# Matthew-Mosior/text-compression

Measured on AMD Instinct MI355X. Metric: BWT+MTF+RLE encode MB/s on 1 GiB ACGTN, higher is better.
Workload: dtype u8; 1 GPU; 1 x 1073741824-byte iid ACGTN record(s) (splitmix64 counter generator), fused BWT->MTF->RLE encode, in/out resident in HBM; record_bytes=1073741824, records=1, parallelism=record-per-gpu x1

## Files before the change

include/textcomp_debug.h:

```cpp
#ifndef TEXTCOMP_DEBUG_H
#define TEXTCOMP_DEBUG_H
#include "textcomp.h"
#ifdef __cplusplus
extern "C" {
#endif
int tc_dbg_checksum64_dev(tc_ctx *ctx, const void *d_p, uint64_t bytes, uint64_t *out);
int tc_dbg_stream_bench(tc_ctx *ctx, uint64_t bytes, int width, int mode, int iters, double *gbps);
int tc_dbg_sort_bench(tc_ctx *ctx, uint64_t n, int key_bits, int iters, int check, double *ms_per_pass);
int tc_dbg_scatter_bench(tc_ctx *ctx, uint64_t n, uint32_t bins, uint32_t xrun, int iters, double *ms_per_pass);
int tc_dbg_dispatch_probe(tc_ctx *ctx, uint32_t grid, uint32_t lds_bytes, uint32_t spin_cycles, uint32_t *out6);
int tc_dbg_lcp_set_short_cap(tc_ctx *ctx, uint32_t cap);
int tc_dbg_fm_set_lcp_fanout(tc_ctx *ctx, uint32_t fanout);
int tc_dbg_lz_set_tile(tc_ctx *ctx, uint32_t tile);
int tc_dbg_msd_split_used(tc_ctx *ctx, uint32_t *used);
int tc_dbg_msd_dir(tc_ctx *ctx, uint32_t out[2]);
int tc_dbg_tied_probe(tc_ctx *ctx, uint32_t out[2]);
int tc_dbg_ibwt_walk(tc_ctx *ctx, uint32_t out[3]);
int tc_dbg_seg_sort(tc_ctx *ctx, uint64_t *keys, uint32_t *vals, uint32_t m, int rbits, uint32_t levels[16]);
int tc_dbg_tied_small(tc_ctx *ctx, int mode, uint32_t *slot, uint32_t *idx, uint32_t *grp, uint32_t m,
                      uint32_t *t_idx, uint32_t *t_rank, uint32_t *tpos);
#ifdef __cplusplus
}
#endif
#endif
```

text-compression_amd/csrc/tc_common.hpp:

```cpp
#pragma once
#include <hip/hip_runtime.h>
#include <stdint.h>
#include <stdio.h>
#include <string.h>

#include <string>
#include <vector>

#include "textcomp.h"

typedef uint8_t u8;
typedef uint16_t u16;
typedef uint32_t u32;
typedef uint64_t u64;
typedef int16_t i16;
typedef int32_t i32;
typedef int64_t i64;

#define TC_WAVE 64

struct tc_ctx {
    int device = 0;
    hipStream_t stream = nullptr;
    char *ws = nullptr;
    size_t ws_cap = 0;
    size_t ws_off = 0;
    std::vector<hipMemGenericAllocationHandle_t> ws_chunks;
    size_t ws_chunk_bytes = 0, ws_mapped = 0;
    size_t ws_reserved = 0;
    u32 *d_err = nullptr;
    u64 *d_scalars = nullptr;
    u64 *h_scalars = nullptr;
    u8 *h_hdr = nullptr;
    hipEvent_t ev[8] = {};
    hipEvent_t pev[2 * 16] = {};
    int profile = 0;
    int coding = 0;
    int num_cus = 0;
    int reserved_cus = 0;
    void *hostpipe = nullptr;
    u32 stats_ws_grown = 0;
    u32 lcp_cap = 0;
    u32 fm_lcp_fanout = 0;
    u32 lz_tile = 0;
    int msd_dir_used = 0;
    int msd_split_used = 0;
    int tied_probe_used = 0;
    u32 tied_probe_found = 0;
    u32 ibwt_attempts = 0, ibwt_overflowed = 0, ibwt_extra_taken = 0;
    int mtf_fastin_failed = 0;
    int live_comms = 0;
    int safe_tickets = 0;
    u32 ticket_fallbacks = 0;
    int pev_used = 0;
    std::string err;
    tc_stats stats = {};
};

struct TcFail {
    int code;
};

#define TC_HIP(ctx, expr)                                                                  \
    do {                                                                                   \
        hipError_t e__ = (expr);                                                           \
        if (e__ != hipSuccess) {                                                           \
            char b__[512];                                                                 \
            snprintf(b__, sizeof b__, "%s:%d: %s -> %s", __FILE__, __LINE__, #expr,        \
                     hipGetErrorString(e__));                                              \
            (ctx)->err = b__;                                                              \
            throw TcFail{e__ == hipErrorOutOfMemory ? TC_ERR_OOM : TC_ERR_HIP};            \
        }                                                                                  \
    } while (0)

#define TC_FAIL(ctx, code_, ...)                         \
    do {                                                 \
        char b__[512];                                   \
        snprintf(b__, sizeof b__, __VA_ARGS__);          \
        (ctx)->err = b__;                                \
        throw TcFail{code_};                             \
    } while (0)

#define TC_LAUNCH_CHECK(ctx) TC_HIP(ctx, hipGetLastError())

struct Arena {
    char *base;
    size_t off = 0, peak = 0;
    explicit Arena(char *b) : base(b) {}
    template <class T>
    T *get(size_t count) {
        size_t bytes = (count * sizeof(T) + 255) & ~size_t(255);
        T *p = base ? reinterpret_cast<T *>(base + off) : nullptr;
        off += bytes;
        if (off > peak) peak = off;
        return p;
    }
    void rewind(size_t mark) { off = mark; }
};

void tc_ws_reserve(tc_ctx *ctx, size_t bytes);
template <class F>
static inline void tc_ws_plan(tc_ctx *ctx, size_t base, F &&fn) {
    Arena dry(nullptr);
    fn(dry, true);
    tc_ws_reserve(ctx, base + dry.peak);
    Arena A(ctx->ws + base);
    fn(A, false);
}
u32 tc_persistent_grid(tc_ctx *ctx, int blocks_per_cu);
template <class K>
static inline u32 tc_persistent_grid_for(tc_ctx *ctx, K kernel, int threads, int want_per_cu) {
    int occ = 0;
    if (hipOccupancyMaxActiveBlocksPerMultiprocessor(&occ, kernel, threads, 0) != hipSuccess || occ < 1) {
        (void)hipGetLastError();
        occ = 1;
    }
    return tc_persistent_grid(ctx, occ < want_per_cu ? occ : want_per_cu);
}
void *tc_chunked_alloc(tc_ctx *ctx, size_t bytes, int chunk_log2, void **handle);
void tc_chunked_free(void *handle);
void tc_sync_check(tc_ctx *ctx);

static inline u32 tc_cdiv(u64 a, u64 b) { return (u32)((a + b - 1) / b); }

#ifdef __HIPCC__

__device__ __forceinline__ u32 lane_id() { return __lane_id(); }

__device__ __forceinline__ u64 lanemask_lt() {
    return (1ull << lane_id()) - 1ull;
}

__device__ __forceinline__ u32 wave_incl_sum(u32 v) {
#pragma unroll
    for (int d = 1; d < 64; d <<= 1) {
        u32 t = __shfl_up(v, d, 64);
        if ((int)lane_id() >= d) v += t;
    }
    return v;
}
__device__ __forceinline__ u32 wave_incl_max(u32 v) {
#pragma unroll
    for (int d = 1; d < 64; d <<= 1) {
        u32 t = __shfl_up(v, d, 64);
        if ((int)lane_id() >= d) v = v > t ? v : t;
    }
    return v;
}
__device__ __forceinline__ u64 wave_incl_max64(u64 v) {
#pragma unroll
    for (int d = 1; d < 64; d <<= 1) {
        u64 t = __shfl_up(v, d, 64);
        if ((int)lane_id() >= d) v = v > t ? v : t;
    }
    return v;
}
__device__ __forceinline__ u32 wave_sum(u32 v) {
#pragma unroll
    for (int d = 32; d >= 1; d >>= 1) v += __shfl_xor(v, d, 64);
    return v;
}
__device__ __forceinline__ u64 wave_max64(u64 v) {
#pragma unroll
    for (int d = 32; d >= 1; d >>= 1) {
        u64 t = __shfl_xor(v, d, 64);
        v = v > t ? v : t;
    }
    return v;
}

template <int NT>
__device__ __forceinline__ u32 block_excl_sum(u32 v, u32 *smem, u32 *total) {
    const int w = threadIdx.x >> 6;
    u32 inc = wave_incl_sum(v);
    __syncthreads();
    if (lane_id() == 63) smem[w] = inc;
    __syncthreads();
    u32 base = 0, tot = 0;
#pragma unroll
    for (int i = 0; i < NT / 64; i++) {
        u32 s = smem[i];
        if (i < w) base += s;
        tot += s;
    }
    *total = tot;
    return base + inc - v;
}

template <int NT>
__device__ __forceinline__ u64 block_incl_max64(u64 v, u64 *smem, u64 *total) {
    const int w = threadIdx.x >> 6;
    u64 inc = wave_incl_max64(v);
    __syncthreads();
    if (lane_id() == 63) smem[w] = inc;
    __syncthreads();
    u64 base = 0, tot = 0;
#pragma unroll
    for (int i = 0; i < NT / 64; i++) {
        u64 s = smem[i];
        if (i < w) base = base > s ? base : s;
        tot = tot > s ? tot : s;
// ... 99 lines not shown
```

text-compression_amd/csrc/tc_msd.hpp:

```cpp
#pragma once
#include "tc_sa.hpp"
#include "tc_msd_dir.hpp"

#ifndef MSD_NT
#define MSD_NT 1024
#endif
#ifndef MSD_ITEMS
#define MSD_ITEMS 8
#endif
#define MSD_TILE (MSD_NT * MSD_ITEMS)
#ifndef MSD_GROUP
#define MSD_GROUP 16
#endif
#define MSD_GLOG (MSD_GROUP == 32 ? 5 : MSD_GROUP == 16 ? 4 : 3)
#ifndef MSD_SUB
#define MSD_SUB 1
#endif
#ifndef MSD_BPC
#define MSD_BPC 1
#endif
#define MSD_LEVELS 3
#define MSDF_CAP_SMALL 2048
#ifndef MSDF_KO_NT
#define MSDF_KO_NT 256
// ... 19 lines not shown
    u32 ntot;
    const u32 *cnt_in;
    u32 *flags;
    u64 *dbg;
    u32 *dirfills;
};

#ifdef __HIPCC__

__device__ __forceinline__ u32 msd_tile_lo(u32 T, u32 b, u32 G) { return (u32)(((u64)T * b) / G); }
__device__ __forceinline__ u32 msd_block_of_tile(u32 T, u32 t, u32 G) {
    return (u32)((((u64)t + 1) * G - 1) / T);
}

__global__ void msd_root_kernel(u32 *pstart, u32 *pcnt, u32 N, u32 *maxchild, u32 *dirfills) {
    pstart[0] = 0;
    pcnt[0] = N;
    *maxchild = 0;
    *dirfills = 0;
}

__device__ __forceinline__ u32 msd_block_of_parent(const MsdLevel &L, u32 q, u32 G) {
    return (u32)(((u64)L.pstart[q] * G) / L.ntot);
}
__device__ __forceinline__ u32 msd_first_parent(const MsdLevel &L, u32 b, u32 G) {
    if (b == 0) return 0;
    if (b >= G) return L.nparents;
    u32 lo = 0, hi = L.nparents;
    while (lo < hi) {
        const u32 mid = (lo + hi) >> 1;
        if (msd_block_of_parent(L, mid, G) >= b) hi = mid; else lo = mid + 1;
    }
    return lo;
}
__device__ __forceinline__ void msd_block_range(const MsdLevel &L, u32 b, u32 G, u32 *t0, u32 *t1) {
    if (L.aligned) {
        *t0 = L.tpre[msd_first_parent(L, b, G)];
        *t1 = L.tpre[msd_first_parent(L, b + 1, G)];
    } else {
        const u32 T = L.tpre[L.nparents];
        *t0 = (u32)(((u64)T * b) / G);
        *t1 = (u32)(((u64)T * (b + 1)) / G);
    }
}

__global__ __launch_bounds__(1024) void msd_prep_kernel(const u32 *__restrict__ pcnt, u32 nparents,
                                                        u32 *__restrict__ tpre) {
    __shared__ u32 s_scan[1024 / 64 + 1];
    const u32 per = (nparents + 1023) / 1024;
    const u32 lo = threadIdx.x * per;
    u32 sum = 0;
    if (per == 64 && nparents == 65536u) {
        uint4 v[16];
        const uint4 *pv = reinterpret_cast<const uint4 *>(pcnt + lo);
#pragma unroll
        for (int i = 0; i < 16; i++) v[i] = pv[i];
        u32 t[64];
#pragma unroll
        for (int i = 0; i < 16; i++) {
            t[4 * i] = (v[i].x + MSD_TILE - 1) / MSD_TILE; t[4 * i + 1] = (v[i].y + MSD_TILE - 1) / MSD_TILE;
            t[4 * i + 2] = (v[i].z + MSD_TILE - 1) / MSD_TILE; t[4 * i + 3] = (v[i].w + MSD_TILE - 1) / MSD_TILE;
        }
#pragma unroll
        for (int i = 0; i < 64; i++) sum += t[i];
        u32 tot;
        u32 run = block_excl_sum<1024>(sum, s_scan, &tot);
        uint4 *ov = reinterpret_cast<uint4 *>(tpre + lo);
#pragma unroll
        for (int i = 0; i < 16; i++) {
            uint4 o;
            o.x = run; run += t[4 * i];
            o.y = run; run += t[4 * i + 1];
            o.z = run; run += t[4 * i + 2];
            o.w = run; run += t[4 * i + 3];
            ov[i] = o;
        }
        if (threadIdx.x == 0) tpre[nparents] = tot;
        return;
    }
    for (u32 i = 0; i < per; i++) {
        const u32 q = lo + i;
        if (q < nparents) sum += (pcnt[q] + MSD_TILE - 1) / MSD_TILE;
    }
    u32 tot;
    u32 run = block_excl_sum<1024>(sum, s_scan, &tot);
    for (u32 i = 0; i < per; i++) {
        const u32 q = lo + i;
        if (q < nparents) {
            tpre[q] = run;
            run += (pcnt[q] + MSD_TILE - 1) / MSD_TILE;
        }
    }
    if (threadIdx.x == 0) tpre[nparents] = tot;
}

__device__ __forceinline__ u32 msd_find_parent(const u32 *tpre, u32 nparents, u32 t) {
    u32 lo = 0, hi = nparents;
    while (hi - lo > 1) {
        const u32 mid = (lo + hi) >> 1;
        if (tpre[mid] <= t) lo = mid; else hi = mid;
    }
    return lo;
}

struct MsdTileInfo {
    u32 base;
    u32 valid;
    u32 q;
    u32 last;
};
struct MsdCur {
    u32 q, tq0, tq1, ps, pc;
};
__device__ __forceinline__ void msd_cur_init(const MsdLevel &L, MsdCur &c, u32 t) {
    c.q = msd_find_parent(L.tpre, L.nparents, t);
    c.tq0 = L.tpre[c.q]; c.tq1 = L.tpre[c.q + 1]; c.ps = L.pstart[c.q]; c.pc = L.pcnt[c.q];
}
__device__ __forceinline__ void msd_cur_info(const MsdLevel &L, MsdCur &c, u32 t, u32 t_end, MsdTileInfo *out) {
    if (t >= t_end) {
        out->base = 0; out->valid = 0; out->q = 0; out->last = 0;
        return;
    }
    if (t >= c.tq1) {
        u32 q = c.q + 1;
        while (L.tpre[q + 1] <= t) q++;
        c.q = q; c.tq0 = L.tpre[q]; c.tq1 = L.tpre[q + 1]; c.ps = L.pstart[q]; c.pc = L.pcnt[q];
    }
    const u32 off = (t - c.tq0) * MSD_TILE;
    out->base = c.ps + off;
    out->valid = c.pc - off < MSD_TILE ? c.pc - off : MSD_TILE;
    out->q = c.q;
    out->last = (t + 1 >= t_end || t + 1 >= c.tq1) ? 1u : 0u;
}

struct MsdTextDigit {
    const u8 *text;
    u32 n;
    u32 B, s;
    u16 lut[256];
    u32 hash_ok, hsh, tlo, thi;
};

#ifndef MSD_XCD_MAP
#define MSD_XCD_MAP 0
#endif
__device__ __forceinline__ u32 msd_logical_wg(u32 b, u32 G) {
    return (MSD_XCD_MAP && (G & 7u) == 0) ? (b & 7u) * (G >> 3) + (b >> 3) : b;
}

struct MsdJointRows {
    u8 row[256];
    u8 dig[128];
};
template <bool TEXT, bool JOINT, bool HI>
__device__ __forceinline__ void msd_count_body(const MsdLevel &L, const u64 *__restrict__ keys,
                                               const MsdTextDigit &td, u32 *__restrict__ joint_out,
                                               const MsdJointRows &jr) {
    static_assert(!HI || (!TEXT && JOINT), "the high halves serve the joint count of keys only");
    __shared__ u32 s_cnt[256];
    __shared__ u16 s_lut[TEXT ? 256 : 1];
    __shared__ u32 s_seg[4];
    __shared__ u32 s_joint[JOINT ? 32768 : 1];
    const u32 tid = threadIdx.x, G = gridDim.x, b = msd_logical_wg(blockIdx.x, G);
    if (tid < 256) s_cnt[tid] = 0;
    if (TEXT && tid < 256) s_lut[tid] = td.lut[tid];
    __shared__ u8 s_row[JOINT ? 256 : 1];
    if (JOINT) {
        for (u32 i = tid; i < 32768; i += MSD_NT) s_joint[i] = 0;
        if (tid < 256) s_row[tid] = jr.row[tid];
    }
    const u32 T = L.tpre[L.nparents];
    const u32 t0 = msd_tile_lo(T, b, G), t1 = msd_tile_lo(T, b + 1, G);
    if (t0 >= t1) return;
    u32 t = t0;
    u32 q = 0;
    if (tid == 0) q = msd_find_parent(L.tpre, L.nparents, t0);
    while (t < t1) {
        if (tid == 0) {
            while (L.tpre[q + 1] <= t) q++;
            const u32 tq0 = L.tpre[q], tq1 = L.tpre[q + 1];
            const u32 te = tq1 < t1 ? tq1 : t1;
            const u32 ps = L.pstart[q], pc = L.pcnt[q];
            const u32 lo = ps + (t - tq0) * MSD_TILE;
            const u64 hi = (u64)ps + (u64)(te - tq0) * MSD_TILE;
            s_seg[0] = q; s_seg[1] = lo; s_seg[2] = hi < (u64)ps + pc ? (u32)hi : ps + pc; s_seg[3] = te;
        }
        __syncthreads();
        const u32 sq = s_seg[0], lo = s_seg[1], hi = s_seg[2];
        t = s_seg[3];
        if (TEXT) {
            const bool words = td.s <= 5 && (u64)lo + 8 < td.n && ((((uintptr_t)td.text) + lo) & 15) == 0;
            u32 p = lo;
            if (words) {
                const u32 span = (u64)hi + 8 <= td.n ? hi - lo : td.n - 8 - lo;
                const u32 nfull = span / (16 * MSD_NT);
                const u32 *tw = reinterpret_cast<const u32 *>(td.text + lo);
                auto fetch = [&](u32 r, u32 *x) {
                    const u32 wi = (r * MSD_NT + tid) * 4;
#pragma unroll
                    for (int q = 0; q < 5; q++) x[q] = tw[wi + q];
                };
                auto tally = [&](const u32 *x) {
                    u32 cd[20];
                    if (td.hash_ok) {
#pragma unroll
                        for (int q = 0; q < 5; q++) {
                            const u32 y = __builtin_amdgcn_perm(td.thi, td.tlo, (x[q] >> td.hsh) & 0x07070707u);
#pragma unroll
                            for (int j = 0; j < 4; j++) cd[4 * q + j] = (y >> (8 * j)) & 255u;
                        }
                    } else {
#pragma unroll
                        for (int j = 0; j < 20; j++) cd[j] = s_lut[(x[j >> 2] >> (8 * (j & 3))) & 255u];
                    }
#pragma unroll
                    for (int k = 0; k < 16; k++) {
                        u32 g = 0;
#pragma unroll
                        for (int j = 0; j < 5; j++)
                            if (j < (int)td.s) g = g * td.B + cd[k + j];
                        atomicAdd(&s_cnt[g], 1u);
                    }
                };
                u32 r = 0;
                for (; r + 4 <= nfull; r += 4) {
                    u32 xa[5], xb[5], xc[5], xd[5];
                    fetch(r, xa); fetch(r + 1, xb); fetch(r + 2, xc); fetch(r + 3, xd);
                    tally(xa); tally(xb); tally(xc); tally(xd);
                }
                for (; r < nfull; r++) {
                    u32 x[5];
                    fetch(r, x);
                    tally(x);
                }
                p = lo + nfull * 16 * MSD_NT;
            }
            for (u64 i0 = (u64)p + tid; i0 < hi; i0 += MSD_NT) {
                u64 i = i0;
                u32 g = 0;
                for (u32 j = 0; j < td.s; j++, i++) g = g * td.B + (i < td.n ? (u32)s_lut[td.text[i]] : 0u);
                atomicAdd(&s_cnt[g], 1u);
            }
        } else {
            auto add_dd = [&](u32 dd) {
                if (JOINT) {
                    const u32 r = s_row[dd >> 8];
                    if (r != 0xffu) atomicAdd(&s_joint[(r << 8) | (dd & 255u)], 1u);
                    else {
                        atomicAdd(&s_cnt[dd >> 8], 1u);
                        atomicAdd(&joint_out[((size_t)sq * 256 + (dd >> 8)) * 256 + (dd & 255u)], 1u);
                    }
                } else {
                    atomicAdd(&s_cnt[dd >> 8], 1u);
                }
            };
            auto add = [&](u64 k) { add_dd((u32)(k >> (L.shift - 8)) & 0xffffu); };
            if (HI) {
                const u32 *khi = reinterpret_cast<const u32 *>(keys);
                const u32 hs = (u32)L.shift - 40u;
                auto add4 = [&](const uint4 v) {
                    add_dd((v.x >> hs) & 0xffffu); add_dd((v.y >> hs) & 0xffffu);
                    add_dd((v.z >> hs) & 0xffffu); add_dd((v.w >> hs) & 0xffffu);
                };
                const u32 a0 = (lo + 3u) & ~3u, a = a0 < hi ? a0 : hi;
                if (lo + tid < a) add_dd((khi[lo + tid] >> hs) & 0xffffu);
                const u32 nq = (hi - a) >> 2;
                const uint4 *q4 = reinterpret_cast<const uint4 *>(khi + a);
                u32 i = tid;
                for (; i + 3 * MSD_NT < nq; i += 4 * MSD_NT) {
                    const uint4 v0 = q4[i], v1 = q4[i + MSD_NT], v2 = q4[i + 2 * MSD_NT], v3 = q4[i + 3 * MSD_NT];
                    add4(v0); add4(v1); add4(v2); add4(v3);
                }
                for (; i < nq; i += MSD_NT) add4(q4[i]);
                const u32 p = a + 4 * nq + tid;
                if (p < hi) add_dd((khi[p] >> hs) & 0xffffu);
            } else {
                u32 p = lo + tid;
                for (; p + 3 * MSD_NT < hi; p += 4 * MSD_NT) {
                    const u64 k0 = keys[p], k1 = keys[p + MSD_NT], k2 = keys[p + 2 * MSD_NT], k3 = keys[p + 3 * MSD_NT];
                    add(k0); add(k1); add(k2); add(k3);
                }
                for (; p < hi; p += MSD_NT) add(keys[p]);
            }
        }
        __syncthreads();
        if (JOINT) {
            for (u32 w = tid; w < 32768; w += MSD_NT) {
                const u32 v = s_joint[w];
                if (v) {
                    atomicAdd(&joint_out[((size_t)sq * 256 + jr.dig[w >> 8]) * 256 + (w & 255u)], v);
                    atomicAdd(&s_cnt[jr.dig[w >> 8]], v);
                    s_joint[w] = 0;
                }
            }
            __syncthreads();
        }
        if (tid < 256) {
            L.seg[((size_t)sq + b) * 256 + tid] = s_cnt[tid];
            s_cnt[tid] = 0;
        }
    }
}
template <bool TEXT, bool JOINT>
__global__ __launch_bounds__(MSD_NT) void msd_count_kernel(MsdLevel L, const u64 *__restrict__ keys,
                                                           MsdTextDigit td, u32 *__restrict__ joint_out,
                                                           MsdJointRows jr) {
    msd_count_body<TEXT, JOINT, false>(L, keys, td, joint_out, jr);
}
__global__ __launch_bounds__(MSD_NT) void msd_count_hi_kernel(MsdLevel L, const u32 *__restrict__ khi,
                                                              MsdTextDigit td, u32 *__restrict__ joint_out,
                                                              MsdJointRows jr) {
    msd_count_body<false, true, true>(L, reinterpret_cast<const u64 *>(khi), td, joint_out, jr);
}

__global__ __launch_bounds__(256) void msd_scan_kernel(MsdLevel L, u32 G, u32 *maxchild) {
    __shared__ u32 s_scan[256 / 64 + 1];
    const u32 q = blockIdx.x, d = threadIdx.x;
    const u32 cnt = L.pcnt[q];
    const size_t c = (size_t)q * 256 + d;
    if (cnt == 0) {
        L.ccnt[c] = 0;
        L.cstart[c] = L.pstart[q];
        return;
    }
    if (L.aligned) {
        const u32 tot = L.cnt_in[c];
        u32 all;
        const u32 excl = block_excl_sum<256>(tot, s_scan, &all);
        const u32 start = L.pstart[q] + excl;
        L.cstart[c] = start;
        L.ccnt[c] = tot;
        L.seg[((size_t)q + msd_block_of_parent(L, q, G)) * 256 + d] = start;
        if (d == 0 && all != cnt) atomicOr(L.flags, 8u);
        if (maxchild) {
            u32 m = tot;
#pragma unroll
            for (int x = 32; x >= 1; x >>= 1) {
                const u32 o = __shfl_xor(m, x, 64);
                m = m > o ? m : o;
            }
            if ((d & 63) == 0 && m > MSDF_CAP_SMALL) atomicMax(maxchild, m);
        }
        return;
    }
    const u32 T = L.tpre[L.nparents];
    const u32 bf = msd_block_of_tile(T, L.tpre[q], G), bl = msd_block_of_tile(T, L.tpre[q + 1] - 1, G);
    u32 tot = 0;
#pragma unroll 8
    for (u32 b = bf; b <= bl; b++) {
        const u32 v = L.seg[((size_t)q + b) * 256 + d];
        tot += msd_tile_lo(T, b, G) < msd_tile_lo(T, b + 1, G) ? v : 0u;
    }
    u32 all;
    const u32 excl = block_excl_sum<256>(tot, s_scan, &all);
    u32 run = L.pstart[q] + excl;
    L.cstart[c] = run;
    L.ccnt[c] = tot;
#pragma unroll 8
    for (u32 b = bf; b <= bl; b++) {
        const size_t o = ((size_t)q + b) * 256 + d;
        const u32 v = L.seg[o];
        if (msd_tile_lo(T, b, G) >= msd_tile_lo(T, b + 1, G)) continue;
        L.seg[o] = run;
        run += v;
    }
    if (maxchild) {
        u32 m = tot;
#pragma unroll
        for (int x = 32; x >= 1; x >>= 1) {
            const u32 o = __shfl_xor(m, x, 64);
            m = m > o ? m : o;
        }
        if ((d & 63) == 0 && m > MSDF_CAP_SMALL) atomicMax(maxchild, m);
    }
}

typedef u32 msd_u32x4 __attribute__((ext_vector_type(4)));
template <bool KEYGEN, bool VALS, bool SPLIT, bool DIR = false>
__device__ __forceinline__ void msd_partition_body(const MsdLevel &L, const u64 *kin, const u32 *vin,
                                                   u64 *kout, u32 *vout, u32 *shi, u32 *slo, const u8 *text,
                                                   const RadixKeyGen &kg) {
    static_assert(!SPLIT || !VALS, "the split layout is the key-only levels'");
    static_assert(!DIR || (!KEYGEN && !SPLIT), "the directory is the aligned level's");
    __shared__ __attribute__((aligned(16))) u64 s_keys[MSD_TILE];
    __shared__ __attribute__((aligned(16))) u32 s_vals[VALS ? MSD_TILE : 4];
    __shared__ __attribute__((aligned(16))) u64 c_keys[256 * MSD_GROUP];
    __shared__ __attribute__((aligned(16))) u32 c_vals[VALS ? 256 * MSD_GROUP : 4];
    __shared__ u32 s_cnt[256 * MSD_SUB], s_dstart[256 * MSD_SUB], s_r[256], s_cur[256], s_ph[256];
    __shared__ u32 s_scan[16];
    __shared__ u64 s_lmask[4];
#ifdef MSD_PROFILE
    __shared__ u64 s_dbg[2];
    if (threadIdx.x == 0) { s_dbg[0] = 0; s_dbg[1] = 0; }
#endif
    __shared__ u16 s_live[256];
    __shared__ u16 s_klut[KEYGEN ? 256 : 1];
    constexpr bool KG_SPLIT = KEYGEN && !VALS && MSD_ITEMS == 8;
    __shared__ __attribute__((aligned(16))) u8 s_kr[KG_SPLIT ? MSD_TILE + 16 + 80 + 32 : 16];
    __shared__ __attribute__((aligned(16))) u8 s_kg8[KG_SPLIT ? MSD_TILE + 64 : 16];
    __shared__ u32 s_scan2[2];
    static_assert(MSD_GROUP == 8 || MSD_GROUP == 16 || MSD_GROUP == 32, "group = 8, 16 or 32 pairs");
    constexpr u32 DIRCAP = DIR ? (VALS ? 128 : 1024) : 1;
    __shared__ MsdDirEnt s_dir[DIRCAP];
    __shared__ u32 s_rseg[DIR ? 256 : 1];
    __shared__ u64 s_rmask[4];
    __shared__ u32 s_nq[4], s_dst[6];
    static_assert(((size_t)MSD_TILE * (VALS ? 12 : 8) + 256 * MSD_GROUP * (VALS ? 12 : 8) + 8192 + (KG_SPLIT ? 2 * MSD_TILE + 256 : 0) + (DIR ? DIRCAP * sizeof(MsdDirEnt) + 1024 + 128 : 0)) * (VALS ? 1 : MSD_BPC) <= 163840, "LDS budget");
    __shared__ MsdTileInfo s_info[4];

    const u32 tid = threadIdx.x, G = gridDim.x, b = msd_logical_wg(blockIdx.x, G);
    if (KEYGEN && tid < 256) s_klut[tid] = kg.lut[tid];
    if (tid < 256) { s_r[tid] = 0; s_ph[tid] = 0; s_cur[tid] = 0; }
    for (u32 i = tid; i < 256 * MSD_SUB; i += MSD_NT) s_cnt[i] = 0;
    if (DIR) {
        if (tid == 0 || tid == 64) {
            const u32 w = tid >> 6;
            u32 q = 0, tq = 0;
            if (!(*L.flags & 8u)) {
                q = msd_first_parent(L, b + w, G);
                tq = L.tpre[q];
            }
            s_scan2[w] = tq; s_dst[1 + w] = q;
        }
        if (tid == 0) { s_dst[0] = 0; s_dst[3] = 0; s_dst[4] = MSD_DIR_NONE; }
    } else if (tid == 0) {
        u32 ta = 0, tb = 0;
        if (!(L.aligned && (*L.flags & 8u))) msd_block_range(L, b, G, &ta, &tb);
        s_scan2[0] = ta; s_scan2[1] = tb;
    }
    __syncthreads();
    const u32 t0 = s_scan2[0], t1 = s_scan2[1];
    if (t0 >= t1) return;
    MsdCur cs = {};
    u32 dir_e = 0, dir_k = 0;
    auto dir_refill = [&]() {
        u32 n = 0, qn = s_dst[1];
        const u32 qe = s_dst[2];
        while (n == 0 && qn < qe) {
            const u32 q = qn + tid;
            const bool in = q < qe;
            const u32 pc = in ? L.pcnt[q] : 0u, ps = in ? L.pstart[q] : 0u;
            const u64 m = __ballot(pc != 0);
            if ((tid & 63) == 0) s_scan[tid >> 6] = (u32)__popcll(m);
            __syncthreads();
            u32 before = 0, tot = 0;
#pragma unroll
            for (u32 i = 0; i < MSD_NT / 64; i++) {
                const u32 c = s_scan[i];
                tot += c;
                before += i < (tid >> 6) ? c : 0u;
            }
            const u32 rank = before + (u32)__popcll(m & ((1ull << (tid & 63)) - 1ull));
            if (pc != 0 && rank < DIRCAP) { s_dir[rank].q = q; s_dir[rank].ps = ps; s_dir[rank].pc = pc; }
            if (pc != 0 && rank == DIRCAP) s_dst[5] = q;
            __syncthreads();
            if (tot > DIRCAP) { n = DIRCAP; qn = s_dst[5]; }
            else { n = tot; qn = qe - qn < (u32)MSD_NT ? qe : qn + MSD_NT; }
            if (tid == 0) atomicAdd(L.dirfills, 1u);
        }
        __syncthreads();
        if (tid == 0) { s_dst[0] = n; s_dst[1] = qn; s_dst[3] = 0; }
        dir_e = 0; dir_k = 0;
    };
    auto dir_gen = [&](u32 x) {
        MsdDirCur c = {dir_e, dir_k, s_dst[0], s_dst[1], s_dst[2], s_dst[3]};
// ... 1083 lines not shown
```

text-compression_amd/csrc/tc_sa.hpp:

```cpp
#pragma once
#include <type_traits>
#include "tc_radix.hpp"

#define SA_NT 256
#define SA_ITEMS 16
#define SA_TILE (SA_NT * SA_ITEMS)
#define KB_HALO 72

struct SaConfig {
    u32 sigma_text;
    u32 B;
    u32 w;
    u32 s;
    u32 P;
    u32 h0;
    double entropy;
    u16 lut[256];
};

#ifdef __HIPCC__

__global__ __launch_bounds__(256) void hist256_kernel(const u8 *__restrict__ text, u64 n,
                                                      u32 *__restrict__ counts) {
    __shared__ u32 s_h[256 * 64];
// ... 349 lines not shown
            slot = slots[k];
        }
        const u64 mle = hb[k] & ((2ull << l) - 1ull);
        const u32 hl = mle ? 63u - (u32)__builtin_clzll(mle) : 0u;
        const u32 sv = INIT ? 0u : (u32)__shfl((int)slot, (int)hl, 64);
        const u32 g = mle ? (INIT ? (u32)(jb + hl) : sv) : cur_head - 1u;
        if (hb[k]) {
            u32 hlast = 63u - (u32)__builtin_clzll(hb[k]);
            cur_head = (INIT ? (u32)(jb + hlast) : (u32)__shfl((int)slot, (int)hlast, 64)) + 1u;
        }
        const u32 o = cur_cnt + (u32)__popcll(ab[k] & lanemask_lt());
        cur_cnt += (u32)__popcll(ab[k]);
        if (!in) continue;
        if (INIT) {
            if (a.isa_only) {
                if (a.pairs) a.pairs[j] = ((u64)a.vals[j] << 32) | g;
                else a.isa[a.vals[j]] = g;
            } else {
                a.L[j] = (u8)(lowb[k >> 2] >> (8 * (k & 3)));
                const u32 v = a.vals[j];
                if (a.pairs) a.pairs[j] = ((u64)v << 32) | g;
                else if (a.isa) a.isa[v] = g;
                if (act) {
                    a.out_slot[o] = (u32)j;
                    a.out_idx[o] = v;
                    a.out_grp[o] = g;
                }
            }
        } else {
            const u32 i = a.vals_are_idx ? k0 : a.in_idx[k0];
            if (!act) {
                a.sa[slot] = i;
                a.L[slot] = i ? a.text[i - 1] : (u8)0;
            }
            const bool moved = g != reinterpret_cast<const u32 *>(a.keys)[2 * j + 1];
            u32 tp = 0;
            if (a.pairs) a.pairs[j] = moved ? ((u64)i << 32) | g : ~0ull;
            else if (a.isa) { if (moved) a.isa[i] = g; }
            else if (!a.norank) {
                tp = a.in_tpos[k0];
                if (moved) a.t_rank[tp] = g;
            }
            if (act) {
                a.out_slot[o] = slot;
                a.out_idx[o] = i;
                a.out_grp[o] = g;
                if (!a.isa && !a.norank) a.out_tpos[o] = tp;
            }
        }
    }
    __syncthreads();
    }
}

#define RBIN_NT 1024
#define RBIN_ITEMS 16
#define RBIN_TILE (RBIN_NT * RBIN_ITEMS)

__global__ __launch_bounds__(256) void rank_cursor_kernel(u32 *cursor, int shift) {
    cursor[threadIdx.x] = (u32)threadIdx.x << shift;
}

__global__ __launch_bounds__(RBIN_NT) void rank_bin_kernel(const u64 *__restrict__ in, u32 m, int shift,
                                                           u32 *__restrict__ cursor, u64 *__restrict__ out, u64 nslots) {
    __shared__ u64 s_stage[RBIN_TILE];
    __shared__ u32 s_cnt[256], s_lb[256], s_gb[256];
    __shared__ u32 s_scan[RBIN_NT / 64 + 1];
    const u32 tid = threadIdx.x;
    const u64 base = (u64)blockIdx.x * RBIN_TILE;
    const u32 valid = (u64)m - base < (u64)RBIN_TILE ? (u32)((u64)m - base) : (u32)RBIN_TILE;
    if (tid < 256) s_cnt[tid] = 0;
    __syncthreads();
    u64 v[RBIN_ITEMS];
    u32 r[RBIN_ITEMS];
#pragma unroll
    for (int k = 0; k < RBIN_ITEMS; k++) {
        const u32 p = k * RBIN_NT + tid;
        v[k] = p < valid ? in[base + p] : 0ull;
    }
#pragma unroll
    for (int k = 0; k < RBIN_ITEMS; k++) {
        const u32 p = k * RBIN_NT + tid;
        if (p >= valid) v[k] = ~0ull;
        if (v[k] != ~0ull) r[k] = atomicAdd(&s_cnt[(u32)(v[k] >> 32) >> shift], 1u);
    }
    __syncthreads();
    const u32 c = tid < 256 ? s_cnt[tid] : 0u;
    u32 tot;
    const u32 lb = block_excl_sum<RBIN_NT>(c, s_scan, &tot);
    if (tid < 256) {
        s_lb[tid] = lb;
        s_gb[tid] = c ? atomicAdd(&cursor[tid], c) : 0u;
    }
    __syncthreads();
#pragma unroll
    for (int k = 0; k < RBIN_ITEMS; k++) {
        const u32 p = k * RBIN_NT + tid;
        if (v[k] != ~0ull) s_stage[s_lb[(u32)(v[k] >> 32) >> shift] + r[k]] = v[k];
    }
    __syncthreads();
#pragma unroll
    for (int k = 0; k < RBIN_ITEMS; k++) {
        const u32 p = k * RBIN_NT + tid;
        if (p < tot) {
            const u64 x = s_stage[p];
            const u32 d = (u32)(x >> 32) >> shift;
            const u64 g = (u64)s_gb[d] + (p - s_lb[d]);
            if (g < nslots) out[g] = x;
        }
    }
}

#define RSCAT_NT 256
#define RSCAT_ITEMS 8
__global__ __launch_bounds__(RSCAT_NT) void rank_scatter_kernel(const u64 *__restrict__ part, u64 nslots, int shift,
                                                                 const u32 *__restrict__ cursor, u32 *__restrict__ isa) {
    const u64 base = (u64)blockIdx.x * (RSCAT_NT * RSCAT_ITEMS);
    u64 x[RSCAT_ITEMS];
    u32 cur[RSCAT_ITEMS];
    bool ok[RSCAT_ITEMS];
#pragma unroll
    for (int k = 0; k < RSCAT_ITEMS; k++) {
        const u64 p = base + (u64)k * RSCAT_NT + threadIdx.x;
        cur[k] = p < nslots ? cursor[p >> shift] : 0u;
    }
#pragma unroll
    for (int k = 0; k < RSCAT_ITEMS; k++) {
        const u64 p = base + (u64)k * RSCAT_NT + threadIdx.x;
        ok[k] = p < nslots && (u32)p < cur[k];
        x[k] = ok[k] ? part[p] : 0ull;
    }
#pragma unroll
    for (int k = 0; k < RSCAT_ITEMS; k++)
        if (ok[k]) isa[(u32)(x[k] >> 32)] = (u32)x[k];
}

#ifndef FIN_WPW
#define FIN_WPW 8
#endif
#ifndef FIN_NT
#define FIN_NT 256
#endif

__global__ __launch_bounds__(256) void unary_sa_kernel(const u8 *__restrict__ text, u32 n, u32 *__restrict__ sa,
                                                        u8 *__restrict__ L) {
    const u64 j = (u64)blockIdx.x * 256 + threadIdx.x;
    if (j > n) return;
    sa[j] = n - (u32)j;
    L[j] = j < n ? text[0] : (u8)0;
}

#define SAMP_N 8192
#define SAMP_SLOTS 16384
__global__ __launch_bounds__(1024) void sample_dup_kernel(const u8 *__restrict__ text, u32 n, RadixKeyGen kg,
                                                           int topbits, u32 *out) {
    __shared__ u32 table[SAMP_SLOTS];
    __shared__ u16 s_lut[256];
    __shared__ u32 s_dups;
    for (int i = threadIdx.x; i < SAMP_SLOTS; i += 1024) table[i] = 0xFFFFFFFFu;
    if (threadIdx.x < 256) s_lut[threadIdx.x] = kg.lut[threadIdx.x];
    if (threadIdx.x == 0) s_dups = 0;
    __syncthreads();
    u32 dups = 0;
    const u32 nf = ((u32)topbits + kg.w - 1) / kg.w;
    constexpr int SPT = SAMP_N / 1024;
    const bool words = nf * kg.s <= 16;
    u32 tw[SPT][4];
    u64 qs[SPT];
#pragma unroll
    for (int j = 0; j < SPT; j++) {
        const u32 k = threadIdx.x + 1024u * (u32)j;
        u64 z = (u64)(k + 1) * 0x9E3779B97F4A7C15ull;
        z = (z ^ (z >> 29)) * 0xBF58476D1CE4E5B9ull;
        qs[j] = (u64)(((z >> 32) * (u64)n) >> 32);
        const bool in = words && qs[j] + 16 <= n;
#pragma unroll
        for (int x = 0; x < 4; x++) {
            u32 v = 0;
            if (in) __builtin_memcpy(&v, text + qs[j] + 4 * x, 4);
            tw[j][x] = v;
        }
    }
#pragma unroll
    for (int j = 0; j < SPT; j++) {
        u64 q = qs[j];
        const bool in = words && q + 16 <= n;
        u64 key = 0;
        int sh = 64;
        u32 pos = 0;
        for (u32 f = 0; f < nf; f++) {
            u32 g = 0;
            for (u32 t = 0; t < kg.s; t++, q++, pos++) {
                u32 c;
                if (in) {
                    u32 wsel = tw[j][0];
                    wsel = (pos >> 2) == 1 ? tw[j][1] : wsel;
                    wsel = (pos >> 2) == 2 ? tw[j][2] : wsel;
                    wsel = (pos >> 2) == 3 ? tw[j][3] : wsel;
                    c = (u32)s_lut[(wsel >> (8 * (pos & 3))) & 255u];
                } else {
                    c = q < n ? (u32)s_lut[text[q]] : 0u;
                }
                g = g * kg.B + c;
            }
            sh -= kg.w;
            key |= (u64)g << sh;
        }
        u64 kt = key >> (64 - topbits);
        if (topbits > 32) kt = (kt ^ (kt >> 31)) * 0xD6E8FEB86659FD93ull >> 32;
        const u32 v = (u32)kt;
        if (v == 0xFFFFFFFFu) continue;
        u32 slot = (v * 0x9E3779B1u) >> 18;
        for (int probe = 0; probe < SAMP_SLOTS; probe++) {
            const u32 old = atomicCAS(&table[slot], 0xFFFFFFFFu, v);
            if (old == 0xFFFFFFFFu) break;
            if (old == v) { dups++; break; }
            slot = (slot + 1) & (SAMP_SLOTS - 1);
        }
    }
    dups = wave_sum(dups);
    if (lane_id() == 0 && dups) atomicAdd(&s_dups, dups);
    __syncthreads();
    if (threadIdx.x == 0) *out = s_dups;
}

struct FinishArgs {
    const u64 *keys;
    const u32 *sa_in;
    u32 N;
    int tshift;
    int lshift, lbits;
    u32 *sa_out;
    u8 *L;
    u32 *out_slot, *out_idx, *out_grp;
    u32 act_cap;
    u32 *counters;
    u32 *rcount;
    u32 rcap;
    u32 fix_cap;
    u32 *ovbits;
};

#define FIN_REGIONS 64
#define FIN_RSTRIDE 64
#ifndef FIN_STAGE
#define FIN_STAGE 192
#endif
__global__ __launch_bounds__(FIN_NT) void finish_kernel(FinishArgs a) {
    __shared__ u32 s_low[FIN_NT / 64][128];
#if FIN_STAGE
    __shared__ u32 s_stg[FIN_NT / 64][3][FIN_STAGE + 128];
#endif
    const int w = threadIdx.x >> 6, l = threadIdx.x & 63;
    u32 *low = s_low[w];
#if FIN_STAGE
    __shared__ u32 s_nstg[FIN_NT / 64];
    __shared__ u32 s_base;
    u32 nstg = 0;
    const u32 region = blockIdx.x % FIN_REGIONS;
    u32 *rctr = a.rcount + region * FIN_RSTRIDE;
    const u32 rbase = region * a.rcap;
    auto flush = [&](bool have_base, u32 base) {
        if (!have_base) {
            if (l == 0) base = atomicAdd(rctr, nstg);
            base = __shfl(base, 0, 64);
        }
        __builtin_amdgcn_wave_barrier();
        for (u32 e = l; e < nstg; e += 64) {
            const u32 o = rbase + base + e;
            if (base + e < a.rcap) {
                a.out_slot[o] = s_stg[w][0][e];
                a.out_idx[o] = s_stg[w][1][e];
                a.out_grp[o] = s_stg[w][2][e];
            }
        }
        __builtin_amdgcn_wave_barrier();
        nstg = 0;
    };
#endif
    const u64 N = a.N;
    const u64 wave = (u64)blockIdx.x * (FIN_NT / 64) + w;
    const u64 ws0 = wave * 64 * FIN_WPW;
#if !FIN_STAGE
#error "finish_kernel needs the staged hand-over (FIN_STAGE > 0)"
#endif
    const u64 lowmask = a.lbits >= 64 ? ~0ull : ((1ull << a.lbits) - 1ull);

    u64 kk[FIN_WPW + 1];
    u32 vv[FIN_WPW + 1];
    const bool interior = ws0 + (u64)(FIN_WPW + 1) * 64 <= N;
    if (interior) {
#pragma unroll
        for (int c = 0; c <= FIN_WPW; c++) {
            const u64 pos = ws0 + (u64)c * 64 + l;
            kk[c] = a.keys[pos];
            vv[c] = a.sa_in[pos];
        }
    } else {
#pragma unroll
        for (int c = 0; c <= FIN_WPW; c++) {
            const u64 pos = ws0 + (u64)c * 64 + l;
            kk[c] = pos < N ? a.keys[pos] : ~0ull;
            vv[c] = pos < N ? a.sa_in[pos] : 0u;
        }
    }
    u64 tprev = (ws0 > 0 && ws0 <= N) ? (a.keys[ws0 - 1] >> a.tshift) : 0;
    bool hasprev = ws0 > 0;

    auto window = [&](auto full_tag, const int win) {
        constexpr bool FULL = decltype(full_tag)::value;
        const u64 ws = ws0 + (u64)win * 64;
        if (!FULL && ws >= N) return;
        const u64 kA = kk[win], kB = kk[win + 1];
        const u32 vA = vv[win], vB = vv[win + 1];
        const bool inA = FULL || ws + l < N, inB = FULL || ws + 64 + l < N;
        const u64 tA = kA >> a.tshift, tB = kB >> a.tshift;
        u64 upA = __shfl_up(tA, 1, 64);
        u64 lastA = __shfl(tA, 63, 64);
        u64 upB = __shfl_up(tB, 1, 64);
        bool hA = inA && ((l == 0) ? (!hasprev || tA != tprev) : (tA != upA));
        bool hB = inB && ((l == 0) ? (tB != lastA) : (tB != upB));
        const u64 hbA = __ballot(hA), hbB = __ballot(hB);
        const u64 inbA = __ballot(inA), inbB = __ballot(inB);
        const int a0 = hbA ? __builtin_ctzll(hbA) : 64;
        const int b0 = hbB ? __builtin_ctzll(hbB) : 64;
        if (hbA && !hbB && (~inbB) == 0ull) {
            if (l == 0 && !(__hip_atomic_load(&a.counters[1], __ATOMIC_RELAXED, __HIP_MEMORY_SCOPE_AGENT) & 1u))
                atomicOr(&a.counters[1], 1u);
        }
        const bool ownA = inA && l >= a0;
        const bool ownB = inB && hbA && l < b0;
        u64 mleA = hbA & ((2ull << l) - 1ull);
        int sA = mleA ? 63 - __builtin_clzll(mleA) : 0;
        u64 mgtA = (l == 63) ? 0ull : (hbA & ~((2ull << l) - 1ull));
        int endA_in_A = mgtA ? __builtin_ctzll(mgtA) : -1;
        int lastHeadA = hbA ? 63 - __builtin_clzll(hbA) : 0;
        int endB = b0 < 64 ? 64 + b0 : (int)(__popcll(inbA) + __popcll(inbB));
        int tAend = endA_in_A >= 0 ? endA_in_A : endB;
        const u32 lowA = (u32)((kA >> a.lshift) & lowmask), lowB = (u32)((kB >> a.lshift) & lowmask);
        low[l] = lowA;
        low[64 + l] = lowB;
        __builtin_amdgcn_wave_barrier();
        const int cA = l, cB = 64 + l;
        const int sB = lastHeadA, tBend = endB;
        int lenA = ownA ? tAend - sA : 0;
        int maxlen = lenA;
#pragma unroll
        for (int d = 32; d >= 1; d >>= 1) {
            int o = __shfl_xor(maxlen, d, 64);
            maxlen = maxlen > o ? maxlen : o;
        }
        u32 rankA = 0, ltA = 0, leA = 0;
        for (int t = 0; t < maxlen; t++) {
            const int u = sA + t;
            if (ownA && u < tAend) {
                const u32 y = low[u];
                ltA += y < lowA;
                leA += y <= lowA;
                rankA += (y < lowA) | ((y == lowA) & (u < cA));
            }
        }
        const u32 eqA = ownA ? leA - ltA - 1u : 0u;
        u32 rankB = 0, ltB = 0, leB = 0;
        if (hbA && b0 > 0) {
            for (int u = sB; u < tBend; u++) {
                const u32 y = low[u];
                ltB += y < lowB;
                leB += y <= lowB;
                rankB += (y < lowB) | ((y == lowB) & (u < cB));
            }
        }
        const u32 eqB = ownB ? leB - ltB - 1u : 0u;
        __builtin_amdgcn_wave_barrier();
        const bool actA = ownA && eqA > 0, actB = ownB && eqB > 0;
        const u64 abA = __ballot(actA), abB = __ballot(actB);
        const u32 nact = (u32)__popcll(abA) + (u32)__popcll(abB);
// ... 964 lines not shown
```

text-compression_amd/csrc/tc_sa_host.hpp:

```cpp
#pragma once
#include <chrono>

#include "tc_sa_plan.hpp"

#ifndef SA_KDIR_BITS
#define SA_KDIR_BITS 26
#endif
struct SaBuffers {
    u64 *k0, *k1;
    u32 *v0, *v1;
    u32 *isa;
    u32 *v2;
    u32 *act[2][4];
    u64 *sk[2];
    u32 *sv[2];
    u32 *t_idx, *t_rank;
    u64 *t_bits;
    u32 *t_dir;
    u32 *t_bsum;
    u32 *fin_rc;
    u32 *kdir;
    u64 sparse_cap;
    u32 *hist;
    u64 *rstatus;
    u64 *gstatus;
    u32 *counts;
    u32 *msd_pstart[MSD_LEVELS + 1], *msd_pcnt[MSD_LEVELS + 1];
    u32 *msd_tpre[MSD_LEVELS], *msd_seg[MSD_LEVELS];
    u32 *msd_joint;
    u32 msd_grid;
    TiedTable tp;
    SegBuffers seg;
    u32 *chain_ref, *chain_code, *chain_summ;
};

static inline u64 msd_min_n() { return (u64)env_int("TC_SA_MSD_MIN_LOG2", 27) >= 40 ? ~0ull : 1ull << env_int("TC_SA_MSD_MIN_LOG2", 27); }
static inline bool msd_wanted(u64 N) { return env_int("TC_SA_MSD", 1) != 0 && N >= msd_min_n() && N >= 1024; }

static void seg_carve(Arena &A, u64 N, SegBuffers &g) {
    g.cap_runs = (size_t)(N / SEG_CAP + 2);
    g.cap_tiles = (size_t)(N / SEG_PT + 2) + g.cap_runs;
    g.segbits = A.get<u64>(seg_bit_words(N));
    g.ybits = A.get<u64>(seg_bit_words(N));
    for (int q = 0; q < 2; q++) {
        g.lstart[q] = A.get<u32>(g.cap_runs);
        g.lsize[q] = A.get<u32>(g.cap_runs);
        g.ltbase[q] = A.get<u32>(g.cap_runs);
        g.lshift[q] = A.get<u32>(g.cap_runs);
    }
    g.tile_seg = A.get<u32>(g.cap_tiles);
    g.hist = A.get<u32>(g.cap_runs * 256);
    g.mm = A.get<u32>(g.cap_runs * 2);
    g.counters = A.get<u32>(64);
}

static size_t sa_carve(Arena &A, u64 N, SaBuffers &b, bool own_v1) {
    b.k0 = A.get<u64>(N + 32);
    b.k1 = A.get<u64>(N);
    b.v0 = A.get<u32>(N);
    b.v1 = own_v1 ? A.get<u32>(N) : nullptr;
    b.isa = A.get<u32>(N + 1);
    b.v2 = A.get<u32>(N);
    b.sparse_cap = N / 8 + 1024;
    for (int s = 0; s < 2; s++) {
        for (int q = 0; q < 3; q++) b.act[s][q] = A.get<u32>(N);
        b.act[s][3] = A.get<u32>(b.sparse_cap);
        b.sk[s] = A.get<u64>(b.sparse_cap);
        b.sv[s] = A.get<u32>(b.sparse_cap);
    }
    b.t_idx = A.get<u32>(b.sparse_cap);
    b.t_rank = A.get<u32>(b.sparse_cap);
    b.t_bits = A.get<u64>(N / 64 + 2);
    b.t_dir = A.get<u32>(N / 64 + 2);
    b.t_bsum = A.get<u32>(N / 64 / BDIR_TILE + 2);
    b.fin_rc = A.get<u32>(FIN_REGIONS * FIN_RSTRIDE + 128);
    b.kdir = A.get<u32>(((size_t)1 << SA_KDIR_BITS) + 2 + ((size_t)1 << SA_KDIR_BITS) / KDF_CHUNK + 64);
    b.hist = A.get<u32>(RDX_MAX_PASSES * RDX_BINS);
    b.rstatus = A.get<u64>(radix_status_words(N));
    b.gstatus = A.get<u64>(2 * (size_t)tc_cdiv(N, GRP_TILE) + 4);
    b.counts = A.get<u32>(260);
    seg_carve(A, N, b.seg);
    for (int l = 0; l <= MSD_LEVELS; l++) b.msd_pstart[l] = b.msd_pcnt[l] = nullptr;
    if (msd_wanted(N)) {
        b.msd_grid = 256 * MSD_BPC;
        size_t np = 1;
        for (int l = 0; l <= MSD_LEVELS; l++, np *= 256) {
            b.msd_pstart[l] = A.get<u32>(np);
            b.msd_pcnt[l] = A.get<u32>(np);
            if (l < MSD_LEVELS) {
                b.msd_tpre[l] = A.get<u32>(np + 1);
                b.msd_seg[l] = A.get<u32>((np + b.msd_grid) * 256);
            }
        }
        b.msd_joint = A.get<u32>((size_t)256 * 256 * 256);
        b.tp.key = A.get<u64>((size_t)1 << TP_SLOT_BITS);
        b.tp.grp = A.get<u32>((size_t)1 << TP_SLOT_BITS);
        b.tp.cnt = A.get<u32>((size_t)1 << TP_SLOT_BITS);
        b.tp.bloom = A.get<u32>(((size_t)1 << TP_BLOOM_LOG2) / 32);
    }
    b.chain_ref = A.get<u32>(N + 1);
    b.chain_code = A.get<u32>(N + 1);
    b.chain_summ = A.get<u32>(chain_summ_words());
    return A.off;
}

enum SaSlot {
    SA_SLOT_PRIMARY = 0,
    SA_SLOT_ACTIVE = 1,
    SA_SLOT_PROBE = 11,
    SA_SLOT_TIED = 12,
    SA_SLOT_DROPPED = 13,
    SA_SLOT_SAMPLE = 14,
    SA_SLOT_MAXCHILD = 15,
    SA_SLOT_SEG = 24,
    SA_SLOT_ERR = 62,
    SA_SLOT_MSD_PROF = 64,
    SA_SLOT_MSDK_PROF = 112,
    SA_SLOT_MSD_DIR = 122,
};
static inline u32 sa_slot_lo(const tc_ctx *ctx, int slot) { return (u32)(ctx->h_scalars[slot] & 0xffffffffu); }
static inline u32 sa_slot_hi(const tc_ctx *ctx, int slot) { return (u32)(ctx->h_scalars[slot] >> 32); }
static inline u32 *sa_dev_slot(tc_ctx *ctx, int slot) { return reinterpret_cast<u32 *>(ctx->d_scalars + slot); }

#ifdef SEG_PROFILE
static void seg_profile_dump(tc_ctx *ctx, u32 m) {
    u64 h[16];
    TC_HIP(ctx, hipStreamSynchronize(ctx->stream));
    TC_HIP(ctx, hipMemcpyFromSymbol(h, HIP_SYMBOL(seg_prof), sizeof h));
    const double w = (double)(h[7] | 1);
    fprintf(stderr, "seg_small: %llu members, %llu windows (that sort), mid members per window %.0f | cycles per window: bits %.0f attr+masks %.0f (prefix) %.0f image %.0f tiny+compact %.0f tiny store %.0f network %.0f store %.0f\n",
            (unsigned long long)m, (unsigned long long)h[7], h[8] / w, h[0] / w, h[1] / w, 0.0, h[2] / w, h[3] / w, h[4] / w, h[5] / w, h[6] / w);
    memset(h, 0, sizeof h);
    TC_HIP(ctx, hipMemcpyToSymbol(HIP_SYMBOL(seg_prof), h, sizeof h));
}
#else
static inline void seg_profile_dump(tc_ctx *, u32) {}
#endif

static void seg_sort_pairs(tc_ctx *ctx, SegBuffers &g, u64 *kx, u32 *vx, u64 *ky, u32 *vy, u32 m, int rbits,
                           u32 *levels = nullptr) {
    hipStream_t s = ctx->stream;
    if (levels) memset(levels, 0, 16 * sizeof(u32));
    const u32 nwords = (u32)seg_bit_words(m);
    TC_HIP(ctx, hipMemsetAsync(g.ybits, 0, (size_t)nwords * sizeof(u64), s));
    TC_HIP(ctx, hipMemsetAsync(g.counters, 0, 8 * sizeof(u32), s));
    u32 igrid = tc_cdiv((u64)nwords * 64, 256);
    if (igrid > 16384) igrid = 16384;
    seg_init_kernel<<<igrid, 256, 0, s>>>(kx, m, g.segbits, nwords, g.lstart[0], g.lsize[0], g.ltbase[0], g.lshift[0],
                                          (u32)(rbits > 8 ? rbits - 8 : 0), g.counters, (u32)g.cap_runs);
    TC_LAUNCH_CHECK(ctx);
    const int nlev = 8;
    int cur = 0;
    for (int L = 0;; L++) {
        TC_HIP(ctx, hipMemcpyAsync(&ctx->h_scalars[SA_SLOT_SEG], g.counters + 2 * cur, 2 * sizeof(u32), hipMemcpyDeviceToHost, s));
        TC_HIP(ctx, hipStreamSynchronize(s));
        const u32 S = sa_slot_lo(ctx, SA_SLOT_SEG), T = sa_slot_hi(ctx, SA_SLOT_SEG);
        if (S == 0) break;
        if (levels && L < nlev) { levels[2 * L] = S; levels[2 * L + 1] = T; }
        if (L >= nlev) TC_FAIL(ctx, TC_ERR_INTERNAL, "segmented sort: %u runs still unsorted after %d levels", S, nlev);
        if (S > g.cap_runs || T > g.cap_tiles) TC_FAIL(ctx, TC_ERR_INTERNAL, "segmented sort: %u long runs / %u tiles exceed the tables", S, T);
        const int nxt = cur ^ 1;
        TC_HIP(ctx, hipMemsetAsync(g.hist, 0, (size_t)S * 256 * sizeof(u32), s));
        seg_mm_init_kernel<<<tc_cdiv(S, 256), 256, 0, s>>>(g.mm, S);
        TC_LAUNCH_CHECK(ctx);
        TC_HIP(ctx, hipMemsetAsync(g.counters + 2 * nxt, 0, 2 * sizeof(u32), s));
        u32 wgrid = tc_cdiv(S, 4);
        if (wgrid > 8192) wgrid = 8192;
        seg_tilemap_kernel<<<wgrid, 256, 0, s>>>(g.lsize[cur], g.ltbase[cur], S, g.tile_seg, (u32)g.cap_tiles);
        TC_LAUNCH_CHECK(ctx);
        seg_count_kernel<<<T, 256, 0, s>>>(kx, ky, g.lstart[cur], g.lsize[cur], g.ltbase[cur], g.lshift[cur], g.tile_seg, g.counters + 2 * cur, g.hist, g.mm);
        TC_LAUNCH_CHECK(ctx);
        seg_scan_kernel<<<wgrid, 256, 0, s>>>(g.lstart[cur], g.lsize[cur], g.lshift[cur], g.counters + 2 * cur, g.hist, g.mm, g.segbits, 0,
                                              g.lstart[nxt], g.lsize[nxt], g.ltbase[nxt], g.lshift[nxt], g.counters + 2 * nxt, (u32)g.cap_runs);
        TC_LAUNCH_CHECK(ctx);
        seg_scatter_kernel<<<T, 256, 0, s>>>(kx, vx, ky, vy, g.lstart[cur], g.lsize[cur], g.ltbase[cur], g.lshift[cur], g.tile_seg, g.counters + 2 * cur,
                                             g.hist, g.mm, g.ybits);
        TC_LAUNCH_CHECK(ctx);
        cur = nxt;
    }
    seg_small_kernel<<<tc_cdiv(m, SEG_SPAN), SEG_NT, 0, s>>>(kx, vx, ky, vy, m, g.segbits, g.ybits);
    TC_LAUNCH_CHECK(ctx);
    seg_profile_dump(ctx, m);
}

static void sa_choose_config(const u32 *counts, u64 n, int forced_fields, SaConfig &c) {
    u32 sig = 0;
    double H = 0;
    for (int v = 0; v < 256; v++) {
        c.lut[v] = 0;
        if (counts[v]) {
            c.lut[v] = (u16)(++sig);
            double p = (double)counts[v] / (double)n;
            H -= p * log2(p);
        }
    }
    c.sigma_text = sig;
    c.B = sig + 1;
    if (c.B <= 16) {
        c.w = 8;
        c.s = 1;
        u32 pw = c.B;
        while (pw * c.B <= 256) {
            pw *= c.B;
            c.s++;
        }
    } else {
        c.s = 1;
        c.w = (u32)ceil_log2_u64(c.B);
    }
    u32 pmax = 56 / c.w;
    double need = (double)ceil_log2_u64(n + 1) + 8.0;
    double per_field = H * c.s;
    u32 P = pmax;
    if (per_field > 1e-9) {
        double pf = ceil(need / per_field);
        if (pf < (double)pmax) P = (u32)pf;
    }
    if (P < 1) P = 1;
    if (forced_fields > 0) P = (u32)forced_fields;
    if (P > pmax) P = pmax;
    c.P = P;
    c.h0 = P * c.s;
    c.entropy = H;
}

static void sa_run(tc_ctx *ctx, SaBuffers &b, const u8 *d_text, u64 n, u32 *d_sa, u8 *d_L,
                   u64 *primary, u32 *counts256_out);

struct TicketTrip {};
__global__ void err_or_kernel(u32 *err, u32 bits) { atomicOr(err, bits); }
static void ticket_check(tc_ctx *ctx) {
    if (env_int("TC_DBG_TICKET_TRIP", 0) != 0) {
        err_or_kernel<<<1, 1, 0, ctx->stream>>>(ctx->d_err, 2u);
        TC_LAUNCH_CHECK(ctx);
    }
    TC_HIP(ctx, hipMemcpyAsync(&ctx->h_scalars[SA_SLOT_ERR], ctx->d_err, sizeof(u32), hipMemcpyDeviceToHost,
                               ctx->stream));
    TC_HIP(ctx, hipStreamSynchronize(ctx->stream));
    if (sa_slot_lo(ctx, SA_SLOT_ERR) & 2u) throw TicketTrip{};
}

static void sa_build(tc_ctx *ctx, Arena &A, const u8 *d_text, u64 n, u32 *d_sa, u8 *d_L,
                     u64 *primary, u32 *counts256_out, bool dry) {
    const u64 N = n + 1;
    SaBuffers b;
    sa_carve(A, N, b, d_sa == nullptr);
    if (dry) return;
    try {
        sa_run(ctx, b, d_text, n, d_sa, d_L, primary, counts256_out);
    } catch (const TicketTrip &) {
        tc_memset_async(ctx, ctx->d_err, 0, sizeof(u32));
        ctx->safe_tickets = 1;
        ctx->ticket_fallbacks++;
        sa_run(ctx, b, d_text, n, d_sa, d_L, primary, counts256_out);
    }
    ctx->stats.ticket_fallbacks = ctx->ticket_fallbacks;
}

struct SaRun {
    tc_ctx *ctx;
    SaBuffers &b;
    const u8 *text;
    u64 n, N;
    int rbits;
    u32 *d_sa;
    u32 *sa;
    u8 *d_L;
    SaKnobs K;
    SaConfig cfg;
    int rshift;
    u64 bin_min;
    u64 *part_act1;
    bool part_act1_ok;
    u64 m = 0;
    u64 h_start = 0;
    const u64 *skeys = nullptr;
    const u64 *tkeys = nullptr;
    int tkeys_shift = 0;
    bool isa_ready = false;
    bool dense = false;
    RankLookup rl = {};
    std::chrono::steady_clock::time_point trace_t0;

    hipStream_t stream() const { return ctx->stream; }
    tc_stats &st() const { return ctx->stats; }
};

template <class X>
static inline void sa_fill(const SaConfig &c, X &x) {
    x.B = c.B; x.w = c.w; x.s = c.s; x.P = c.P;
    memcpy(x.lut, c.lut, sizeof x.lut);
}
static inline void sa_fill(const SaConfig &c, MsdTextDigit &x) {
    x.B = c.B; x.s = c.s;
    memcpy(x.lut, c.lut, sizeof x.lut);
}
static RadixKeyGen sa_keygen(const SaRun &R) {
    RadixKeyGen kg;
    sa_fill(R.cfg, kg);
    kg.n_text = (u32)R.n;
    kg.hash_ok = 0; kg.hsh = 0; kg.tlo = 0; kg.thi = 0;
    return kg;
}
static RadixBuffers sa_radix_buffers(const SaRun &R, u64 *keys, u64 *keys_alt, u32 *vals, u32 *vals_alt) {
    RadixBuffers rb;
    rb.keys = keys; rb.keys_alt = keys_alt; rb.vals = vals; rb.vals_alt = vals_alt;
    rb.hist = R.b.hist; rb.status = R.b.rstatus; rb.status_cap = radix_status_words(R.N);
    return rb;
}
static RadixBuffers sa_sparse_buffers(const SaRun &R) {
    return sa_radix_buffers(R, R.b.sk[0], R.b.sk[1], R.b.sv[0], R.b.sv[1]);
}

static void sa_trace_buffers(const SaRun &R) {
    if (R.K.trace != 2) return;
    fprintf(stderr, "textcomp: buffers text %p k0 %p k1 %p v0 %p v1 %p sa %p L %p\n", (const void *)R.text, (void *)R.b.k0,
            (void *)R.b.k1, (void *)R.b.v0, (void *)R.b.v1, (void *)R.d_sa, (void *)R.d_L);
}
static void sa_trace_step(SaRun &R, const char *what, u64 count) {
    if (!R.K.trace) return;
    (void)hipStreamSynchronize(R.stream());
    auto t1 = std::chrono::steady_clock::now();
    fprintf(stderr, "textcomp:   %-28s %10llu  %8.3f ms\n", what, (unsigned long long)count,
            std::chrono::duration<double, std::milli>(t1 - R.trace_t0).count());
    R.trace_t0 = t1;
}
static void sa_trace_tied_checksums(SaRun &R, u32 fm) {
    if (R.K.trace < 2 || fm == 0) return;
    tc_ctx *ctx = R.ctx;
    std::vector<u32> hk(fm), hh(fm), hs(fm), hg(fm);
    tc_d2h(ctx, hk.data(), R.b.act[0][1], fm * sizeof(u32));
    tc_d2h(ctx, hh.data(), R.b.act[0][3], fm * sizeof(u32));
    tc_d2h(ctx, hs.data(), R.b.act[0][0], fm * sizeof(u32));
    tc_d2h(ctx, hg.data(), R.b.act[0][2], fm * sizeof(u32));
    TC_HIP(ctx, hipStreamSynchronize(R.stream()));
    u64 a1 = 0, a2 = 0, a3 = 0, a4 = 0;
    for (u32 i = 0; i < fm; i++) { a1 += hk[i]; a2 += hh[i]; a3 += hs[i]; a4 += hg[i]; }
    fprintf(stderr, "textcomp: tied members: sum klo %llx khi %llx slot %llx grp %llx\n", (unsigned long long)a1, (unsigned long long)a2, (unsigned long long)a3, (unsigned long long)a4);
    for (u32 i = 0; i < fm && i < 6; i++) fprintf(stderr, "textcomp:   member %u: klo %08x khi %06x slot %u grp %u\n", i, hk[i], hh[i], hs[i], hg[i]);
}
static void sa_trace_group_sizes(SaRun &R, int cur, u32 mm) {
    if (!R.K.trace) return;
    tc_ctx *ctx = R.ctx;
    u64 *gh = reinterpret_cast<u64 *>(R.b.hist);
    tc_memset_async(ctx, gh, 0, 32 * sizeof(u64));
    group_size_hist_kernel<<<tc_cdiv(mm, 256), 256, 0, R.stream()>>>(R.b.act[cur][0], R.b.act[cur][2], mm, gh);
    u64 hh32[32];
    tc_d2h(ctx, hh32, gh, sizeof hh32);
    (void)hipStreamSynchronize(R.stream());
    fprintf(stderr, "textcomp:   members by group size 2^c:");
    for (int c = 0; c < 32; c++) if (hh32[c]) fprintf(stderr, " %d:%.1f%%", c, 100.0 * (double)hh32[c] / (double)mm);
    fprintf(stderr, "\n");
    R.trace_t0 = std::chrono::steady_clock::now();
}
static void sa_trace_chain_tables(SaRun &R, int cur, u32 mm, u32 hh, const ChainDims &cd, const u64 *chain_path, const u64 *chain_sign) {
    if (!R.K.trace) return;
    tc_ctx *ctx = R.ctx;
    unsigned long long *dg = reinterpret_cast<unsigned long long *>(R.b.hist);
    tc_memset_async(ctx, dg, 0, 8 * sizeof(u64));
    chain_diag_kernel<<<4096, 256, 0, R.stream()>>>(R.b.act[cur][1], R.b.act[cur][2], mm, chain_path, chain_sign, R.b.chain_code, dg);
    u64 hd[8];
    tc_d2h(ctx, hd, dg, sizeof hd);
    (void)hipStreamSynchronize(R.stream());
    fprintf(stderr, "textcomp:   chain tables (h = %u, %u x %u cells of %u rows, %s ranks): members %u, on path %llu, k = 0: %llu, largest k %llu\n",
            hh, cd.nb, cd.h, cd.bk, R.dense ? "dense" : "sparse", mm, (unsigned long long)hd[0], (unsigned long long)hd[1], (unsigned long long)hd[2]);
    R.trace_t0 = std::chrono::steady_clock::now();
}
#ifdef MSDK_PROFILE
static void msdk_profile_dump(tc_ctx *ctx) {
    u64 h[10];
    tc_d2h(ctx, h, ctx->d_scalars + SA_SLOT_MSDK_PROF, sizeof h);
    TC_HIP(ctx, hipStreamSynchronize(ctx->stream));
    const double c = (double)(h[8] | 1);
    fprintf(stderr, "finish (key-only): chunks %llu, keys per chunk %.0f | cycles per chunk: land %.0f B %.0f zero+B %.0f bins+B %.0f scan+B %.0f scatter+B %.0f walk+prefetch+rank+B %.0f copy-out %.0f\n",
            (unsigned long long)h[8], h[9] / c, h[0] / c, h[1] / c, h[2] / c, h[3] / c, h[4] / c, h[5] / c, h[6] / c, h[7] / c);
    tc_memset_async(ctx, ctx->d_scalars + SA_SLOT_MSDK_PROF, 0, sizeof h);
}
#else
static inline void msdk_profile_dump(tc_ctx *) {}
#endif
#ifdef MSD_PROFILE
static void msd_profile_dump(tc_ctx *ctx) {
    u64 h[48];
    tc_d2h(ctx, h, ctx->d_scalars + SA_SLOT_MSD_PROF, sizeof h);
    TC_HIP(ctx, hipStreamSynchronize(ctx->stream));
    for (int l = 0; l < MSD_LEVELS; l++)
        fprintf(stderr, "msd level %d: tiles %llu | cursor+B0 %llu keygen/S1+B1 %llu S2 %llu S3 %llu land %llu B3 %llu S4 %llu (cycles per tile)\n", l + 1,
                (unsigned long long)h[16 * l + 1], (unsigned long long)(h[16 * l] / (h[16 * l + 1] | 1)), (unsigned long long)(h[16 * l + 2] / (h[16 * l + 1] | 1)),
                (unsigned long long)(h[16 * l + 3] / (h[16 * l + 1] | 1)), (unsigned long long)(h[16 * l + 4] / (h[16 * l + 1] | 1)), (unsigned long long)(h[16 * l + 5] / (h[16 * l + 1] | 1)),
                (unsigned long long)(h[16 * l + 6] / (h[16 * l + 1] | 1)), (unsigned long long)(h[16 * l + 7] / (h[16 * l + 1] | 1)));
    for (int l = 0; l < MSD_LEVELS; l++)
        fprintf(stderr, "   level %d, S1 alone per tile: wave 0 %llu, last wave %llu cycles; slowest wave B0 -> before B1 %llu, B0 -> prefetch issued %llu\n", l + 1,
                (unsigned long long)(h[16 * l + 8] / (h[16 * l + 1] | 1)), (unsigned long long)(h[16 * l + 9] / (h[16 * l + 1] | 1)),
                (unsigned long long)(h[16 * l + 10] / (h[16 * l + 1] | 1)), (unsigned long long)(h[16 * l + 11] / (h[16 * l + 1] | 1)));
    for (int l = 0; l < MSD_LEVELS; l++)
        fprintf(stderr, "   level %d, ends of segments: %llu, %llu cycles each (flush, barriers, next ranges; outside the per-tile stamps)\n", l + 1,
                (unsigned long long)h[16 * l + 13], (unsigned long long)(h[16 * l + 12] / (h[16 * l + 13] | 1)));
    tc_memset_async(ctx, ctx->d_scalars + SA_SLOT_MSD_PROF, 0, sizeof h);
}
#else
static inline void msd_profile_dump(tc_ctx *) {}
#endif

static void sa_dbg_msd_dir(tc_ctx *ctx, uint32_t out[2]) {
    u64 w = 0;
    out[0] = ctx->msd_dir_used ? 1u : 0u;
    out[1] = 0;
    if (ctx->msd_dir_used) {
        tc_d2h(ctx, &w, ctx->d_scalars + SA_SLOT_MSD_DIR, sizeof w);
        TC_HIP(ctx, hipStreamSynchronize(ctx->stream));
        out[1] = (u32)(w & 0xffffffffu);
    }
}

static void sa_run_group(SaRun &R, bool init, GroupArgs ga) {
    tc_ctx *ctx = R.ctx;
    hipStream_t s = R.stream();
    const u32 gtiles = tc_cdiv(R.N, GRP_TILE);
    u32 tiles = tc_cdiv(ga.count, GRP_TILE);
    tc_memset_async(ctx, R.b.gstatus, 0, (2 * (size_t)gtiles + 4) * sizeof(u64));
    ga.text = R.text; ga.sa = R.sa; ga.L = R.d_L;
    ga.status_max = R.b.gstatus; ga.status_sum = R.b.gstatus + gtiles;
    ga.ticket = reinterpret_cast<u32 *>(R.b.gstatus + 2 * (size_t)gtiles);
    ga.scalars = ctx->d_scalars; ga.err = ctx->d_err;
    u32 grid = init ? tc_persistent_grid_for(ctx, group_kernel<true>, GRP_NT, 2)
                    : tc_persistent_grid_for(ctx, group_kernel<false>, GRP_NT, 2);
    if (grid > tiles) grid = tiles;
    if (init) group_kernel<true><<<grid, GRP_NT, 0, s>>>(ga);
    else group_kernel<false><<<grid, GRP_NT, 0, s>>>(ga);
    TC_LAUNCH_CHECK(ctx);
}
static u64 sa_fetch_m(SaRun &R) {
    tc_d2h(R.ctx, R.ctx->h_scalars, R.ctx->d_scalars, 2 * sizeof(u64));
    TC_HIP(R.ctx, hipStreamSynchronize(R.stream()));
    return R.ctx->h_scalars[SA_SLOT_ACTIVE];
}
static void sa_apply_pairs(SaRun &R, const u64 *pairs, u32 count, u64 *part) {
    tc_ctx *ctx = R.ctx;
    hipStream_t s = R.stream();
    u32 *cursor = R.b.hist;
    rank_cursor_kernel<<<1, 256, 0, s>>>(cursor, R.rshift);
    TC_LAUNCH_CHECK(ctx);
    rank_bin_kernel<<<tc_cdiv(count, RBIN_TILE), RBIN_NT, 0, s>>>(pairs, count, R.rshift, cursor, part, R.N);
    TC_LAUNCH_CHECK(ctx);
    rank_scatter_kernel<<<tc_cdiv(R.N, RSCAT_NT * RSCAT_ITEMS), RSCAT_NT, 0, s>>>(part, R.N, R.rshift, cursor, R.b.isa);
    TC_LAUNCH_CHECK(ctx);
}

static RadixBuffers sa_build_keys_and_sort(SaRun &R, const RadixPlan &plan, bool sa_in_alt_at_end) {
    tc_ctx *ctx = R.ctx;
    SaBuffers &b = R.b;
    const SaConfig &cfg = R.cfg;
    hipStream_t s = R.stream();
    const u32 n = (u32)R.n;
    KeyBuildParams kp;
    sa_fill(cfg, kp);
    kp.plan.npass = plan.npass;
    for (int p = 0; p < plan.npass; p++) {
        kp.plan.shift[p] = plan.shift[p];
        kp.plan.mask[p] = plan.mask[p];
    }
    tc_memset_async(ctx, b.hist, 0, sizeof(u32) * RDX_MAX_PASSES * RDX_BINS);
    bool onehist = cfg.w == 8 && plan.npass < RDX_MAX_PASSES && R.K.kb_onehist != 0;
    for (int p = 0; p < plan.npass; p++)
        if (plan.mask[p] != 255u || plan.shift[p] % 8 != 0) onehist = false;
    const u32 kgrid = tc_cdiv(R.N, SA_TILE);
    const bool fuse = onehist && RDX_TILE == SA_TILE && R.K.keygen_fused != 0;
    R.st().keygen_fused = fuse ? 1u : 0u;
    const RadixKeyGen kg = sa_keygen(R);
    if (fuse) {
        u32 ggrid = tc_cdiv(R.N, 256 * 16 * 4);
        if (ggrid > 2048) ggrid = 2048;
        if (cfg.s == 3) ghist_kernel<3><<<ggrid, 256, 0, s>>>(R.text, n, kp, b.hist);
        else ghist_kernel<0><<<ggrid, 256, 0, s>>>(R.text, n, kp, b.hist);
        TC_LAUNCH_CHECK(ctx);
        keyhist_fix_kernel<<<1, 256, 0, s>>>(R.text, n, kp, b.hist);
    } else if (onehist) {
        if (cfg.s == 3 && cfg.P == 6) keybuild_kernel<true, 3, 6><<<kgrid, SA_NT, 0, s>>>(R.text, n, kp, b.k0, b.hist);
        else if (cfg.s == 3 && cfg.P == 5) keybuild_kernel<true, 3, 5><<<kgrid, SA_NT, 0, s>>>(R.text, n, kp, b.k0, b.hist);
        else keybuild_kernel<true, 0, 0><<<kgrid, SA_NT, 0, s>>>(R.text, n, kp, b.k0, b.hist);
        TC_LAUNCH_CHECK(ctx);
        keyhist_fix_kernel<<<1, 256, 0, s>>>(R.text, n, kp, b.hist);
    } else {
        keybuild_kernel<false, 0, 0><<<kgrid, SA_NT, 0, s>>>(R.text, n, kp, b.k0, b.hist);
    }
    TC_LAUNCH_CHECK(ctx);
    const bool even = plan.npass % 2 == 0;
    const bool start_in_sa = sa_in_alt_at_end ? !even : even;
    RadixBuffers rb = start_in_sa ? sa_radix_buffers(R, b.k0, b.k1, R.sa, b.v0) : sa_radix_buffers(R, b.k0, b.k1, b.v0, R.sa);
    ctx->pev_used = 0;
    const bool xcd_group = !ctx->safe_tickets && R.K.xcd_group != 0;
    radix_sort_pairs(ctx, rb, (u32)R.N, plan, true, true, true,
                     R.text, fuse ? &kg : nullptr, xcd_group);
    if (xcd_group) ticket_check(ctx);
    return rb;
}

static bool sa_alphabet(SaRun &R, u32 *counts256_out, u64 *primary) {
    tc_ctx *ctx = R.ctx;
    hipStream_t s = R.stream();
    tc_memset_async(ctx, R.b.counts, 0, 256 * sizeof(u32));
    {
        u32 grid = tc_cdiv(R.n, 256 * 64);
        if (grid > 2048) grid = 2048;
        if (grid < 1) grid = 1;
        hist256_kernel<<<grid, 256, 0, s>>>(R.text, R.n, R.b.counts);
        TC_LAUNCH_CHECK(ctx);
    }
    u32 counts[256];
    tc_d2h(ctx, counts, R.b.counts, sizeof counts);
    TC_HIP(ctx, hipStreamSynchronize(s));
    if (counts256_out) memcpy(counts256_out, counts, sizeof counts);
    sa_choose_config(counts, R.n, R.K.fields, R.cfg);
    if (R.cfg.sigma_text != 1 || R.n == 0) return false;
    unary_sa_kernel<<<tc_cdiv(R.N, 256), 256, 0, s>>>(R.text, (u32)R.n, R.sa, R.d_L);
    TC_LAUNCH_CHECK(ctx);
    *primary = R.n;
    tc_stats &st = R.st();
    st.sigma = 2; st.rounds = 0; st.radix_launches = 0; st.ms_radix = 0;
    return true;
}


static void sa_sample(SaRun &R, int topbits) {
    tc_ctx *ctx = R.ctx;
    sample_dup_kernel<<<1, 1024, 0, R.stream()>>>(R.text, (u32)R.n, sa_keygen(R), topbits, sa_dev_slot(ctx, SA_SLOT_SAMPLE));
    TC_LAUNCH_CHECK(ctx);
    tc_d2h(ctx, &ctx->h_scalars[SA_SLOT_SAMPLE], ctx->d_scalars + SA_SLOT_SAMPLE, sizeof(u64));
    TC_HIP(ctx, hipStreamSynchronize(R.stream()));
    R.st().sample_dups = sa_slot_lo(ctx, SA_SLOT_SAMPLE);
}

struct Round0Out {
    bool msd, msd_big, keyonly;
    int tb;
    FinishArgs fa;
    const u64 *keys;
    const u64 *keys_sorted;
    int npass;
};
static void sa_round0_begin(SaRun &R, int tb, Round0Out &o) {
    tc_ctx *ctx = R.ctx;
    SaBuffers &b = R.b;
    const int keybits = (int)(R.cfg.P * R.cfg.w);
    FinishArgs &fa = o.fa;
    o.tb = tb;
    o.keys_sorted = nullptr;
    fa.N = (u32)R.N; fa.tshift = 64 - tb;
    fa.lshift = 64 - keybits; fa.lbits = keybits - tb;
    fa.sa_out = R.sa; fa.L = R.d_L;
    fa.out_slot = b.act[1][0]; fa.out_idx = b.act[1][1]; fa.out_grp = b.act[1][2];
    fa.act_cap = (u32)R.N; fa.counters = sa_dev_slot(ctx, SA_SLOT_TIED);
    fa.rcount = b.fin_rc; fa.rcap = (u32)(R.N / FIN_REGIONS);
    fa.fix_cap = (u32)(b.sparse_cap - 1024);
    fa.ovbits = b.act[1][0];
    tc_memset_async(ctx, ctx->d_scalars + SA_SLOT_TIED, 0, 2 * sizeof(u64));
    tc_memset_async(ctx, b.fin_rc, 0, (FIN_REGIONS * FIN_RSTRIDE + 128) * sizeof(u32));
}

static Round0Out sa_round0_lsd(SaRun &R, const Round0Plan &pl) {
    Round0Out o;
    o.msd = o.msd_big = o.keyonly = false;
    sa_round0_begin(R, pl.topbits, o);
    R.st().msd_path = 0;
    RadixPlan plan;
    plan.add_range(64 - pl.topbits, 64);
    RadixBuffers rb = sa_build_keys_and_sort(R, plan, true);
    o.npass = plan.npass;
    o.keys = rb.keys;
    o.fa.keys = rb.keys; o.fa.sa_in = rb.vals;
    const u32 waves = tc_cdiv(R.N, 64 * FIN_WPW);
    finish_kernel<<<tc_cdiv(waves, FIN_NT / 64), FIN_NT, 0, R.stream()>>>(o.fa);
    TC_LAUNCH_CHECK(R.ctx);
    return o;
}

static Round0Out sa_round0_msd(SaRun &R, const Round0Plan &pl, bool keyonly) {
    tc_ctx *ctx = R.ctx;
    SaBuffers &b = R.b;
    const SaConfig &cfg = R.cfg;
    hipStream_t s = R.stream();
    tc_stats &st = R.st();
    const u32 n = (u32)R.n, N = (u32)R.N;
    Round0Out o;
    o.msd = true; o.msd_big = pl.msd_big; o.keyonly = keyonly;
    sa_round0_begin(R, 8 * MSD_LEVELS, o);
    u32 *counters = o.fa.counters;
    RadixKeyGen kg = sa_keygen(R);
    radix_keygen_hash(kg);
    if (R.K.keygen_hash == 0) kg.hash_ok = 0;
    MsdTextDigit td;
    sa_fill(cfg, td);
    td.text = R.text; td.n = n;
    td.hash_ok = kg.hash_ok; td.hsh = kg.hsh; td.tlo = kg.tlo; td.thi = kg.thi;
    u32 G = b.msd_grid < (u32)ctx->num_cus * MSD_BPC ? b.msd_grid : (u32)ctx->num_cus * MSD_BPC;
    if (ctx->reserved_cus > 0 && G > (u32)(ctx->num_cus - ctx->reserved_cus) * MSD_BPC)
        G = (u32)(ctx->num_cus - ctx->reserved_cus) * MSD_BPC;
    if (R.K.msd_grid > 0 && (u32)R.K.msd_grid < G) G = (u32)R.K.msd_grid;
    u32 *maxchild = sa_dev_slot(ctx, SA_SLOT_MAXCHILD);
    msd_root_kernel<<<1, 1, 0, s>>>(b.msd_pstart[0], b.msd_pcnt[0], N, maxchild, sa_dev_slot(ctx, SA_SLOT_MSD_DIR));
    TC_LAUNCH_CHECK(ctx);
    u64 *kbuf[2] = {b.k0, b.k1};
    u32 *vbuf[2] = {keyonly ? nullptr : b.v0, keyonly ? nullptr : R.sa};
    st.msd_keyonly = keyonly ? 1u : 0u;
    ctx->pev_used = 0;
    st.keygen_fused = 1;
    MsdJointRows jr;
    u32 nrows = 0;
    {
        memset(jr.row, 0xff, sizeof jr.row);
        memset(jr.dig, 0, sizeof jr.dig);
        u32 nd = 1;
        for (u32 j = 0; j < cfg.s; j++) nd *= cfg.B;
        for (u32 d = 0; d < nd && d < 256; d++) {
            bool real = true;
            for (u32 v = d, j = 0; j < cfg.s; j++, v /= cfg.B) real = real && (v % cfg.B) != 0;
            if (real) {
                if (nrows < 128) { jr.row[d] = (u8)nrows; jr.dig[nrows] = (u8)d; }
                nrows++;
            }
        }
    }
    const bool joint = R.K.msd_joint != 0 && nrows <= 128;
    const bool split = keyonly && joint && R.K.msd_split != 0 && MSD_LEVELS == 3;
    u32 *khi = reinterpret_cast<u32 *>(b.k0), *klo = khi + msd_split_npad(N);
    ctx->msd_split_used = split ? 1 : 0;
    const bool dir = joint && R.K.msd_dir != 0;
    ctx->msd_dir_used = dir ? 1 : 0;
    if (joint) tc_memset_async(ctx, b.msd_joint, 0, (size_t)256 * 256 * 256 * sizeof(u32));
    u32 np = 1;
    for (int l = 0; l < MSD_LEVELS; l++, np *= 256) {
        MsdLevel ML;
        ML.pstart = b.msd_pstart[l]; ML.pcnt = b.msd_pcnt[l]; ML.tpre = b.msd_tpre[l];
        ML.nparents = np; ML.shift = 56 - 8 * l; ML.seg = b.msd_seg[l];
        ML.cstart = b.msd_pstart[l + 1]; ML.ccnt = b.msd_pcnt[l + 1];
        ML.aligned = (joint && l == MSD_LEVELS - 1) ? 1 : 0;
        ML.ntot = N; ML.cnt_in = b.msd_joint; ML.flags = counters + 1;
        ML.dbg = ctx->d_scalars + SA_SLOT_MSD_PROF + 16 * l;
        ML.dirfills = sa_dev_slot(ctx, SA_SLOT_MSD_DIR);
        const u64 *kin = l ? kbuf[(l - 1) & 1] : nullptr;
        const u32 *vin = l ? vbuf[(l - 1) & 1] : nullptr;
        msd_prep_kernel<<<1, 1024, 0, s>>>(ML.pcnt, np, b.msd_tpre[l]);
        TC_LAUNCH_CHECK(ctx);
        if (l == 0) msd_count_kernel<true, false><<<G, MSD_NT, 0, s>>>(ML, nullptr, td, nullptr, jr);
        else if (ML.aligned) {  }
        else if (joint && l == MSD_LEVELS - 2 && split) msd_count_hi_kernel<<<G, MSD_NT, 0, s>>>(ML, khi, td, b.msd_joint, jr);
        else if (joint && l == MSD_LEVELS - 2) msd_count_kernel<false, true><<<G, MSD_NT, 0, s>>>(ML, kin, td, b.msd_joint, jr);
        else msd_count_kernel<false, false><<<G, MSD_NT, 0, s>>>(ML, kin, td, nullptr, jr);
        TC_LAUNCH_CHECK(ctx);
        msd_scan_kernel<<<np, 256, 0, s>>>(ML, G, l == MSD_LEVELS - 1 ? maxchild : nullptr);
        TC_LAUNCH_CHECK(ctx);
        const bool ev = ctx->profile && ctx->pev_used < 16;
        if (ev) TC_HIP(ctx, hipEventRecord(ctx->pev[2 * ctx->pev_used], s));
        if (split && l <= 1) {
            if (l == 0) msd_partition_split_kernel<true><<<G, MSD_NT, 0, s>>>(ML, khi, klo, nullptr, R.text, kg);
            else msd_partition_split_kernel<false><<<G, MSD_NT, 0, s>>>(ML, khi, klo, kbuf[1], R.text, kg);
        } else if (dir && ML.aligned) {
            if (keyonly) msd_partition_dir_kernel<false><<<G, MSD_NT, 0, s>>>(ML, kin, nullptr, kbuf[l & 1], nullptr, kg);
            else msd_partition_dir_kernel<true><<<G, MSD_NT, 0, s>>>(ML, kin, vin, kbuf[l & 1], vbuf[l & 1], kg);
        } else if (keyonly) {
            if (l == 0) msd_partition_kernel<true, false><<<G, MSD_NT, 0, s>>>(ML, nullptr, nullptr, kbuf[0], nullptr, R.text, kg);
            else msd_partition_kernel<false, false><<<G, MSD_NT, 0, s>>>(ML, kin, nullptr, kbuf[l & 1], nullptr, R.text, kg);
        } else if (l == 0) msd_partition_kernel<true><<<G, MSD_NT, 0, s>>>(ML, nullptr, nullptr, kbuf[0], vbuf[0], R.text, kg);
        else msd_partition_kernel<false><<<G, MSD_NT, 0, s>>>(ML, kin, vin, kbuf[l & 1], vbuf[l & 1], R.text, kg);
        TC_LAUNCH_CHECK(ctx);
        if (ev) {
            TC_HIP(ctx, hipEventRecord(ctx->pev[2 * ctx->pev_used + 1], s));
            ctx->pev_used++;
        }
    }
    o.keys = kbuf[(MSD_LEVELS - 1) & 1];
    MsdFinishArgs mf;
    mf.keys = o.keys; mf.vals = vbuf[(MSD_LEVELS - 1) & 1];
    mf.pcnt = b.msd_pcnt[MSD_LEVELS - 1];
    mf.cstart = b.msd_pstart[MSD_LEVELS]; mf.ccnt = b.msd_pcnt[MSD_LEVELS];
    mf.sa_out = R.sa; mf.L = R.d_L;
    mf.out_slot = o.fa.out_slot; mf.out_idx = o.fa.out_idx; mf.out_grp = o.fa.out_grp;
    mf.rcount = o.fa.rcount; mf.rcap = o.fa.rcap; mf.counters = counters;
    mf.kout = kbuf[MSD_LEVELS & 1];
    o.keys_sorted = mf.kout;
    mf.whole_list = b.msd_seg[MSD_LEVELS - 1];
    mf.whole_cap = 1u << 20;
    mf.out_khi = b.v0;
    MsdFinishLut *flut = reinterpret_cast<MsdFinishLut *>(b.msd_seg[MSD_LEVELS - 1] + 2 * (size_t)mf.whole_cap);
    msd_finish_lut_kernel<<<1, 256, 0, s>>>(b.msd_pcnt[1], flut);
    TC_LAUNCH_CHECK(ctx);
    mf.lut = R.K.msd_finish_lut != 0 ? flut : nullptr;
    if (pl.msd_big && keyonly) {
        msd_finish_kernel<MSDF_BIG_NT, MSDF_BIG_ITEMS, 1, 5, true, false><<<np / 256, MSDF_BIG_NT, 0, s>>>(mf);
    } else if (pl.msd_big) {
        msd_finish_kernel<MSDF_BIG_NT, MSDF_BIG_ITEMS, 1, 5, true><<<np / 256, MSDF_BIG_NT, 0, s>>>(mf);
        TC_LAUNCH_CHECK(ctx);
        msd_whole_kernel<<<1024, MSDW_NT, 0, s>>>(mf);
    } else if (keyonly && R.K.msd_finish_ko != 0) {
        msd_finish_ko_kernel<3><<<np / 256, 256, 0, s>>>(mf, flut);
        msdk_profile_dump(ctx);
    } else if (keyonly) {
        msd_finish_kernel<MSDF_KO_NT, MSDF_CAP_SMALL / MSDF_KO_NT, 4, 1, false, false><<<np / 256, MSDF_KO_NT, 0, s>>>(mf);
    } else {
        msd_finish_kernel<256, 8, 4, 1, false><<<np / 256, 256, 0, s>>>(mf);
    }
    TC_LAUNCH_CHECK(ctx);
    o.npass = MSD_LEVELS;
    st.msd_path = 1;
    msd_profile_dump(ctx);
    return o;
}

static bool sa_keyonly_recover(SaRun &R, u32 fm, u32 flags) {
    tc_ctx *ctx = R.ctx;
    SaBuffers &b = R.b;
    const SaConfig &cfg = R.cfg;
    hipStream_t s = R.stream();
    const u32 n = (u32)R.n;
    bool ok = fm <= TP_MAX_TIED && (u64)fm + 1024 <= b.sparse_cap && !(flags & 2u);
    if (ok) sa_trace_tied_checksums(R, fm);
    if (ok && fm > 0) {
        tc_memset_async(ctx, b.tp.key, 0, sizeof(u64) << TP_SLOT_BITS);
        tc_memset_async(ctx, b.tp.cnt, 0, sizeof(u32) << TP_SLOT_BITS);
        tc_memset_async(ctx, b.tp.bloom, 0, ((size_t)1 << TP_BLOOM_LOG2) / 8);
        u32 *d_total = sa_dev_slot(ctx, SA_SLOT_PROBE);
        tc_memset_async(ctx, d_total, 0, sizeof(u64));
        tied_table_kernel<<<tc_cdiv(fm, 256), 256, 0, s>>>(b.act[0][1], b.act[0][3], b.act[0][2], fm, cfg.B, cfg.s, cfg.P, b.tp);
        TC_LAUNCH_CHECK(ctx);
        RadixKeyGen kgp = sa_keygen(R);
        radix_keygen_hash(kgp);
        const bool wide = kgp.hash_ok != 0 && R.K.keygen_hash != 0 && cfg.B <= 8 && R.K.tied_probe != 0;
        u32 pgrid = (u32)ctx->num_cus * 3;
        if (pgrid > tc_cdiv(n, TPK_TILE)) pgrid = tc_cdiv(n, TPK_TILE);
        switch (cfg.s) {
#define TC_PROBE(S) case S: \
            if (wide) tied_probe_w_kernel<S><<<pgrid, TPK_NT, 0, s>>>(R.text, n, kgp, b.tp, b.act[0][0], b.act[0][1], b.act[0][2], d_total, fm); \
            else tied_probe_kernel<S><<<pgrid, TPK_NT, 0, s>>>(R.text, n, kgp, b.tp, b.act[0][0], b.act[0][1], b.act[0][2], d_total, fm); \
            break;
            TC_PROBE(1) TC_PROBE(2) TC_PROBE(3) TC_PROBE(4) TC_PROBE(5) TC_PROBE(6) TC_PROBE(7) TC_PROBE(8)
#undef TC_PROBE
            default: TC_FAIL(ctx, TC_ERR_INTERNAL, "key-only levels: %u symbols per field", cfg.s);
        }
        TC_LAUNCH_CHECK(ctx);
        tc_d2h(ctx, &ctx->h_scalars[SA_SLOT_PROBE], ctx->d_scalars + SA_SLOT_PROBE, sizeof(u64));
        TC_HIP(ctx, hipStreamSynchronize(s));
        ctx->tied_probe_used = wide ? 2 : 1;
        ctx->tied_probe_found = sa_slot_lo(ctx, SA_SLOT_PROBE);
        ok = ctx->tied_probe_found == fm;
    }
    if (R.K.trace)
        fprintf(stderr, "textcomp: key-only levels: %u tied suffixes %s (the pass over the text met %u)\n", fm,
                ok ? "found again in the text" : "-- NOT recoverable: the levels run again with suffix starts", sa_slot_lo(ctx, SA_SLOT_PROBE));
    return ok;
}

static void sa_tier2_fix(SaRun &R, const FinishArgs &fa, u32 &fm, u32 &flags, u32 &fm_dropped) {
    tc_ctx *ctx = R.ctx;
    hipStream_t s = R.stream();
    const u32 fm_lean = fm;
    u32 *flagword = sa_dev_slot(ctx, SA_SLOT_TIED) + 1;
    u32 *ndropped = sa_dev_slot(ctx, SA_SLOT_DROPPED);
    tc_memset_async(ctx, flagword, 0, sizeof(u32));
    tc_memset_async(ctx, ndropped, 0, sizeof(u64));
    tc_memset_async(ctx, fa.ovbits, 0, ((size_t)tc_cdiv(R.N, 64) + 1) * sizeof(u64));
    const u32 fwaves = tc_cdiv(R.N, 64 * FIX_WIN);
    finish_fix_kernel<<<tc_cdiv(fwaves, FIN_NT / 64), FIN_NT, 0, s>>>(fa);
    TC_LAUNCH_CHECK(ctx);
    if (fm_lean) {
        finish_filter_kernel<<<tc_cdiv(fm_lean, 256) < 4096u ? tc_cdiv(fm_lean, 256) : 4096u, 256, 0, s>>>(fa.out_slot, fm_lean, fa.ovbits, ndropped);
        TC_LAUNCH_CHECK(ctx);
    }
    tc_d2h(ctx, &ctx->h_scalars[SA_SLOT_TIED], ctx->d_scalars + SA_SLOT_TIED, 2 * sizeof(u64));
    TC_HIP(ctx, hipStreamSynchronize(s));
    fm = sa_slot_lo(ctx, SA_SLOT_TIED);
    flags = sa_slot_hi(ctx, SA_SLOT_TIED);
    fm_dropped = sa_slot_lo(ctx, SA_SLOT_DROPPED);
}

static void sa_order_tied(SaRun &R, u32 fm, u32 slot_bits) {
    tc_ctx *ctx = R.ctx;
    SaBuffers &b = R.b;
    hipStream_t s = R.stream();
    if (fm <= SEG_W && R.K.tiny != 0) {
        tied_small_kernel<0><<<1, SEG_NT, 0, s>>>(b.act[0][0], b.act[0][1], b.act[0][2], fm, nullptr, nullptr, nullptr);
        TC_LAUNCH_CHECK(ctx);
        return;
    }
    pack_active_kernel<<<tc_cdiv(fm, 256), 256, 0, s>>>(b.act[0][0], b.act[0][2], fm, b.sk[0]);
    TC_LAUNCH_CHECK(ctx);
    TC_HIP(ctx, hipMemcpyAsync(b.sv[0], b.act[0][1], fm * sizeof(u32), hipMemcpyDeviceToDevice, s));
    RadixPlan ps;
    ps.add_range(32, 32 + (int)slot_bits);
    RadixBuffers rs = sa_sparse_buffers(R);
    radix_sort_pairs(ctx, rs, fm, ps, false, false);
    unpack_active_kernel<<<tc_cdiv(fm, 256), 256, 0, s>>>(rs.keys, fm, b.act[0][0], b.act[0][2]);
    TC_LAUNCH_CHECK(ctx);
    TC_HIP(ctx, hipMemcpyAsync(b.act[0][1], rs.vals, fm * sizeof(u32), hipMemcpyDeviceToDevice, s));
}

static void sa_key_round(SaRun &R, u64 *kall) {
    tc_ctx *ctx = R.ctx;
    SaBuffers &b = R.b;
    hipStream_t s = R.stream();
    tc_stats &st = R.st();
    const u32 mm = (u32)R.m;
    key_round_kernel<<<tc_cdiv(mm, 256), 256, 0, s>>>(b.act[0][0], b.act[0][2], kall, mm, b.sk[0], b.sv[0]);
    TC_LAUNCH_CHECK(ctx);
    seg_sort_pairs(ctx, b.seg, b.sk[0], b.sv[0], b.sk[1], b.sv[1], mm, 32);
    key_round_store_kernel<<<tc_cdiv(mm, 256), 256, 0, s>>>(b.sk[0], b.act[0][0], mm, kall);
    TC_LAUNCH_CHECK(ctx);
    GroupArgs gk = {};
    gk.keys = b.sk[0]; gk.count = mm; gk.vals = b.sv[0]; gk.vals_are_idx = 0; gk.norank = 1;
    gk.in_slot = b.act[0][0]; gk.in_idx = b.act[0][1];
    gk.out_slot = b.act[1][0]; gk.out_idx = b.act[1][1]; gk.out_grp = b.act[1][2];
    sa_run_group(R, false, gk);
    const u64 m2 = sa_fetch_m(R);
    for (int q = 0; q < 3; q++)
        if (m2) TC_HIP(ctx, hipMemcpyAsync(b.act[0][q], b.act[1][q], m2 * sizeof(u32), hipMemcpyDeviceToDevice, s));
    st.m[st.rounds] = R.m; st.key_bytes[st.rounds] = 8; st.passes[st.rounds] = 1; st.h[st.rounds] = (u32)R.h_start;
    st.rounds++;
    st.seg_rounds++;
    if (R.K.trace)
        fprintf(stderr, "textcomp: key round: %u members of whole buckets ordered by the key's remaining 32 bits, %llu stay tied\n", mm, (unsigned long long)m2);
    R.m = m2;
    R.h_start = R.cfg.h0;
}

enum Round0Result {
    R0_ACCEPTED,
    R0_GIVE_WAY,
    R0_NEED_STARTS,
};
static Round0Result sa_round0_collect(SaRun &R, Round0Out &o, bool keyround, bool &many_ties) {
    tc_ctx *ctx = R.ctx;
    SaBuffers &b = R.b;
    hipStream_t s = R.stream();
    tc_stats &st = R.st();
    FinishArgs &fa = o.fa;
    u32 *roff = b.fin_rc + FIN_REGIONS * FIN_RSTRIDE;
    finish_regions_kernel<<<1, 64, 0, s>>>(fa.rcount, fa.rcap, roff, fa.counters);
    TC_LAUNCH_CHECK(ctx);
    if (o.msd && o.keyonly)
        finish_compact_kernel<<<1024, 256, 0, s>>>(roff, fa.rcap, b.act[1][0], b.act[1][1], b.act[1][2],
                                                  b.act[0][0], b.act[0][1], b.act[0][2], b.v0, b.act[0][3], (u32)b.sparse_cap);
    else
        finish_compact_kernel<<<1024, 256, 0, s>>>(roff, fa.rcap, b.act[1][0], b.act[1][1], b.act[1][2],
                                                  b.act[0][0], b.act[0][1], b.act[0][2]);
    TC_LAUNCH_CHECK(ctx);
    fa.out_slot = b.act[0][0]; fa.out_idx = b.act[0][1]; fa.out_grp = b.act[0][2];
    tc_d2h(ctx, &ctx->h_scalars[SA_SLOT_TIED], ctx->d_scalars + SA_SLOT_TIED, sizeof(u64));
    TC_HIP(ctx, hipStreamSynchronize(s));
    u32 fm = sa_slot_lo(ctx, SA_SLOT_TIED), over = sa_slot_hi(ctx, SA_SLOT_TIED);
    if (R.K.trace)
        fprintf(stderr, "textcomp: round 0 %s way%s: tied %u, flags 0x%x (1 over-long bucket left to the fix pass, 2 whole buckets tied, 4 bucket above the finish chunk, 8 joint counts off)\n",
                o.msd ? "MSD" : "LSD", o.msd && o.msd_big ? " (big finish)" : "", fm, over);
    if (o.msd && (over & (4u | 8u))) return R0_GIVE_WAY;
    if (o.msd && o.keyonly && !sa_keyonly_recover(R, fm, over)) return R0_NEED_STARTS;
    u32 slot_bits = (u32)R.rbits, fm_dropped = 0;
    if (!o.msd && (over & 1u) && fm <= fa.fix_cap && R.K.tier2 != 0) {
        sa_tier2_fix(R, fa, fm, over, fm_dropped);
        slot_bits = (u32)R.rbits + 1;
    }
    if (o.msd && !o.msd_big && fm > (1u << 18)) return R0_GIVE_WAY;
    if ((over & 1u) || fm > b.sparse_cap - 1024) {
        if (!o.msd && fm > b.sparse_cap - 1024) many_ties = true;
        return R0_GIVE_WAY;
    }
    R.m = fm - fm_dropped;
    if (over & 2u) R.h_start = (u64)(o.tb / (int)R.cfg.w) * R.cfg.s;
    if (o.msd && o.msd_big) {
        R.skeys = o.keys_sorted;
    } else {
        R.tkeys = o.keys;
        R.tkeys_shift = 64 - o.tb;
    }
    st.finish_pass = 1;
    st.rounds = 1;
    st.m[0] = R.N; st.key_bytes[0] = 8; st.passes[0] = (u32)o.npass; st.h[0] = 0;
    if (R.m > 0) sa_order_tied(R, fm, slot_bits);
    if (o.msd && o.msd_big && (over & 2u) && keyround && R.m >= (u64)R.K.seg_min && R.K.seg != 0)
        sa_key_round(R, const_cast<u64 *>(o.keys_sorted));
    return R0_ACCEPTED;
}

static bool sa_round0(SaRun &R, bool &hopeless, bool &many_ties) {
    SaConfig &cfg = R.cfg;
    Round0In in;
    in.entropy = cfg.entropy; in.w = cfg.w; in.s = cfg.s; in.P = cfg.P;
    in.N = R.N;
    in.msd_carved = R.b.msd_pstart[0] != nullptr && msd_wanted(R.N);
    in.want_sa = R.d_sa != nullptr;
    in.sample_dups = 0;
    in.msd_levels = MSD_LEVELS; in.cap_small = MSDF_CAP_SMALL; in.cap_big = MSDF_CAP_BIG;
    in.samp_n = SAMP_N; in.tied_max = TP_MAX_TIED;
    Round0Plan pl;
    sa_round0_depth(in, R.K, pl);
    const bool finish_fits = (int)(cfg.P * cfg.w) - pl.topbits <= 32;
    if (finish_fits && R.n >= (1u << 20) && R.K.sample != 0) {
        sa_sample(R, pl.topbits);
        hopeless = R.st().sample_dups > SAMP_N / 10;
    }
    if (!finish_fits || hopeless) return false;
    in.sample_dups = R.st().sample_dups;
    sa_round0_plan(in, R.K, pl);
    if (pl.P != cfg.P) {
        cfg.P = pl.P;
        cfg.h0 = cfg.P * cfg.s;
        R.h_start = cfg.h0;
    }
    Round0Result res = R0_GIVE_WAY;
    if (pl.try_msd) {
        Round0Out o = sa_round0_msd(R, pl, pl.keyonly);
        res = sa_round0_collect(R, o, pl.keyround, many_ties);
        if (res == R0_NEED_STARTS) {
            o = sa_round0_msd(R, pl, false);
            res = sa_round0_collect(R, o, pl.keyround, many_ties);
        }
    }
    if (res == R0_GIVE_WAY) {
        R.ctx->msd_split_used = 0;
        R.ctx->msd_dir_used = 0;
        Round0Out o = sa_round0_lsd(R, pl);
        res = sa_round0_collect(R, o, pl.keyround, many_ties);
    }
    return res == R0_ACCEPTED;
}

static void sa_full_path(SaRun &R, u32 P_full, bool hopeless, bool many_ties) {
    SaBuffers &b = R.b;
    SaConfig &cfg = R.cfg;
    tc_stats &st = R.st();
    cfg.P = P_full;
    if ((hopeless || st.finish_pass == 0) && R.K.fields == 0 && R.K.deep != 0 && R.K.finish != 0)
        cfg.P = 56 / cfg.w;
    cfg.h0 = cfg.P * cfg.s;
    R.h_start = cfg.h0;
    RadixPlan plan;
    plan.add_range(64 - (int)(cfg.P * cfg.w), 64);
    RadixBuffers rb = sa_build_keys_and_sort(R, plan, false);
    R.skeys = rb.keys;
    GroupArgs g0 = {};
    g0.keys = R.skeys; g0.count = (u32)R.N; g0.vals = R.sa;
    g0.out_slot = b.act[0][0]; g0.out_idx = b.act[0][1]; g0.out_grp = b.act[0][2]; g0.out_tpos = b.act[0][3];
    const bool ties = hopeless || many_ties;
    if (ties) { g0.isa = b.isa; R.isa_ready = true; }
    const bool g0_pairs = ties && R.N >= R.bin_min && R.part_act1_ok;
    if (g0_pairs) g0.pairs = rb.keys_alt;
    sa_run_group(R, true, g0);
    if (g0_pairs) sa_apply_pairs(R, rb.keys_alt, (u32)R.N, R.part_act1);
    R.m = sa_fetch_m(R);
    st.rounds = 1;
    st.m[0] = R.N; st.key_bytes[0] = 8; st.passes[0] = (u32)plan.npass; st.h[0] = 0;
}

static void sa_rank_accel(SaRun &R) {
    tc_ctx *ctx = R.ctx;
    SaBuffers &b = R.b;
    hipStream_t s = R.stream();
    RankLookup &rl = R.rl;
    const u64 N = R.N;
    const u32 nwords = (u32)(N / 64 + 1);
    const u32 nb = tc_cdiv(nwords, BDIR_TILE);
    bitdir_sum_kernel<<<nb, 256, 0, s>>>(b.t_bits, nwords, b.t_bsum);
    TC_LAUNCH_CHECK(ctx);
    bitdir_spine_kernel<<<1, 1024, 0, s>>>(b.t_bsum, nb);
    TC_LAUNCH_CHECK(ctx);
    bitdir_down_kernel<<<nb, 256, 0, s>>>(b.t_bits, nwords, b.t_bsum, b.t_dir);
    TC_LAUNCH_CHECK(ctx);
    rl.t_bits = b.t_bits; rl.t_dir = b.t_dir;
    const u64 *dkeys = R.tkeys ? R.tkeys : ((R.skeys == b.k0 || R.skeys == b.k1) ? R.skeys : nullptr);
    if (!dkeys) return;
    int kb = R.tkeys ? (64 - R.tkeys_shift < SA_KDIR_BITS ? 64 - R.tkeys_shift : SA_KDIR_BITS) : SA_KDIR_BITS;
    while (kb > 16 && (1ull << kb) > N / 16) kb--;
    if (R.K.kdir_search != 0) {
        kdir_build_kernel<<<tc_cdiv((1ull << kb) + 1, 256), 256, 0, s>>>(dkeys, (u32)N, kb, b.kdir);
        TC_LAUNCH_CHECK(ctx);
    } else {
        const u64 entries = (1ull << kb) + 1;
        const u32 nbk = tc_cdiv(entries, KDF_CHUNK);
        u32 *bmin = b.kdir + ((size_t)1 << SA_KDIR_BITS) + 2;
        tc_memset_async(ctx, b.kdir, 0xff, entries * sizeof(u32));
        kdir_mark_kernel<<<tc_cdiv(N, 256), 256, 0, s>>>(dkeys, (u32)N, kb, b.kdir);
        TC_LAUNCH_CHECK(ctx);
        kdir_fill_min_kernel<<<nbk, 256, 0, s>>>(b.kdir, entries, bmin);
        TC_LAUNCH_CHECK(ctx);
        kdir_fill_spine_kernel<<<1, 1024, 0, s>>>(bmin, nbk);
        TC_LAUNCH_CHECK(ctx);
        kdir_fill_apply_kernel<<<nbk, 256, 0, s>>>(b.kdir, entries, bmin);
        TC_LAUNCH_CHECK(ctx);
    }
    rl.kdir = b.kdir; rl.kdir_bits = kb;
}

static void sa_rank_tables(SaRun &R) {
    tc_ctx *ctx = R.ctx;
    SaBuffers &b = R.b;
    hipStream_t s = R.stream();
    RankLookup &rl = R.rl;
    const u64 m = R.m, N = R.N;
    R.dense = m > b.sparse_cap - 1024 || R.K.dense != 0;
    sa_fill(R.cfg, rl);
    rl.text = R.text; rl.n = (u32)R.n; rl.N = (u32)N; rl.h0 = R.cfg.h0;
    if (R.dense && !R.skeys) TC_FAIL(ctx, TC_ERR_INTERNAL, "dense mode needs the sorted keys");
    if (R.dense) {
        if (!R.isa_ready) {
            GroupArgs gi = {};
            gi.keys = R.skeys; gi.count = (u32)N; gi.vals = R.sa;
            gi.isa = b.isa; gi.isa_only = 1;
            u64 *kfree = R.skeys == b.k0 ? b.k1 : b.k0;
            const bool gi_pairs = N >= R.bin_min && R.part_act1_ok && (R.skeys == b.k0 || R.skeys == b.k1);
            if (gi_pairs) gi.pairs = kfree;
            sa_run_group(R, true, gi);
            if (gi_pairs) sa_apply_pairs(R, kfree, (u32)N, R.part_act1);
        }
        rl.isa = b.isa;
        return;
    }
    rl.skeys = R.skeys; rl.tkeys = R.tkeys; rl.tshift = R.tkeys_shift; rl.sa = R.sa; rl.t_idx = b.t_idx; rl.t_rank = b.t_rank; rl.t_n = (u32)m;
    if (m == 0) return;
    const u32 mm = (u32)m;
    if (m <= SEG_W && R.K.tiny != 0) {
        tied_small_kernel<1><<<1, SEG_NT, 0, s>>>(b.act[0][0], b.act[0][1], b.act[0][2], mm, b.t_idx, b.t_rank, b.act[0][3]);
        TC_LAUNCH_CHECK(ctx);
        return;
    }
    widen_u32_kernel<<<tc_cdiv(mm, 256), 256, 0, s>>>(b.act[0][1], b.sk[0], mm);
    TC_LAUNCH_CHECK(ctx);
    RadixPlan pt;
    pt.add_range(0, R.rbits);
    RadixBuffers rt = sa_sparse_buffers(R);
    radix_sort_pairs(ctx, rt, mm, pt, true, false);
    const bool accel = m >= (u64)R.K.accel_min;
    if (accel) tc_memset_async(ctx, b.t_bits, 0, (size_t)(u32)(N / 64 + 1) * sizeof(u64));
    table_build_kernel<<<tc_cdiv(mm, 256), 256, 0, s>>>(rt.keys, rt.vals, b.act[0][2], mm,
                                                       b.t_idx, b.t_rank, b.act[0][3],
                                                       accel ? b.t_bits : nullptr);
    TC_LAUNCH_CHECK(ctx);
    if (accel) sa_rank_accel(R);
}

static void sa_chain_codes(SaRun &R, int cur, u32 mm, u32 hh, u64 *chain_path, u64 *chain_sign, u32 chain_words) {
    tc_ctx *ctx = R.ctx;
    SaBuffers &b = R.b;
    hipStream_t s = R.stream();
    const u64 N = R.N;
    const ChainDims cd = chain_dims(N, hh);
    u64 *pathbits = b.seg.segbits, *signbits = b.seg.ybits;
    u32 *any = b.chain_summ + chain_any_offset();
    tc_memset_async(ctx, b.chain_ref, 0xff, (size_t)N * sizeof(u32));
    chain_ref_kernel<<<tc_cdiv(mm, 256), 256, 0, s>>>(b.act[cur][0], b.act[cur][1], b.act[cur][2], R.rl, mm, hh, b.chain_ref);
    TC_LAUNCH_CHECK(ctx);
    if (R.dense) {
        u32 fgrid = tc_cdiv(chain_words, 4);
        if (fgrid > 16384) fgrid = 16384;
        chain_flags_kernel<<<fgrid, 256, 0, s>>>(b.isa, b.chain_ref, (u32)N, hh, pathbits, signbits, chain_words);
    } else {
        tc_memset_async(ctx, pathbits, 0, (size_t)chain_words * sizeof(u64));
        tc_memset_async(ctx, signbits, 0, (size_t)chain_words * sizeof(u64));
        u32 fgrid = tc_cdiv(mm, 256);
        if (fgrid > 16384) fgrid = 16384;
        chain_flags_members_kernel<<<fgrid, 256, 0, s>>>(b.act[cur][1], b.act[cur][2], R.rl, mm, hh, b.chain_ref, pathbits, signbits);
    }
    TC_LAUNCH_CHECK(ctx);
    TC_HIP(ctx, hipMemcpyAsync(chain_path, pathbits, (size_t)chain_words * sizeof(u64), hipMemcpyDeviceToDevice, s));
    TC_HIP(ctx, hipMemcpyAsync(chain_sign, signbits, (size_t)chain_words * sizeof(u64), hipMemcpyDeviceToDevice, s));
    {
        tc_memset_async(ctx, any, 0, (size_t)cd.nb * sizeof(u32));
        u64 parts = ((u64)cd.bk * cd.h / 64) / 4096 + 1;
        if (parts > 1024) parts = 1024;
        chain_blockany_kernel<<<dim3(cd.nb, (u32)parts), 256, 0, s>>>(chain_path, cd, any);
        TC_LAUNCH_CHECK(ctx);
    }
    const u32 cgrid = (u32)tc_cdiv((u64)cd.nb * cd.h, 256);
    if (cd.nb > 1) {
        chain_scan_a_kernel<<<cgrid, 256, 0, s>>>(chain_path, chain_sign, cd, any, b.chain_summ);
        TC_LAUNCH_CHECK(ctx);
        chain_scan_b_kernel<<<tc_cdiv(cd.h, 256), 256, 0, s>>>(b.chain_summ, cd);
        TC_LAUNCH_CHECK(ctx);
    }
    chain_scan_c_kernel<<<cgrid, 256, 0, s>>>(chain_path, chain_sign, cd, any, b.chain_summ, b.chain_code);
    TC_LAUNCH_CHECK(ctx);
    R.st().chain_rounds++;
    sa_trace_step(R, "chain round: codes", N);
    sa_trace_chain_tables(R, cur, mm, hh, cd, chain_path, chain_sign);
}

static void sa_doubling_round(SaRun &R, ChainPolicy &chain, int &cur, u64 &h) {
    tc_ctx *ctx = R.ctx;
    SaBuffers &b = R.b;
    hipStream_t s = R.stream();
    tc_stats &st = R.st();
    const RankLookup &rl = R.rl;
    const bool dense = R.dense;
    const u64 N = R.N, m = R.m;
    const int rbits = R.rbits;
    const u32 mm = (u32)m;
    const u32 hh = h > N ? (u32)N : (u32)h;
    sa_trace_group_sizes(R, cur, mm);
    u64 *k2 = dense ? b.k0 : b.sk[0], *k2alt = dense ? b.k1 : b.sk[1];
    u32 *kv = dense ? b.v0 : b.sv[0], *kvalt = dense ? b.v2 : b.sv[1];
    RadixPlan p2;
    p2.add_range(0, rbits);
    p2.add_range(32, 32 + rbits);
    RadixPlanDev pd2;
    pd2.npass = p2.npass;
    for (int p = 0; p < p2.npass; p++) { pd2.shift[p] = p2.shift[p]; pd2.mask[p] = p2.mask[p]; }
    const bool seg_round = R.K.seg != 0 && mm >= (u32)R.K.seg_min;
    const bool fuse_hist = mm >= (1u << 20) && !seg_round && chain.keymode == 0;
    const bool vals_idx = dense;
    if (fuse_hist) tc_memset_async(ctx, b.hist, 0, sizeof(u32) * RDX_MAX_PASSES * RDX_BINS);
    const u32 chain_words = (u32)(N / 64 + 1);
    u64 *chain_path = reinterpret_cast<u64 *>(b.chain_ref), *chain_sign = chain_path + chain_words;
    if (chain.start(seg_round, hh, h, N, m)) sa_chain_codes(R, cur, mm, hh, chain_path, chain_sign, chain_words);
    const int keymode = chain.keymode;
    if (keymode == 1) {
        chain_key1_kernel<<<tc_cdiv(mm, 256), 256, 0, s>>>(b.act[cur][1], b.act[cur][2], chain_path, chain_sign, b.chain_code, mm, k2, vals_idx ? kv : nullptr);
    } else if (keymode == 2) {
        u32 kgrid = tc_cdiv(mm, 256);
        if (kgrid > 65536) kgrid = 65536;
        chain_key2_kernel<<<kgrid, 256, 0, s>>>(b.act[cur][1], b.act[cur][2], chain_path, chain_sign, b.chain_code, rl, mm, hh, k2, vals_idx ? kv : nullptr);
    } else {
        u32 kgrid = fuse_hist ? tc_cdiv(mm, 256 * 8) : tc_cdiv(mm, 256);
        if (fuse_hist && kgrid > 8192) kgrid = 8192;
        if (!fuse_hist && !vals_idx && !rl.isa && !rl.skeys && rl.tkeys && mm <= 65536u) kgrid = tc_cdiv(mm, 4);
        if (fuse_hist) key2_kernel<true><<<kgrid, 256, 0, s>>>(b.act[cur][1], b.act[cur][2], rl, mm, hh, k2, vals_idx ? kv : nullptr, pd2, b.hist);
        else key2_kernel<false><<<kgrid, 256, 0, s>>>(b.act[cur][1], b.act[cur][2], rl, mm, hh, k2, vals_idx ? kv : nullptr, pd2, b.hist);
    }
    TC_LAUNCH_CHECK(ctx);
    sa_trace_step(R, "round: keys (rank lookups)", mm);
    RadixBuffers r2 = sa_radix_buffers(R, k2, k2alt, kv, kvalt);
    if (seg_round) {
        if (!vals_idx) {
            seg_iota_kernel<<<tc_cdiv(mm, 256), 256, 0, s>>>(kv, mm);
            TC_LAUNCH_CHECK(ctx);
        }
        seg_sort_pairs(ctx, b.seg, k2, kv, k2alt, kvalt, mm, keymode == 1 ? 32 : rbits);
        st.seg_rounds++;
    } else {
        radix_sort_pairs(ctx, r2, mm, p2, !vals_idx, fuse_hist);
    }
    sa_trace_step(R, seg_round ? "round: segmented sort" : "round: radix passes", mm);
    GroupArgs gr = {};
    gr.keys = r2.keys; gr.count = mm; gr.vals = r2.vals; gr.vals_are_idx = vals_idx ? 1 : 0;
    gr.in_slot = b.act[cur][0]; gr.in_idx = b.act[cur][1]; gr.in_tpos = b.act[cur][3];
    gr.isa = dense ? b.isa : nullptr; gr.t_rank = dense ? nullptr : b.t_rank;
    gr.out_slot = b.act[cur ^ 1][0]; gr.out_idx = b.act[cur ^ 1][1];
    gr.out_grp = b.act[cur ^ 1][2]; gr.out_tpos = b.act[cur ^ 1][3];
    const bool gr_pairs = dense && mm >= R.bin_min;
    if (gr_pairs) gr.pairs = r2.keys_alt;
    sa_run_group(R, false, gr);
    if (gr_pairs) sa_apply_pairs(R, r2.keys_alt, mm, r2.keys);
    if (keymode != 2) {
        st.m[st.rounds] = m; st.key_bytes[st.rounds] = 8; st.passes[st.rounds] = seg_round ? 1u : (u32)p2.npass;
        st.h[st.rounds] = hh;
        st.rounds++;
    } else {
        st.passes[st.rounds - 1]++;
    }
    R.m = sa_fetch_m(R);
    sa_trace_step(R, "round: groups", mm);
    cur ^= 1;
    if (chain.finish(mm, R.m)) h *= 2;
}

static void sa_run(tc_ctx *ctx, SaBuffers &b, const u8 *d_text, u64 n, u32 *d_sa, u8 *d_L,
                   u64 *primary, u32 *counts256_out) {
    const u64 N = n + 1;
    hipStream_t s = ctx->stream;
    tc_stats &st = ctx->stats;
    SaRun R{ctx, b, d_text, n, N, ceil_log2_u64(N), d_sa, d_sa ? d_sa : b.v1, d_L, SaKnobs{}};
    R.rshift = R.rbits > 8 ? R.rbits - 8 : 0;
    R.bin_min = 1ull << R.K.bin_min_log2;
    R.part_act1 = reinterpret_cast<u64 *>(b.act[1][0]);
    R.part_act1_ok = (size_t)((char *)b.act[1][2] - (char *)b.act[1][0]) >= N * sizeof(u64) &&
                     ((uintptr_t)b.act[1][0] & 7) == 0;
    sa_trace_buffers(R);
    ctx->msd_split_used = 0;
    ctx->msd_dir_used = 0;
    ctx->tied_probe_used = 0;
    ctx->tied_probe_found = 0;
    if (sa_alphabet(R, counts256_out, primary)) return;

    const u32 P_full = R.cfg.P;
    R.h_start = R.cfg.h0;
    bool hopeless = false;
    bool many_ties = false;
    tc_memset_async(ctx, ctx->d_scalars, 0, 16 * sizeof(u64));
    const bool fast = R.K.finish != 0 && R.K.dense == 0 && sa_round0(R, hopeless, many_ties);
    if (!fast) sa_full_path(R, P_full, hopeless, many_ties);

    R.trace_t0 = std::chrono::steady_clock::now();
    sa_trace_step(R, "(sync before the rank table)", R.m);
    sa_rank_tables(R);
    sa_trace_step(R, R.dense ? "ranks: dense ISA" : "ranks: sparse table", R.m);

    if (R.K.h_start > 0) R.h_start = (u64)R.K.h_start;
    ChainPolicy chain(R.K.chain);
    int cur = 0;
    u64 h = R.h_start;
    while (R.m > 0) {
        if (st.rounds >= TC_MAX_ROUNDS) TC_FAIL(ctx, TC_ERR_INTERNAL, "suffix sort did not converge");
        sa_doubling_round(R, chain, cur, h);
    }
    primary_kernel<<<1, 64, 0, s>>>(R.rl, ctx->d_scalars);
    TC_LAUNCH_CHECK(ctx);
    tc_d2h(ctx, ctx->h_scalars, ctx->d_scalars, sizeof(u64));
    TC_HIP(ctx, hipStreamSynchronize(s));
    *primary = ctx->h_scalars[SA_SLOT_PRIMARY];
    st.sigma = R.cfg.sigma_text + 1;
    st.radix_launches = 0;
    st.ms_radix = 0;
    for (int i = 0; i < ctx->pev_used; i++) {
        float ms = 0;
        if (hipEventElapsedTime(&ms, ctx->pev[2 * i], ctx->pev[2 * i + 1]) == hipSuccess) {
            st.ms_radix += ms;
            st.radix_launches++;
        }
    }
}
```

text-compression_amd/csrc/tc_sa_plan.hpp:

```cpp
#pragma once
#include <math.h>
#include <stdint.h>

struct SaKnobs {
    int trace = env_int("TC_SA_TRACE", 0);
    int fields = env_int("TC_SA_FIELDS", 0);
    int bin_min_log2 = env_int("TC_SA_BIN_MIN_LOG2", 25);
    int kb_onehist = env_int("TC_KB_ONEHIST", 1);
    int keygen_fused = env_int("TC_KEYGEN_FUSED", 1);
    int xcd_group = env_int("TC_XCD_GROUP", 1);
    int finish = env_int("TC_SA_FINISH", 1);
    int dense = env_int("TC_SA_DENSE", 0);
    int global_passes = env_int("TC_SA_GLOBAL_PASSES", 0);
    int sample = env_int("TC_SA_SAMPLE", 1);
    int msd = env_int("TC_SA_MSD", 1);
    int msd_big = env_int("TC_SA_MSD_BIG", 0);
    int msd_max_dups = env_int("TC_SA_MSD_MAX_DUPS", 8);
    int keyround = env_int("TC_SA_KEYROUND", 1);
    int msd_keyonly = env_int("TC_SA_MSD_KEYONLY", 1);
    int keygen_hash = env_int("TC_KEYGEN_HASH", 1);
    int msd_grid = env_int("TC_MSD_GRID", 0);
    int msd_joint = env_int("TC_SA_MSD_JOINT", 1);
    int msd_split = env_int("TC_MSD_SPLIT", 1);
    int msd_dir = env_int("TC_MSD_DIR", 1);
    int tied_probe = env_int("TC_TIED_PROBE", 1);
    int msd_finish_lut = env_int("TC_MSD_FINISH_LUT", 1);
    int msd_finish_ko = env_int("TC_MSD_FINISH_KO", 1);
    int tier2 = env_int("TC_SA_TIER2", 1);
    int tiny = env_int("TC_SA_TINY", 1);
    int seg = env_int("TC_SA_SEG", 1);
    int seg_min = env_int("TC_SA_SEG_MIN", 1 << 16);
    int deep = env_int("TC_SA_DEEP", 1);
    int accel_min = env_int("TC_SA_ACCEL_MIN", 1 << 20);
    int kdir_search = env_int("TC_SA_KDIR_SEARCH", 0);
    int h_start = env_int("TC_SA_H_START", 0);
    int chain = env_int("TC_SA_CHAIN", 1);
};

struct Round0In {
    double entropy;
    uint32_t w, s, P;
    uint64_t N;
    bool msd_carved;
    bool want_sa;
    uint32_t sample_dups;
    int msd_levels;
    uint32_t cap_small, cap_big;
    uint32_t samp_n, tied_max;
};
struct Round0Plan {
    int G, topbits;
    bool msd_cand;
    uint32_t P;
    bool try_msd, msd_big, keyonly, keyround;
};

static inline void sa_round0_depth(const Round0In &in, const SaKnobs &K, Round0Plan &pl) {
    const int keybits = (int)(in.P * in.w);
    double e8 = in.w == 8 ? in.entropy * in.s : in.entropy * 8.0 / in.w;
    int G = e8 > 1e-9 ? (int)ceil((log2((double)in.N) - 4.0) / e8) : 64;
    if (G < (keybits - 32 + 7) / 8) G = (keybits - 32 + 7) / 8;
    if (G < 1) G = 1;
    if (K.global_passes > 0) G = K.global_passes;
    pl.msd_cand = in.w == 8 && in.msd_carved && K.fields == 0 && K.global_passes == 0;
    if (pl.msd_cand && G < in.msd_levels) G = in.msd_levels;
    pl.G = G;
    pl.topbits = 8 * G < keybits ? 8 * G : keybits;
    pl.P = in.P;
}

static inline void sa_round0_plan(const Round0In &in, const SaKnobs &K, Round0Plan &pl) {
    if (K.fields == 0) {
        uint32_t pf = (uint32_t)((pl.topbits + 32) / (int)in.w);
        if (pf > 56 / in.w) pf = 56 / in.w;
        if (pf > pl.P) pl.P = pf;
    }
    const double field_bits = in.entropy * in.s < 8.0 ? in.entropy * in.s : 8.0;
    const double lvl_bits = field_bits * in.msd_levels;
    const double msd_bucket = (double)in.N / exp2(lvl_bits);
    pl.msd_big = msd_bucket > (double)in.cap_small / 3.0 || K.msd_big != 0;
    const bool msd_fits = msd_bucket <= (double)in.cap_big * 0.8;
    const double iid_dups = (double)in.samp_n * in.samp_n / 2.0 / exp2(field_bits * (pl.topbits / 8));
    const bool msd_iid = (double)in.sample_dups <= (double)K.msd_max_dups + 3.0 * iid_dups;
    pl.keyround = K.keyround != 0;
    pl.try_msd = pl.msd_cand && pl.P == 7 &&
                 (K.msd == 2 || (msd_fits && (msd_iid || (pl.msd_big && pl.keyround && K.msd == 3))));
    const double tied_est = (double)in.N * (double)in.N / exp2(in.entropy * (double)(pl.P * in.s));
    pl.keyonly = !in.want_sa && (tied_est < (double)in.tied_max / 4.0 || K.msd_keyonly == 2) && K.msd_keyonly != 0;
}

struct ChainPolicy {
    int mode;
    int keymode = 0;
    uint64_t prev_mm = 0;
    int chain_fail = 0, chain_wait = 0;
    uint64_t chain_m0 = 0;

    explicit ChainPolicy(int mode_) : mode(mode_) {}

    bool start(bool seg_round, uint32_t hh, uint64_t h, uint64_t N, uint64_t m) {
        if (keymode != 0 || !seg_round || hh < 4 || h >= N || mode == 0) return false;
        if (mode != 2 && !(m >= (1u << 20) && prev_mm > 0 && (prev_mm - m) * 256 < prev_mm && chain_wait == 0 && chain_fail < 3))
            return false;
        keymode = 1;
        chain_m0 = m;
        return true;
    }
    bool finish(uint64_t m, uint64_t m_left) {
        if (keymode == 1) {
            keymode = 2;
            return false;
        }
        if (keymode == 2) {
            if ((chain_m0 - m_left) * 8 < chain_m0) chain_wait = 1 << ++chain_fail;
        } else if (chain_wait > 0) chain_wait--;
        prev_mm = keymode == 2 ? 0 : m;
        keymode = 0;
        return true;
    }
};
```

text-compression_amd/csrc/textcomp.hip:

```cpp
#include "tc_common.hpp"
#include "tc_encode_host.hpp"
#include "tc_decode_host.hpp"
#include "tc_ws_host.hpp"
#include "tc_fm_host.hpp"
#include "tc_lcp_host.hpp"
#include "tc_lz_host.hpp"
#include "tc_rep_host.hpp"
#include "tc_kmer_host.hpp"
#include "tc_tm_host.hpp"
#include "tc_container_host.hpp"
#include "tc_hostio_host.hpp"
#include "tc_generate.hpp"
#include "tc_dbg_host.hpp"
#include "tc_comm.hpp"
#include "textcomp_debug.h"

#define TC_API_BEGIN(ctx)                                  \
    if (!(ctx)) return TC_ERR_ARG;                         \
    try {                                                  \
        if (hipSetDevice((ctx)->device) != hipSuccess) {   \
            (ctx)->err = "hipSetDevice failed";            \
            return TC_ERR_HIP;                             \
        }
#define TC_API_END(ctx)                                    \
        return TC_OK;                                      \
    } catch (const TcFail &f) {                            \
        (void)hipGetLastError();                           \
        return f.code;                                     \
    } catch (...) {                                        \
        (ctx)->err = "unexpected exception";               \
        return TC_ERR_INTERNAL;                            \
    }

extern "C" {

const char *tc_version(void) { return "textcomp-amd 0.1 (gfx950)"; }

int tc_ctx_create(int device, tc_ctx **out) {
    if (!out) return TC_ERR_ARG;
    *out = nullptr;
    int count = 0;
    if (hipGetDeviceCount(&count) != hipSuccess || count <= 0) {
        (void)hipGetLastError();
        return TC_ERR_HIP;
    }
    if (device < 0 || device >= count) return TC_ERR_ARG;
    tc_ctx *ctx = new tc_ctx();
    ctx->device = device;
    try {
        TC_HIP(ctx, hipSetDevice(device));
        {
            hipDeviceProp_t prop;
            TC_HIP(ctx, hipGetDeviceProperties(&prop, device));
            ctx->num_cus = prop.multiProcessorCount;
        }
        TC_HIP(ctx, hipStreamCreateWithFlags(&ctx->stream, hipStreamNonBlocking));
        TC_HIP(ctx, hipMalloc((void **)&ctx->d_err, 256));
        TC_HIP(ctx, hipMalloc((void **)&ctx->d_scalars, 128 * sizeof(u64)));
        TC_HIP(ctx, hipHostMalloc((void **)&ctx->h_scalars, 64 * sizeof(u64), hipHostMallocDefault));
        TC_HIP(ctx, hipHostMalloc((void **)&ctx->h_hdr, 1024, hipHostMallocDefault));
        TC_HIP(ctx, hipMemsetAsync(ctx->d_err, 0, 256, ctx->stream));
        TC_HIP(ctx, hipMemsetAsync(ctx->d_scalars, 0, 128 * sizeof(u64), ctx->stream));
        for (int i = 0; i < 8; i++) TC_HIP(ctx, hipEventCreate(&ctx->ev[i]));
        for (int i = 0; i < 32; i++) TC_HIP(ctx, hipEventCreate(&ctx->pev[i]));
        TC_HIP(ctx, hipStreamSynchronize(ctx->stream));
    } catch (const TcFail &f) {
        int code = f.code;
        tc_ctx_destroy(ctx);
        return code;
    }
    *out = ctx;
    return TC_OK;
}

void tc_ctx_destroy(tc_ctx *ctx) {
    if (!ctx) return;
    (void)hipSetDevice(ctx->device);
    if (ctx->stream) (void)hipStreamSynchronize(ctx->stream);
    for (int i = 0; i < 8; i++)
        if (ctx->ev[i]) (void)hipEventDestroy(ctx->ev[i]);
    for (int i = 0; i < 32; i++)
        if (ctx->pev[i]) (void)hipEventDestroy(ctx->pev[i]);
    hp_release(ctx);
    tc_ws_release(ctx);
    if (ctx->d_err) (void)hipFree(ctx->d_err);
    if (ctx->d_scalars) (void)hipFree(ctx->d_scalars);
    if (ctx->h_scalars) (void)hipHostFree(ctx->h_scalars);
    if (ctx->h_hdr) (void)hipHostFree(ctx->h_hdr);
    if (ctx->stream) (void)hipStreamDestroy(ctx->stream);
    delete ctx;
}

const char *tc_last_error(const tc_ctx *ctx) { return ctx ? ctx->err.c_str() : "null ctx"; }

int tc_get_stats(const tc_ctx *ctx, tc_stats *out) {
    if (!ctx || !out) return TC_ERR_ARG;
    *out = ctx->stats;
    out->ws_chunks = (uint32_t)ctx->ws_chunks.size();
    out->ws_grown = ctx->stats_ws_grown;
    return TC_OK;
}

void *tc_ctx_stream(const tc_ctx *ctx) { return ctx ? (void *)ctx->stream : nullptr; }

int tc_ctx_place_workspace(tc_ctx *ctx, const uint8_t *d_text, uint64_t n, tc_block *out, int tries, double *ms,
                           int *chosen) {
    TC_API_BEGIN(ctx)
    ws_place_entry(ctx, d_text, n, out, tries, ms, chosen);
    TC_API_END(ctx)
}

int tc_ctx_set_profile(tc_ctx *ctx, int on) {
    if (!ctx) return TC_ERR_ARG;
    ctx->profile = on ? 1 : 0;
    return TC_OK;
}

int tc_ctx_set_container_coding(tc_ctx *ctx, int coding) {
    if (!ctx) return TC_ERR_ARG;
    if (coding != TC_CODING_PACKED && coding != TC_CODING_HUFFMAN) {
        ctx->err = "unknown container coding";
        return TC_ERR_ARG;
    }
    ctx->coding = coding;
    return TC_OK;
}

int tc_ctx_get_container_coding(const tc_ctx *ctx) { return ctx ? ctx->coding : TC_ERR_ARG; }

int tc_bwt_encode_dev(tc_ctx *ctx, const uint8_t *d_text, uint64_t n, uint8_t *d_L,
                      uint64_t *primary) {
    TC_API_BEGIN(ctx)
    bwt_encode_entry(ctx, d_text, n, d_L, primary, true);
    TC_API_END(ctx)
}

int tc_bwt_encode(tc_ctx *ctx, const uint8_t *text, uint64_t n, uint8_t *L, uint64_t *primary) {
    TC_API_BEGIN(ctx)
    bwt_encode_entry(ctx, text, n, L, primary, false);
    TC_API_END(ctx)
}

int tc_suffix_array(tc_ctx *ctx, const uint8_t *text, uint64_t n, uint32_t *sa) {
    TC_API_BEGIN(ctx)
    suffix_array_entry(ctx, text, n, sa);
    TC_API_END(ctx)
}

int tc_suffix_array_dev(tc_ctx *ctx, const uint8_t *d_text, uint64_t n, uint32_t *d_sa) {
    TC_API_BEGIN(ctx)
    suffix_array_dev_entry(ctx, d_text, n, d_sa);
    TC_API_END(ctx)
}

int tc_lcp_array_dev(tc_ctx *ctx, const uint8_t *d_text, uint64_t n, const uint32_t *d_sa, uint32_t *d_lcp) {
    TC_API_BEGIN(ctx)
    lcp_array_dev_entry(ctx, d_text, n, d_sa, d_lcp);
    TC_API_END(ctx)
}

int tc_lcp_array(tc_ctx *ctx, const uint8_t *text, uint64_t n, uint32_t *sa, uint32_t *lcp) {
    TC_API_BEGIN(ctx)
    lcp_array_host_entry(ctx, text, n, sa, lcp);
    TC_API_END(ctx)
}

int tc_lcp_summary_dev(tc_ctx *ctx, const uint32_t *d_lcp, uint64_t N, uint32_t *max_lcp, uint64_t *row, uint64_t *sum) {
    TC_API_BEGIN(ctx)
    lcp_summary_entry(ctx, d_lcp, N, max_lcp, row, sum);
    TC_API_END(ctx)
}

int tc_lpf_array(tc_ctx *ctx, const uint8_t *text, uint64_t n, uint32_t *lpf, uint32_t *src) {
    TC_API_BEGIN(ctx)
    lpf_array_entry(ctx, text, n, lpf, src, false);
    TC_API_END(ctx)
}

int tc_lpf_array_dev(tc_ctx *ctx, const uint8_t *d_text, uint64_t n, uint32_t *d_lpf, uint32_t *d_src) {
    TC_API_BEGIN(ctx)
    lpf_array_entry(ctx, d_text, n, d_lpf, d_src, true);
    TC_API_END(ctx)
}

int tc_lz_parse(tc_ctx *ctx, const uint8_t *text, uint64_t n, uint32_t *ph_src, uint32_t *ph_len, uint64_t *nph) {
    TC_API_BEGIN(ctx)
    lz_parse_entry(ctx, text, n, ph_src, ph_len, nph, false);
    TC_API_END(ctx)
}

int tc_lz_parse_dev(tc_ctx *ctx, const uint8_t *d_text, uint64_t n, uint32_t *d_ph_src, uint32_t *d_ph_len, uint64_t *nph) {
    TC_API_BEGIN(ctx)
    lz_parse_entry(ctx, d_text, n, d_ph_src, d_ph_len, nph, true);
    TC_API_END(ctx)
}

int tc_lz_unparse(tc_ctx *ctx, const uint32_t *ph_src, const uint32_t *ph_len, uint64_t nph, uint8_t *text, uint64_t *nbytes) {
    TC_API_BEGIN(ctx)
    lz_unparse_entry(ctx, ph_src, ph_len, nph, text, nbytes, false);
    TC_API_END(ctx)
}

int tc_lz_unparse_dev(tc_ctx *ctx, const uint32_t *d_ph_src, const uint32_t *d_ph_len, uint64_t nph, uint8_t *d_text,
                      uint64_t *nbytes) {
    TC_API_BEGIN(ctx)
    lz_unparse_entry(ctx, d_ph_src, d_ph_len, nph, d_text, nbytes, true);
    TC_API_END(ctx)
}

int tc_repeats(tc_ctx *ctx, const uint8_t *text, uint64_t n, int kind, uint32_t min_len, uint32_t min_occ, uint32_t *sa,
               uint32_t *rep_pos, uint32_t *rep_len, uint32_t *rep_occ, uint32_t *rep_row, uint64_t *nrep) {
    TC_API_BEGIN(ctx)
    repeats_entry(ctx, text, n, kind, min_len, min_occ, sa, rep_pos, rep_len, rep_occ, rep_row, nrep, false);
    TC_API_END(ctx)
}

int tc_repeats_dev(tc_ctx *ctx, const uint8_t *d_text, uint64_t n, int kind, uint32_t min_len, uint32_t min_occ, uint32_t *d_sa,
                   uint32_t *d_rep_pos, uint32_t *d_rep_len, uint32_t *d_rep_occ, uint32_t *d_rep_row, uint64_t *nrep) {
    TC_API_BEGIN(ctx)
    repeats_entry(ctx, d_text, n, kind, min_len, min_occ, d_sa, d_rep_pos, d_rep_len, d_rep_occ, d_rep_row, nrep, true);
    TC_API_END(ctx)
}

int tc_kmers(tc_ctx *ctx, const uint8_t *text, uint64_t n, uint32_t k, uint32_t min_occ, uint32_t max_occ, uint32_t *sa,
             uint32_t *kmer_pos, uint32_t *kmer_occ, uint32_t *kmer_row, uint64_t *nk) {
    TC_API_BEGIN(ctx)
    kmers_entry(ctx, text, n, k, min_occ, max_occ, sa, kmer_pos, kmer_occ, kmer_row, nk, false);
    TC_API_END(ctx)
}

int tc_kmers_dev(tc_ctx *ctx, const uint8_t *d_text, uint64_t n, uint32_t k, uint32_t min_occ, uint32_t max_occ, uint32_t *d_sa,
                 uint32_t *d_kmer_pos, uint32_t *d_kmer_occ, uint32_t *d_kmer_row, uint64_t *nk) {
    TC_API_BEGIN(ctx)
    kmers_entry(ctx, d_text, n, k, min_occ, max_occ, d_sa, d_kmer_pos, d_kmer_occ, d_kmer_row, nk, true);
    TC_API_END(ctx)
}

int tc_kmers_esa_dev(tc_ctx *ctx, const uint32_t *d_sa, const uint32_t *d_lcp, uint64_t N, uint32_t k, uint32_t min_occ,
                     uint32_t max_occ, uint32_t *d_kmer_pos, uint32_t *d_kmer_occ, uint32_t *d_kmer_row, uint64_t *nk) {
    TC_API_BEGIN(ctx)
    kmers_esa_entry(ctx, d_sa, d_lcp, N, k, min_occ, max_occ, d_kmer_pos, d_kmer_occ, d_kmer_row, nk);
    TC_API_END(ctx)
}

int tc_kmer_spectrum(tc_ctx *ctx, const uint8_t *text, uint64_t n, uint32_t k, uint32_t bins, uint64_t *hist, uint64_t *distinct,
                     uint64_t *total) {
    TC_API_BEGIN(ctx)
    kmer_spectrum_entry(ctx, text, n, k, bins, hist, distinct, total);
    TC_API_END(ctx)
}

int tc_kmer_spectrum_esa_dev(tc_ctx *ctx, const uint32_t *d_sa, const uint32_t *d_lcp, uint64_t N, uint32_t k, uint32_t bins,
                             uint64_t *d_hist, uint64_t *distinct, uint64_t *total) {
    TC_API_BEGIN(ctx)
    kmer_spectrum_esa_entry(ctx, d_sa, d_lcp, N, k, bins, d_hist, distinct, total);
    TC_API_END(ctx)
}

int tc_kmer_profile(tc_ctx *ctx, const uint8_t *text, uint64_t n, uint32_t kmax, uint64_t *distinct, uint64_t *unique) {
    TC_API_BEGIN(ctx)
    kmer_profile_entry(ctx, text, n, kmax, distinct, unique);
    TC_API_END(ctx)
}

int tc_kmer_profile_esa_dev(tc_ctx *ctx, const uint32_t *d_lcp, uint64_t N, uint32_t kmax, uint64_t *distinct, uint64_t *unique) {
    TC_API_BEGIN(ctx)
    kmer_profile_esa_entry(ctx, d_lcp, N, kmax, distinct, unique);
    TC_API_END(ctx)
}

int tc_text_match_stats(tc_ctx *ctx, const uint8_t *query, uint64_t a, const uint8_t *target, uint64_t b, uint32_t *ms_len,
                        uint32_t *ms_pos, uint32_t *ms_occ) {
    TC_API_BEGIN(ctx)
    text_match_stats_entry(ctx, query, a, target, b, ms_len, ms_pos, ms_occ, false);
    TC_API_END(ctx)
// ... 40 lines not shown
    mems_from_stats_entry(ctx, d_ms_len, d_ms_pos, a, min_len, d_mem_start, d_mem_pos, d_mem_len, nmem);
    TC_API_END(ctx)
}

int tc_mtf_encode(tc_ctx *ctx, const uint8_t *L, uint64_t N, int64_t primary, uint16_t *idx,
                  int16_t *final_list, uint32_t *sigma) {
    TC_API_BEGIN(ctx)
    mtf_encode_entry(ctx, L, N, primary, idx, final_list, sigma);
    TC_API_END(ctx)
}

int tc_mtf_encode_sym(tc_ctx *ctx, const int16_t *sym, uint64_t N, uint16_t *idx,
                      int16_t *final_list, uint32_t *sigma) {
    TC_API_BEGIN(ctx)
    mtf_encode_sym_entry(ctx, sym, N, idx, final_list, sigma);
    TC_API_END(ctx)
}

int tc_rle_encode(tc_ctx *ctx, const uint8_t *L, uint64_t N, int64_t primary, uint32_t *counts,
                  int16_t *syms, uint64_t *nruns) {
    TC_API_BEGIN(ctx)
    rle_encode_entry(ctx, L, N, primary, counts, syms, nruns);
    TC_API_END(ctx)
}

int tc_rle_encode_sym(tc_ctx *ctx, const int16_t *sym, uint64_t N, uint32_t *counts,
                      int16_t *syms, uint64_t *nruns) {
    TC_API_BEGIN(ctx)
    rle_encode_vals_entry<SymAcc, i16>(ctx, sym, N, counts, syms, nruns);
    TC_API_END(ctx)
}

int tc_rle_encode_u16(tc_ctx *ctx, const uint16_t *vals, uint64_t N, uint32_t *counts,
                      uint16_t *run_vals, uint64_t *nruns) {
    TC_API_BEGIN(ctx)
    rle_encode_vals_entry<U16Acc, u16>(ctx, vals, N, counts, run_vals, nruns);
    TC_API_END(ctx)
}

int tc_encode_dev(tc_ctx *ctx, const uint8_t *d_text, uint64_t n, tc_block *out) {
    TC_API_BEGIN(ctx)
    encode_entry(ctx, d_text, n, out, true);
    TC_API_END(ctx)
}

int tc_encode(tc_ctx *ctx, const uint8_t *text, uint64_t n, tc_block *out) {
    TC_API_BEGIN(ctx)
    encode_entry(ctx, text, n, out, false);
    TC_API_END(ctx)
}

int tc_generate_dev(tc_ctx *ctx, int kind, uint64_t seed, uint64_t n, uint8_t *d_out) {
    TC_API_BEGIN(ctx)
    generate_entry(ctx, kind, seed, n, d_out);
    TC_API_END(ctx)
}

int tc_bwt_decode(tc_ctx *ctx, const uint8_t *L, uint64_t N, uint64_t primary, uint8_t *text) {
    TC_API_BEGIN(ctx)
    bwt_decode_entry(ctx, L, N, primary, text);
    TC_API_END(ctx)
}

int tc_bwt_decode_sym(tc_ctx *ctx, const int16_t *sym, uint64_t N, uint8_t *text, uint64_t *n_out) {
    TC_API_BEGIN(ctx)
    bwt_decode_sym_entry(ctx, sym, N, text, n_out);
    TC_API_END(ctx)
}

int tc_mtf_decode(tc_ctx *ctx, const uint16_t *idx, uint64_t N, const int16_t *list,
                  uint32_t nlist, int16_t *sym) {
    TC_API_BEGIN(ctx)
    mtf_decode_entry(ctx, idx, N, list, nlist, sym);
    TC_API_END(ctx)
}

int tc_rle_decode(tc_ctx *ctx, const uint32_t *counts, const int16_t *syms, uint64_t nruns,
                  int16_t *sym_out, uint64_t *N) {
    TC_API_BEGIN(ctx)
    rle_decode_entry<i16>(ctx, counts, syms, nruns, sym_out, N);
    TC_API_END(ctx)
}

int tc_rle_decode_u16(tc_ctx *ctx, const uint32_t *counts, const uint16_t *run_vals,
                      uint64_t nruns, uint16_t *vals_out, uint64_t *N) {
    TC_API_BEGIN(ctx)
    rle_decode_entry<u16>(ctx, counts, run_vals, nruns, vals_out, N);
    TC_API_END(ctx)
}

int tc_decode_dev(tc_ctx *ctx, const tc_block *blk, uint8_t *d_text) {
    TC_API_BEGIN(ctx)
    decode_entry(ctx, blk, d_text, true);
    TC_API_END(ctx)
}

int tc_decode(tc_ctx *ctx, const tc_block *blk, uint8_t *text) {
    TC_API_BEGIN(ctx)
    decode_entry(ctx, blk, text, false);
    TC_API_END(ctx)
}

uint64_t tc_block_packed_bound(uint64_t nruns, uint32_t sigma) {
    const int fmt = pack_format(sigma);
    if (fmt == 0) return nruns + 16 * ((nruns + PK_TILE - 1) / PK_TILE + 1) + 4 * nruns;
    return (((u64)fmt * nruns + 7) & ~7ull) + 8 * nruns + 8;
}

int tc_block_pack_dev(tc_ctx *ctx, const tc_block *blk, uint8_t *d_packed, uint64_t *packed_bytes,
                      uint64_t *nesc) {
    TC_API_BEGIN(ctx)
    block_pack_device(ctx, blk, d_packed, packed_bytes, nesc);
    TC_API_END(ctx)
}

int tc_block_unpack_dev(tc_ctx *ctx, const uint8_t *d_packed, uint64_t packed_bytes, uint64_t nruns,
                        uint32_t sigma, uint64_t nesc, tc_block *blk) {
    TC_API_BEGIN(ctx)
    block_unpack_device(ctx, d_packed, packed_bytes, nruns, sigma, nesc, blk);
    TC_API_END(ctx)
}

uint64_t tc_container_bound(uint64_t nruns, uint32_t sigma) {
    return TC_CONTAINER_HEADER + tc_block_packed_bound(nruns, sigma);
}

int tc_encode_container_dev(tc_ctx *ctx, const uint8_t *d_text, uint64_t n, uint8_t *d_out, uint64_t *bytes) {
    TC_API_BEGIN(ctx)
    encode_container_dev_entry(ctx, d_text, n, d_out, bytes);
    TC_API_END(ctx)
}

int tc_block_to_container_dev(tc_ctx *ctx, const tc_block *blk, uint8_t *d_out, uint64_t *bytes) {
    TC_API_BEGIN(ctx)
    container_write_device(ctx, blk, d_out, bytes);
    TC_API_END(ctx)
}

int tc_container_to_block_dev(tc_ctx *ctx, const uint8_t *d_in, uint64_t bytes, tc_block *blk) {
    TC_API_BEGIN(ctx)
    container_read_device(ctx, d_in, bytes, blk);
    TC_API_END(ctx)
}

int tc_container_info(tc_ctx *ctx, const uint8_t *container, uint64_t bytes, uint64_t *n, uint64_t *nruns) {
    if (!ctx) return TC_ERR_ARG;
    try {
        if (!container || bytes < TC_CONTAINER_HEADER) TC_FAIL(ctx, TC_ERR_MALFORMED, "container shorter than its header");
        const ContainerHeader h = container_header_parse(ctx, container, bytes, HDR_MAGIC);
        if (n) *n = h.n;
        if (nruns) *nruns = h.nruns;
        return TC_OK;
    } catch (const TcFail &f) {
        return f.code;
    }
}

int tc_container_coding(tc_ctx *ctx, const uint8_t *container, uint64_t bytes, int *coding) {
    if (!ctx) return TC_ERR_ARG;
    try {
        if (!coding) TC_FAIL(ctx, TC_ERR_ARG, "bad argument");
        if (!container || bytes < TC_CONTAINER_HEADER) TC_FAIL(ctx, TC_ERR_MALFORMED, "container shorter than its header");
        const ContainerHeader h = container_header_parse(ctx, container, bytes, HDR_MAGIC);
        if (h.format == HF_FORMAT) *coding = TC_CODING_HUFFMAN;
        else if (h.sigma <= TC_MAX_SIGMA && h.format == (u32)pack_format(h.sigma)) *coding = TC_CODING_PACKED;
        else TC_FAIL(ctx, TC_ERR_MALFORMED, "container header names no known body format");
        return TC_OK;
    } catch (const TcFail &f) {
        return f.code;
    }
}

int tc_encode_container(tc_ctx *ctx, const uint8_t *text, uint64_t n, uint8_t *out, uint64_t *bytes) {
    TC_API_BEGIN(ctx)
    encode_container_entry(ctx, text, n, out, bytes);
    TC_API_END(ctx)
}

int tc_decode_container(tc_ctx *ctx, const uint8_t *container, uint64_t bytes, uint8_t *text, uint64_t *n_out) {
    TC_API_BEGIN(ctx)
    decode_container_entry(ctx, container, bytes, text, n_out);
    TC_API_END(ctx)
}

uint64_t tc_stream_bound(uint64_t n, uint64_t block_bytes) {
    if (block_bytes == 0) block_bytes = TC_STREAM_BLOCK_DEFAULT;
    if (block_bytes > TC_MAX_N) block_bytes = TC_MAX_N;
    const u64 nb = stream_blocks(n, block_bytes);
    const u64 last = n - (nb - 1) * block_bytes;
    return (nb - 1) * container_bound_any(block_bytes) + container_bound_any(last);
}

int tc_encode_stream(tc_ctx *ctx, const uint8_t *text, uint64_t n, uint64_t block_bytes, uint8_t *out,
                     uint64_t *bytes) {
    TC_API_BEGIN(ctx)
    encode_stream_entry(ctx, text, n, block_bytes, out, bytes);
    TC_API_END(ctx)
}

int tc_stream_info(tc_ctx *ctx, const uint8_t *stream, uint64_t bytes, uint64_t *n_total, uint64_t *nblocks) {
    if (!ctx) return TC_ERR_ARG;
    try {
        const StreamIndex ix = stream_index(ctx, stream, bytes);
        if (n_total) *n_total = ix.n_total;
        if (nblocks) *nblocks = ix.off.size();
        return TC_OK;
    } catch (const TcFail &f) {
        return f.code;
    }
}

int tc_decode_stream(tc_ctx *ctx, const uint8_t *stream, uint64_t bytes, uint8_t *text, uint64_t *n_out) {
    TC_API_BEGIN(ctx)
    decode_stream_entry(ctx, stream, bytes, text, n_out);
    TC_API_END(ctx)
}

int tc_fm_build(tc_ctx *ctx, const uint8_t *text, uint64_t n, tc_fm **out) {
    TC_API_BEGIN(ctx)
    fm_build_entry(ctx, text, nullptr, n, 1, 0, 0, out);
    TC_API_END(ctx)
}

int tc_fm_build_dev(tc_ctx *ctx, const uint8_t *d_text, uint64_t n, tc_fm **out) {
    TC_API_BEGIN(ctx)
    fm_build_entry(ctx, nullptr, d_text, n, 1, 0, 0, out);
    TC_API_END(ctx)
}

int tc_fm_build_sampled(tc_ctx *ctx, const uint8_t *text, uint64_t n, uint32_t sa_rate, tc_fm **out) {
    TC_API_BEGIN(ctx)
    fm_build_entry(ctx, text, nullptr, n, sa_rate, 0, 1, out);
    TC_API_END(ctx)
}

int tc_fm_build_sampled_dev(tc_ctx *ctx, const uint8_t *d_text, uint64_t n, uint32_t sa_rate, tc_fm **out) {
    TC_API_BEGIN(ctx)
    fm_build_entry(ctx, nullptr, d_text, n, sa_rate, 0, 1, out);
    TC_API_END(ctx)
}

int tc_fm_build_self(tc_ctx *ctx, const uint8_t *text, uint64_t n, uint32_t sa_rate, uint32_t text_rate, tc_fm **out) {
    TC_API_BEGIN(ctx)
    fm_build_entry(ctx, text, nullptr, n, sa_rate, text_rate, 2, out);
    TC_API_END(ctx)
}

int tc_fm_build_self_dev(tc_ctx *ctx, const uint8_t *d_text, uint64_t n, uint32_t sa_rate, uint32_t text_rate, tc_fm **out) {
    TC_API_BEGIN(ctx)
    fm_build_entry(ctx, nullptr, d_text, n, sa_rate, text_rate, 2, out);
    TC_API_END(ctx)
}

int tc_fm_build_lcp(tc_ctx *ctx, const uint8_t *text, uint64_t n, uint32_t sa_rate, uint32_t text_rate, tc_fm **out) {
    TC_API_BEGIN(ctx)
    fm_build_entry(ctx, text, nullptr, n, sa_rate, text_rate, 2, out, true);
    TC_API_END(ctx)
}

int tc_fm_build_lcp_dev(tc_ctx *ctx, const uint8_t *d_text, uint64_t n, uint32_t sa_rate, uint32_t text_rate, tc_fm **out) {
    TC_API_BEGIN(ctx)
    fm_build_entry(ctx, nullptr, d_text, n, sa_rate, text_rate, 2, out, true);
    TC_API_END(ctx)
}

int tc_fm_has_lcp(const tc_fm *fm) { return fm && fm->d_lcp ? 1 : 0; }
uint32_t tc_fm_sa_rate(const tc_fm *fm) { return fm ? fm->sa_rate : 0; }
uint32_t tc_fm_text_rate(const tc_fm *fm) { return fm ? fm->text_rate : 0; }
uint64_t tc_fm_device_bytes(const tc_fm *fm, int part) { return fm_device_bytes(fm, part); }
void tc_fm_free(tc_fm *fm) { fm_release(fm); }

uint64_t tc_fm_export_bound(const tc_fm *fm, int with_locate) { return fm_export_bound(fm, with_locate); }

int tc_fm_export_dev(tc_ctx *ctx, const tc_fm *fm, int with_locate, uint8_t *d_out, uint64_t *bytes) {
    TC_API_BEGIN(ctx)
    fm_export_device(ctx, fm, with_locate, d_out, bytes);
    TC_API_END(ctx)
}

int tc_fm_import_dev(tc_ctx *ctx, const uint8_t *d_in, uint64_t bytes, tc_fm **out) {
    TC_API_BEGIN(ctx)
    fm_import_device(ctx, d_in, bytes, out);
    TC_API_END(ctx)
}

int tc_fm_count_dev(tc_ctx *ctx, const tc_fm *fm, const uint8_t *d_pats, const uint64_t *d_offs,
                    uint64_t npat, int64_t *d_out) {
    TC_API_BEGIN(ctx)
    fm_count_entry(ctx, fm, d_pats, d_offs, npat, true, 0, d_out, true);
    TC_API_END(ctx)
}

int tc_fm_count(tc_ctx *ctx, const tc_fm *fm, const uint8_t *pats, const uint64_t *offs,
                uint64_t npat, int64_t *out) {
    TC_API_BEGIN(ctx)
    fm_count_entry(ctx, fm, pats, offs, npat, true, 0, out, false);
    TC_API_END(ctx)
}

int tc_fm_locate(tc_ctx *ctx, const tc_fm *fm, const uint8_t *pats, const uint64_t *offs,
                 uint64_t npat, uint64_t *hit_offs, uint64_t *hits, uint64_t *nhits) {
    TC_API_BEGIN(ctx)
    fm_locate_entry(ctx, fm, pats, offs, npat, true, 0, hit_offs, hits, nullptr, nhits, false);
    TC_API_END(ctx)
}

int tc_fm_locate_dev(tc_ctx *ctx, const tc_fm *fm, const uint8_t *d_pats, const uint64_t *d_offs,
                     uint64_t npat, uint64_t *d_hit_offs, uint64_t *d_hits, uint64_t *nhits) {
    TC_API_BEGIN(ctx)
    fm_locate_entry(ctx, fm, d_pats, d_offs, npat, true, 0, d_hit_offs, d_hits, nullptr, nhits, true);
    TC_API_END(ctx)
}

int tc_fm_count_mm_dev(tc_ctx *ctx, const tc_fm *fm, const uint8_t *d_pats, const uint64_t *d_offs, uint64_t npat, uint32_t k,
                       int64_t *d_out) {
    TC_API_BEGIN(ctx)
    fm_count_entry(ctx, fm, d_pats, d_offs, npat, false, k, d_out, true);
    TC_API_END(ctx)
}

int tc_fm_count_mm(tc_ctx *ctx, const tc_fm *fm, const uint8_t *pats, const uint64_t *offs, uint64_t npat, uint32_t k,
                   int64_t *out) {
    TC_API_BEGIN(ctx)
    fm_count_entry(ctx, fm, pats, offs, npat, false, k, out, false);
    TC_API_END(ctx)
}

int tc_fm_locate_mm(tc_ctx *ctx, const tc_fm *fm, const uint8_t *pats, const uint64_t *offs, uint64_t npat, uint32_t k,
                    uint64_t *hit_offs, uint64_t *hits, uint8_t *hit_mm, uint64_t *nhits) {
    TC_API_BEGIN(ctx)
    fm_locate_entry(ctx, fm, pats, offs, npat, false, k, hit_offs, hits, hit_mm, nhits, false);
    TC_API_END(ctx)
}

int tc_fm_locate_mm_dev(tc_ctx *ctx, const tc_fm *fm, const uint8_t *d_pats, const uint64_t *d_offs, uint64_t npat, uint32_t k,
                        uint64_t *d_hit_offs, uint64_t *d_hits, uint8_t *d_hit_mm, uint64_t *nhits) {
    TC_API_BEGIN(ctx)
    fm_locate_entry(ctx, fm, d_pats, d_offs, npat, false, k, d_hit_offs, d_hits, d_hit_mm, nhits, true);
    TC_API_END(ctx)
}

int tc_fm_extract_dev(tc_ctx *ctx, const tc_fm *fm, const uint64_t *d_starts, const uint64_t *d_lens, uint64_t nq,
                      uint64_t *d_out_offs, uint8_t *d_out, uint64_t *nbytes) {
    TC_API_BEGIN(ctx)
    fm_extract_entry(ctx, fm, d_starts, d_lens, nq, d_out_offs, d_out, nbytes, true);
    TC_API_END(ctx)
}

int tc_fm_extract(tc_ctx *ctx, const tc_fm *fm, const uint64_t *starts, const uint64_t *lens, uint64_t nq,
                  uint64_t *out_offs, uint8_t *out, uint64_t *nbytes) {
    TC_API_BEGIN(ctx)
    fm_extract_entry(ctx, fm, starts, lens, nq, out_offs, out, nbytes, false);
    TC_API_END(ctx)
}

int tc_fm_factorize(tc_ctx *ctx, const tc_fm *fm, const uint8_t *pats, const uint64_t *offs, uint64_t npat, uint64_t *fac_offs,
                    uint64_t *fac_pos, uint32_t *fac_len, uint64_t *nfac) {
    TC_API_BEGIN(ctx)
    fm_factor_entry(ctx, fm, pats, offs, npat, fac_offs, fac_pos, fac_len, nfac, false);
    TC_API_END(ctx)
}

int tc_fm_factorize_dev(tc_ctx *ctx, const tc_fm *fm, const uint8_t *d_pats, const uint64_t *d_offs, uint64_t npat,
                        uint64_t *d_fac_offs, uint64_t *d_fac_pos, uint32_t *d_fac_len, uint64_t *nfac) {
    TC_API_BEGIN(ctx)
    fm_factor_entry(ctx, fm, d_pats, d_offs, npat, d_fac_offs, d_fac_pos, d_fac_len, nfac, true);
    TC_API_END(ctx)
}

int tc_fm_unfactorize(tc_ctx *ctx, const tc_fm *fm, const uint64_t *fac_offs, const uint64_t *fac_pos, const uint32_t *fac_len,
                      uint64_t npat, uint64_t *out_offs, uint8_t *out, uint64_t *nbytes) {
    TC_API_BEGIN(ctx)
    fm_unfactor_entry(ctx, fm, fac_offs, fac_pos, fac_len, npat, out_offs, out, nbytes, false);
    TC_API_END(ctx)
}

int tc_fm_unfactorize_dev(tc_ctx *ctx, const tc_fm *fm, const uint64_t *d_fac_offs, const uint64_t *d_fac_pos,
                          const uint32_t *d_fac_len, uint64_t npat, uint64_t *d_out_offs, uint8_t *d_out, uint64_t *nbytes) {
    TC_API_BEGIN(ctx)
    fm_unfactor_entry(ctx, fm, d_fac_offs, d_fac_pos, d_fac_len, npat, d_out_offs, d_out, nbytes, true);
    TC_API_END(ctx)
}

int tc_fm_match_stats(tc_ctx *ctx, const tc_fm *fm, const uint8_t *pats, const uint64_t *offs, uint64_t npat, uint32_t *ms_len,
                      uint64_t *ms_pos, uint32_t *ms_occ) {
    TC_API_BEGIN(ctx)
    fm_match_stats_entry(ctx, fm, pats, offs, npat, ms_len, ms_pos, ms_occ, false);
    TC_API_END(ctx)
}

int tc_fm_match_stats_dev(tc_ctx *ctx, const tc_fm *fm, const uint8_t *d_pats, const uint64_t *d_offs, uint64_t npat,
                          uint32_t *d_ms_len, uint64_t *d_ms_pos, uint32_t *d_ms_occ) {
    TC_API_BEGIN(ctx)
    fm_match_stats_entry(ctx, fm, d_pats, d_offs, npat, d_ms_len, d_ms_pos, d_ms_occ, true);
    TC_API_END(ctx)
}

int tc_fm_mems(tc_ctx *ctx, const tc_fm *fm, const uint8_t *pats, const uint64_t *offs, uint64_t npat, uint32_t min_len,
               uint64_t *mem_offs, uint64_t *mem_start, uint64_t *mem_pos, uint32_t *mem_len, uint64_t *nmem) {
    TC_API_BEGIN(ctx)
    fm_mems_entry(ctx, fm, pats, offs, npat, min_len, mem_offs, mem_start, mem_pos, mem_len, nmem, false);
    TC_API_END(ctx)
}

int tc_fm_mems_dev(tc_ctx *ctx, const tc_fm *fm, const uint8_t *d_pats, const uint64_t *d_offs, uint64_t npat, uint32_t min_len,
                   uint64_t *d_mem_offs, uint64_t *d_mem_start, uint64_t *d_mem_pos, uint32_t *d_mem_len, uint64_t *nmem) {
    TC_API_BEGIN(ctx)
    fm_mems_entry(ctx, fm, d_pats, d_offs, npat, min_len, d_mem_offs, d_mem_start, d_mem_pos, d_mem_len, nmem, true);
    TC_API_END(ctx)
}

int tc_fm_info(const tc_fm *fm, uint64_t *N, uint32_t *sigma, int16_t *c_sym, uint64_t *c_val,
               uint64_t *primary) {
    return fm_info(fm, N, sigma, c_sym, c_val, primary);
}

int tc_comm_unique_id(tc_ctx *ctx, uint8_t *id) {
    TC_API_BEGIN(ctx)
    comm_unique_id_entry(ctx, id);
    TC_API_END(ctx)
}

int tc_comm_create(tc_ctx *ctx, const uint8_t *id, int rank, int world, tc_comm **out) {
    TC_API_BEGIN(ctx)
    comm_create_entry(ctx, id, rank, world, out);
    TC_API_END(ctx)
}

void tc_comm_destroy(tc_comm *comm) { comm_destroy_entry(comm); }

int tc_comm_reserved_cus(const tc_comm *comm) { return comm ? comm->cus : 0; }

int tc_comm_wait(tc_comm *c) {
    if (!c) return TC_ERR_ARG;
    tc_ctx *ctx = c->ctx;
    TC_API_BEGIN(ctx)
    comm_wait_entry(ctx, c);
    TC_API_END(ctx)
}

int tc_comm_gather(tc_comm *c, int root, const uint8_t *d_container, uint64_t bytes, uint8_t *d_recv,
                   uint64_t slot_bytes, uint64_t *sizes) {
    if (!c) return TC_ERR_ARG;
    tc_ctx *ctx = c->ctx;
    TC_API_BEGIN(ctx)
    comm_gather_entry(ctx, c, root, d_container, bytes, d_recv, slot_bytes, sizes);
    TC_API_END(ctx)
}

int tc_comm_broadcast(tc_comm *c, int root, uint8_t *d_buf, uint64_t bytes) {
    if (!c) return TC_ERR_ARG;
    tc_ctx *ctx = c->ctx;
    TC_API_BEGIN(ctx)
    comm_broadcast_entry(ctx, c, root, d_buf, bytes);
    TC_API_END(ctx)
}

int tc_dbg_checksum64_dev(tc_ctx *ctx, const void *d_p, uint64_t bytes, uint64_t *out) {
    TC_API_BEGIN(ctx)
    dbg_checksum64_entry(ctx, d_p, bytes, out);
    TC_API_END(ctx)
}

int tc_dbg_stream_bench(tc_ctx *ctx, uint64_t bytes, int width, int mode, int iters, double *gbps) {
    TC_API_BEGIN(ctx)
    dbg_stream_bench_entry(ctx, bytes, width, mode, iters, gbps);
    TC_API_END(ctx)
}

int tc_dbg_scatter_bench(tc_ctx *ctx, uint64_t n, uint32_t bins, uint32_t xrun, int iters, double *ms_per_pass) {
    TC_API_BEGIN(ctx)
    dbg_scatter_bench_entry(ctx, n, bins, xrun, iters, ms_per_pass);
    TC_API_END(ctx)
}

int tc_dbg_lcp_set_short_cap(tc_ctx *ctx, uint32_t cap) {
    if (!ctx) return TC_ERR_ARG;
    if (cap != 0 && (cap < 16 || cap > 65536 || cap % 16 != 0)) {
        ctx->err = "the short cap is a multiple of 16 in 16 .. 65536, or 0";
        return TC_ERR_ARG;
    }
    ctx->lcp_cap = cap;
    return TC_OK;
}

int tc_dbg_fm_set_lcp_fanout(tc_ctx *ctx, uint32_t fanout) {
    if (!ctx) return TC_ERR_ARG;
    if (fanout != 4 && fanout != 8 && fanout != 16 && fanout != 64) {
        ctx->err = "the fan-out of the LCP min tree is 4, 8, 16 or 64";
        return TC_ERR_ARG;
    }
    ctx->fm_lcp_fanout = fanout;
    return TC_OK;
}

int tc_dbg_lz_set_tile(tc_ctx *ctx, uint32_t tile) {
    if (!ctx) return TC_ERR_ARG;
    if (tile != 0 && (tile < 64 || tile > LZ_TILE_MAX || (tile & (tile - 1)) != 0)) {
        ctx->err = "the tile of the LZ77 parse is a power of two in 64 .. 16384, or 0";
        return TC_ERR_ARG;
    }
    ctx->lz_tile = tile;
    return TC_OK;
}

int tc_dbg_msd_split_used(tc_ctx *ctx, uint32_t *used) {
    if (!ctx || !used) return TC_ERR_ARG;
    *used = ctx->msd_split_used ? 1u : 0u;
    return TC_OK;
}

int tc_dbg_msd_dir(tc_ctx *ctx, uint32_t out[2]) {
    TC_API_BEGIN(ctx)
    if (!out) TC_FAIL(ctx, TC_ERR_ARG, "out is null");
    sa_dbg_msd_dir(ctx, out);
    TC_API_END(ctx)
}

int tc_dbg_tied_probe(tc_ctx *ctx, uint32_t out[2]) {
    if (!ctx || !out) return TC_ERR_ARG;
    out[0] = (uint32_t)ctx->tied_probe_used;
    out[1] = ctx->tied_probe_found;
    return TC_OK;
}

int tc_dbg_ibwt_walk(tc_ctx *ctx, uint32_t out[3]) {
    if (!ctx || !out) return TC_ERR_ARG;
    out[0] = ctx->ibwt_attempts;
    out[1] = ctx->ibwt_overflowed;
    out[2] = ctx->ibwt_extra_taken;
    return TC_OK;
}

int tc_dbg_dispatch_probe(tc_ctx *ctx, uint32_t grid, uint32_t lds_bytes, uint32_t spin_cycles, uint32_t *out6) {
    TC_API_BEGIN(ctx)
    dbg_dispatch_probe_entry(ctx, grid, lds_bytes, spin_cycles, out6);
    TC_API_END(ctx)
}

int tc_dbg_sort_bench(tc_ctx *ctx, uint64_t n, int key_bits, int iters, int check, double *ms_per_pass) {
    TC_API_BEGIN(ctx)
    dbg_sort_bench_entry(ctx, n, key_bits, iters, check, ms_per_pass);
    TC_API_END(ctx)
}

int tc_dbg_seg_sort(tc_ctx *ctx, uint64_t *keys, uint32_t *vals, uint32_t m, int rbits, uint32_t levels[16]) {
    TC_API_BEGIN(ctx)
    dbg_seg_sort_entry(ctx, keys, vals, m, rbits, levels);
    TC_API_END(ctx)
}

int tc_dbg_tied_small(tc_ctx *ctx, int mode, uint32_t *slot, uint32_t *idx, uint32_t *grp, uint32_t m, uint32_t *t_idx,
                      uint32_t *t_rank, uint32_t *tpos) {
    TC_API_BEGIN(ctx)
    dbg_tied_small_entry(ctx, mode, slot, idx, grp, m, t_idx, t_rank, tpos);
    TC_API_END(ctx)
}

}
```

Measured before the change: 58790 MB/s.

## Reuse last sort's alphabet to fuse census, level-1 MSD count and sample

Measured after the change: 57720 MB/s. -1.8%, worse.

```diff
diff --git a/include/textcomp_debug.h b/include/textcomp_debug.h
--- a/include/textcomp_debug.h
+++ b/include/textcomp_debug.h
@@ -15,6 +15,7 @@
 int tc_dbg_msd_split_used(tc_ctx *ctx, uint32_t *used);
 int tc_dbg_msd_dir(tc_ctx *ctx, uint32_t out[2]);
 int tc_dbg_tied_probe(tc_ctx *ctx, uint32_t out[2]);
+int tc_dbg_census(tc_ctx *ctx, uint32_t out[3]);
 int tc_dbg_ibwt_walk(tc_ctx *ctx, uint32_t out[3]);
 int tc_dbg_seg_sort(tc_ctx *ctx, uint64_t *keys, uint32_t *vals, uint32_t m, int rbits, uint32_t levels[16]);
 int tc_dbg_tied_small(tc_ctx *ctx, int mode, uint32_t *slot, uint32_t *idx, uint32_t *grp, uint32_t m,
diff --git a/text-compression_amd/csrc/tc_common.hpp b/text-compression_amd/csrc/tc_common.hpp
--- a/text-compression_amd/csrc/tc_common.hpp
+++ b/text-compression_amd/csrc/tc_common.hpp
@@ -47,6 +47,13 @@
     int msd_split_used = 0;
     int tied_probe_used = 0;
     u32 tied_probe_found = 0;
+    struct CensusMemo {
+        int valid = 0;
+        u16 lut[256];
+        u32 B = 0, s = 0, w = 0;
+        int topbits = 0;
+    } census_memo;
+    u32 census_state = 0, census_level1 = 0, census_sample = 0;
     u32 ibwt_attempts = 0, ibwt_overflowed = 0, ibwt_extra_taken = 0;
     int mtf_fastin_failed = 0;
     int live_comms = 0;
diff --git a/text-compression_amd/csrc/tc_msd.hpp b/text-compression_amd/csrc/tc_msd.hpp
--- a/text-compression_amd/csrc/tc_msd.hpp
+++ b/text-compression_amd/csrc/tc_msd.hpp
@@ -195,16 +195,28 @@
     u8 row[256];
     u8 dig[128];
 };
-template <bool TEXT, bool JOINT, bool HI>
+struct MsdCensus {
+    u32 G;
+    u32 blo, bhi;
+    u32 *foreign;
+    u32 *lds;
+};
+#define MSD_CENSUS_LDS_WORDS (256 + 128 + 4)
+template <bool TEXT, bool JOINT, bool HI, bool CENSUS = false>
 __device__ __forceinline__ void msd_count_body(const MsdLevel &L, const u64 *__restrict__ keys,
                                                const MsdTextDigit &td, u32 *__restrict__ joint_out,
-                                               const MsdJointRows &jr) {
+                                               const MsdJointRows &jr, const MsdCensus *cs = nullptr) {
     static_assert(!HI || (!TEXT && JOINT), "the high halves serve the joint count of keys only");
-    __shared__ u32 s_cnt[256];
-    __shared__ u16 s_lut[TEXT ? 256 : 1];
-    __shared__ u32 s_seg[4];
+    static_assert(!CENSUS || (TEXT && !JOINT), "the census is the count of level 1");
+    __shared__ u32 s_cnt_own[CENSUS ? 1 : 256];
+    __shared__ u16 s_lut_own[TEXT && !CENSUS ? 256 : 1];
+    __shared__ u32 s_seg_own[CENSUS ? 1 : 4];
     __shared__ u32 s_joint[JOINT ? 32768 : 1];
-    const u32 tid = threadIdx.x, G = gridDim.x, b = msd_logical_wg(blockIdx.x, G);
+    u32 *const s_cnt = CENSUS ? cs->lds : s_cnt_own;
+    u16 *const s_lut = CENSUS ? reinterpret_cast<u16 *>(cs->lds + 256) : s_lut_own;
+    u32 *const s_seg = CENSUS ? cs->lds + 256 + 128 : s_seg_own;
+    const u32 tid = threadIdx.x, G = CENSUS ? cs->G : gridDim.x, b = msd_logical_wg(blockIdx.x, G);
+    u32 bad = 0;
     if (tid < 256) s_cnt[tid] = 0;
     if (TEXT && tid < 256) s_lut[tid] = td.lut[tid];
     __shared__ u8 s_row[JOINT ? 256 : 1];
@@ -248,13 +260,19 @@
                     if (td.hash_ok) {
 #pragma unroll
                         for (int q = 0; q < 5; q++) {
-                            const u32 y = __builtin_amdgcn_perm(td.thi, td.tlo, (x[q] >> td.hsh) & 0x07070707u);
+                            const u32 sel = (x[q] >> td.hsh) & 0x07070707u;
+                            const u32 y = __builtin_amdgcn_perm(td.thi, td.tlo, sel);
 #pragma unroll
                             for (int j = 0; j < 4; j++) cd[4 * q + j] = (y >> (8 * j)) & 255u;
+                            if (CENSUS && q < 4) bad |= __builtin_amdgcn_perm(cs->bhi, cs->blo, sel) ^ x[q];
                         }
                     } else {
 #pragma unroll
                         for (int j = 0; j < 20; j++) cd[j] = s_lut[(x[j >> 2] >> (8 * (j & 3))) & 255u];
+                        if (CENSUS) {
+#pragma unroll
+                            for (int k = 0; k < 16; k++) bad |= cd[k] == 0 ? 1u : 0u;
+                        }
                     }
 #pragma unroll
                     for (int k = 0; k < 16; k++) {
@@ -281,7 +299,11 @@
             for (u64 i0 = (u64)p + tid; i0 < hi; i0 += MSD_NT) {
                 u64 i = i0;
                 u32 g = 0;
-                for (u32 j = 0; j < td.s; j++, i++) g = g * td.B + (i < td.n ? (u32)s_lut[td.text[i]] : 0u);
+                for (u32 j = 0; j < td.s; j++, i++) {
+                    const u32 c = i < td.n ? (u32)s_lut[td.text[i]] : 0u;
+                    if (CENSUS && j == 0 && i < td.n && c == 0) bad = 1;
+                    g = g * td.B + c;
+                }
                 atomicAdd(&s_cnt[g], 1u);
             }
         } else {
@@ -343,6 +365,7 @@
             s_cnt[tid] = 0;
         }
     }
+    if (CENSUS && bad) atomicOr(cs->foreign, 1u);
 }
 template <bool TEXT, bool JOINT>
 __global__ __launch_bounds__(MSD_NT) void msd_count_kernel(MsdLevel L, const u64 *__restrict__ keys,
@@ -354,6 +377,20 @@
                                                               MsdTextDigit td, u32 *__restrict__ joint_out,
                                                               MsdJointRows jr) {
     msd_count_body<false, true, true>(L, reinterpret_cast<const u64 *>(khi), td, joint_out, jr);
+}
+__global__ __launch_bounds__(MSD_NT) void msd_census_kernel(MsdLevel L, MsdTextDigit td, u32 G, u32 blo, u32 bhi,
+                                                            u32 *foreign, u32 w, int topbits, u32 *sample_out) {
+    static_assert(MSD_NT == 1024, "sample_dup_body is written for 1024 threads");
+    static_assert(SAMP_LDS_WORDS >= MSD_CENSUS_LDS_WORDS, "the sample's LDS holds the count's");
+    __shared__ __attribute__((aligned(16))) u32 s_mem[SAMP_LDS_WORDS];
+    if (blockIdx.x >= G) {
+        sample_dup_body(td.text, td.n, td.lut, td.B, w, td.s, topbits, sample_out, s_mem,
+                        reinterpret_cast<u16 *>(s_mem + SAMP_SLOTS), s_mem + SAMP_SLOTS + 128);
+        return;
+    }
+    const MsdCensus cs = {G, blo, bhi, foreign, s_mem};
+    MsdJointRows jr;
+    msd_count_body<true, false, false, true>(L, nullptr, td, nullptr, jr, &cs);
 }
 
 __global__ __launch_bounds__(256) void msd_scan_kernel(MsdLevel L, u32 G, u32 *maxchild) {
diff --git a/text-compression_amd/csrc/tc_sa.hpp b/text-compression_amd/csrc/tc_sa.hpp
--- a/text-compression_amd/csrc/tc_sa.hpp
+++ b/text-compression_amd/csrc/tc_sa.hpp
@@ -525,19 +525,18 @@
 
 #define SAMP_N 8192
 #define SAMP_SLOTS 16384
-__global__ __launch_bounds__(1024) void sample_dup_kernel(const u8 *__restrict__ text, u32 n, RadixKeyGen kg,
-                                                           int topbits, u32 *out) {
-    __shared__ u32 table[SAMP_SLOTS];
-    __shared__ u16 s_lut[256];
-    __shared__ u32 s_dups;
+#define SAMP_LDS_WORDS (SAMP_SLOTS + 128 + 1)
+__device__ __forceinline__ void sample_dup_body(const u8 *__restrict__ text, u32 n, const u16 *lut, u32 B, u32 w, u32 s,
+                                                int topbits, u32 *out, u32 *table, u16 *s_lut, u32 *s_dups_p) {
+    u32 &s_dups = *s_dups_p;
     for (int i = threadIdx.x; i < SAMP_SLOTS; i += 1024) table[i] = 0xFFFFFFFFu;
-    if (threadIdx.x < 256) s_lut[threadIdx.x] = kg.lut[threadIdx.x];
+    if (threadIdx.x < 256) s_lut[threadIdx.x] = lut[threadIdx.x];
     if (threadIdx.x == 0) s_dups = 0;
     __syncthreads();
     u32 dups = 0;
-    const u32 nf = ((u32)topbits + kg.w - 1) / kg.w;
+    const u32 nf = ((u32)topbits + w - 1) / w;
     constexpr int SPT = SAMP_N / 1024;
-    const bool words = nf * kg.s <= 16;
+    const bool words = nf * s <= 16;
     u32 tw[SPT][4];
     u64 qs[SPT];
 #pragma unroll
@@ -558,25 +557,26 @@
     for (int j = 0; j < SPT; j++) {
         u64 q = qs[j];
         const bool in = words && q + 16 <= n;
+        const u32 w0 = tw[j][0], w1 = tw[j][1], w2 = tw[j][2], w3 = tw[j][3];
         u64 key = 0;
         int sh = 64;
         u32 pos = 0;
         for (u32 f = 0; f < nf; f++) {
             u32 g = 0;
-            for (u32 t = 0; t < kg.s; t++, q++, pos++) {
+            for (u32 t = 0; t < s; t++, q++, pos++) {
                 u32 c;
                 if (in) {
-                    u32 wsel = tw[j][0];
-                    wsel = (pos >> 2) == 1 ? tw[j][1] : wsel;
-                    wsel = (pos >> 2) == 2 ? tw[j][2] : wsel;
-                    wsel = (pos >> 2) == 3 ? tw[j][3] : wsel;
+                    u32 wsel = w0;
+                    wsel = (pos >> 2) == 1 ? w1 : wsel;
+                    wsel = (pos >> 2) == 2 ? w2 : wsel;
+                    wsel = (pos >> 2) == 3 ? w3 : wsel;
                     c = (u32)s_lut[(wsel >> (8 * (pos & 3))) & 255u];
                 } else {
                     c = q < n ? (u32)s_lut[text[q]] : 0u;
                 }
-                g = g * kg.B + c;
-            }
-            sh -= kg.w;
+                g = g * B + c;
+            }
+            sh -= w;
             key |= (u64)g << sh;
         }
         u64 kt = key >> (64 - topbits);
@@ -595,6 +595,13 @@
     if (lane_id() == 0 && dups) atomicAdd(&s_dups, dups);
     __syncthreads();
     if (threadIdx.x == 0) *out = s_dups;
+}
+__global__ __launch_bounds__(1024) void sample_dup_kernel(const u8 *__restrict__ text, u32 n, RadixKeyGen kg,
+                                                           int topbits, u32 *out) {
+    __shared__ u32 table[SAMP_SLOTS];
+    __shared__ u16 s_lut[256];
+    __shared__ u32 s_dups;
+    sample_dup_body(text, n, kg.lut, kg.B, kg.w, kg.s, topbits, out, table, s_lut, &s_dups);
 }
 
 struct FinishArgs {
diff --git a/text-compression_amd/csrc/tc_sa_host.hpp b/text-compression_amd/csrc/tc_sa_host.hpp
--- a/text-compression_amd/csrc/tc_sa_host.hpp
+++ b/text-compression_amd/csrc/tc_sa_host.hpp
@@ -112,12 +112,14 @@
     SA_SLOT_DROPPED = 13,
     SA_SLOT_SAMPLE = 14,
     SA_SLOT_MAXCHILD = 15,
+    SA_SLOT_CENSUS = 16,
     SA_SLOT_SEG = 24,
     SA_SLOT_ERR = 62,
     SA_SLOT_MSD_PROF = 64,
     SA_SLOT_MSDK_PROF = 112,
     SA_SLOT_MSD_DIR = 122,
 };
+static const int SA_HOST_CENSUS = 64;
 static inline u32 sa_slot_lo(const tc_ctx *ctx, int slot) { return (u32)(ctx->h_scalars[slot] & 0xffffffffu); }
 static inline u32 sa_slot_hi(const tc_ctx *ctx, int slot) { return (u32)(ctx->h_scalars[slot] >> 32); }
 static inline u32 *sa_dev_slot(tc_ctx *ctx, int slot) { return reinterpret_cast<u32 *>(ctx->d_scalars + slot); }
@@ -272,6 +274,10 @@
     u64 bin_min;
     u64 *part_act1;
     bool part_act1_ok;
+    bool census_level1 = false;
+    u32 census_G = 0;
+    int census_topbits = 0;
+    u32 census_dups = 0;
     u64 m = 0;
     u64 h_start = 0;
     const u64 *skeys = nullptr;
@@ -521,6 +527,94 @@
     return true;
 }
 
+static u32 sa_msd_grid(const SaRun &R) {
+    const tc_ctx *ctx = R.ctx;
+    u32 G = R.b.msd_grid < (u32)ctx->num_cus * MSD_BPC ? R.b.msd_grid : (u32)ctx->num_cus * MSD_BPC;
+    if (ctx->reserved_cus > 0 && G > (u32)(ctx->num_cus - ctx->reserved_cus) * MSD_BPC)
+        G = (u32)(ctx->num_cus - ctx->reserved_cus) * MSD_BPC;
+    if (R.K.msd_grid > 0 && (u32)R.K.msd_grid < G) G = (u32)R.K.msd_grid;
+    return G;
+}
+static MsdLevel sa_msd_level(const SaRun &R, int l, u32 np) {
+    tc_ctx *ctx = R.ctx;
+    const SaBuffers &b = R.b;
+    MsdLevel ML;
+    ML.pstart = b.msd_pstart[l]; ML.pcnt = b.msd_pcnt[l]; ML.tpre = b.msd_tpre[l];
+    ML.nparents = np; ML.shift = 56 - 8 * l; ML.seg = b.msd_seg[l];
+    ML.cstart = b.msd_pstart[l + 1]; ML.ccnt = b.msd_pcnt[l + 1];
+    ML.aligned = 0;
+    ML.ntot = (u32)R.N; ML.cnt_in = b.msd_joint; ML.flags = sa_dev_slot(ctx, SA_SLOT_TIED) + 1;
+    ML.dbg = ctx->d_scalars + SA_SLOT_MSD_PROF + 16 * l;
+    ML.dirfills = sa_dev_slot(ctx, SA_SLOT_MSD_DIR);
+    return ML;
+}
+static MsdTextDigit sa_msd_text_digit(const SaRun &R, const RadixKeyGen &kg) {
+    MsdTextDigit td;
+    td.B = kg.B; td.s = kg.s;
+    memcpy(td.lut, kg.lut, sizeof td.lut);
+    td.text = R.text; td.n = (u32)R.n;
+    td.hash_ok = kg.hash_ok; td.hsh = kg.hsh; td.tlo = kg.tlo; td.thi = kg.thi;
+    return td;
+}
+
+static bool sa_census(SaRun &R, const tc_ctx::CensusMemo &memo, u32 *counts256_out) {
+    tc_ctx *ctx = R.ctx;
+    SaBuffers &b = R.b;
+    hipStream_t s = R.stream();
+    if (!memo.valid || R.K.census == 0 || !msd_wanted(R.N) || b.msd_pstart[0] == nullptr) return false;
+    if (R.K.finish == 0 || R.K.dense != 0 || R.K.sample == 0) return false;
+    RadixKeyGen kg;
+    kg.B = memo.B; kg.w = memo.w; kg.s = memo.s; kg.P = 0;
+    memcpy(kg.lut, memo.lut, sizeof kg.lut);
+    kg.n_text = (u32)R.n;
+    radix_keygen_hash(kg);
+    u64 bytes = 0;
+    if (kg.hash_ok) {
+        u32 used = 0;
+        for (u32 v = 0; v < 256; v++)
+            if (kg.lut[v]) { bytes |= (u64)v << (8 * ((v >> kg.hsh) & 7u)); used |= 1u << ((v >> kg.hsh) & 7u); }
+        for (u32 h = 0; h < 8; h++)
+            if (!((used >> h) & 1u)) bytes |= (u64)(((h + 1) & 7u) << kg.hsh) << (8 * h);
+    }
+    if (R.K.keygen_hash == 0) kg.hash_ok = 0;
+    const MsdTextDigit td = sa_msd_text_digit(R, kg);
+    const u32 G = sa_msd_grid(R);
+    const bool sample = R.n >= (1u << 20);
+    MsdLevel ML = sa_msd_level(R, 0, 1);
+    u32 *slot = sa_dev_slot(ctx, SA_SLOT_CENSUS);
+    tc_memset_async(ctx, slot, 0, sizeof(u64));
+    msd_root_kernel<<<1, 1, 0, s>>>(b.msd_pstart[0], b.msd_pcnt[0], (u32)R.N, sa_dev_slot(ctx, SA_SLOT_MAXCHILD), sa_dev_slot(ctx, SA_SLOT_MSD_DIR));
+    TC_LAUNCH_CHECK(ctx);
+    msd_prep_kernel<<<1, 1024, 0, s>>>(ML.pcnt, 1, b.msd_tpre[0]);
+    TC_LAUNCH_CHECK(ctx);
+    msd_census_kernel<<<G + (sample ? 1u : 0u), MSD_NT, 0, s>>>(ML, td, G, (u32)bytes, (u32)(bytes >> 32), slot, memo.w, memo.topbits, slot + 1);
+    TC_LAUNCH_CHECK(ctx);
+    msd_scan_kernel<<<1, 256, 0, s>>>(ML, G, nullptr);
+    TC_LAUNCH_CHECK(ctx);
+    u32 *totals = reinterpret_cast<u32 *>(ctx->h_scalars + SA_HOST_CENSUS);
+    tc_d2h(ctx, totals, b.msd_pcnt[1], 256 * sizeof(u32));
+    tc_d2h(ctx, &ctx->h_scalars[SA_SLOT_CENSUS], ctx->d_scalars + SA_SLOT_CENSUS, sizeof(u64));
+    TC_HIP(ctx, hipStreamSynchronize(s));
+    u32 counts[256];
+    ctx->census_state = (u32)sa_census_verdict(totals, sa_slot_lo(ctx, SA_SLOT_CENSUS), memo.lut, memo.B, memo.s, R.n, counts);
+    if (ctx->census_state == SA_CENSUS_HIT) {
+        sa_choose_config(counts, R.n, R.K.fields, R.cfg);
+        if (R.cfg.B != memo.B || R.cfg.s != memo.s || R.cfg.w != memo.w || memcmp(R.cfg.lut, memo.lut, sizeof memo.lut) != 0)
+            ctx->census_state = SA_CENSUS_SHORT;
+    }
+    if (R.K.trace)
+        fprintf(stderr, "textcomp: census by the last sort's alphabet (B %u, %u symbols per field): %s\n", memo.B, memo.s,
+                ctx->census_state == SA_CENSUS_HIT ? "hit" : ctx->census_state == SA_CENSUS_FOREIGN ? "miss, a foreign byte" : "miss, a byte missing or a sum off");
+    if (ctx->census_state != SA_CENSUS_HIT) return false;
+    if (counts256_out) memcpy(counts256_out, counts, sizeof counts);
+    R.census_level1 = true;
+    R.census_G = G;
+    R.census_topbits = sample ? memo.topbits : 0;
+    R.census_dups = sa_slot_hi(ctx, SA_SLOT_CENSUS);
+    ctx->census_sample = R.census_dups;
+    return true;
+}
+
 
 static void sa_sample(SaRun &R, int topbits) {
     tc_ctx *ctx = R.ctx;
@@ -581,7 +675,7 @@
     const SaConfig &cfg = R.cfg;
     hipStream_t s = R.stream();
     tc_stats &st = R.st();
-    const u32 n = (u32)R.n, N = (u32)R.N;
+    const u32 N = (u32)R.N;
     Round0Out o;
     o.msd = true; o.msd_big = pl.msd_big; o.keyonly = keyonly;
     sa_round0_begin(R, 8 * MSD_LEVELS, o);
@@ -589,17 +683,16 @@
     RadixKeyGen kg = sa_keygen(R);
     radix_keygen_hash(kg);
     if (R.K.keygen_hash == 0) kg.hash_ok = 0;
-    MsdTextDigit td;
-    sa_fill(cfg, td);
-    td.text = R.text; td.n = n;
-    td.hash_ok = kg.hash_ok; td.hsh = kg.hsh; td.tlo = kg.tlo; td.thi = kg.thi;
-    u32 G = b.msd_grid < (u32)ctx->num_cus * MSD_BPC ? b.msd_grid : (u32)ctx->num_cus * MSD_BPC;
-    if (ctx->reserved_cus > 0 && G > (u32)(ctx->num_cus - ctx->reserved_cus) * MSD_BPC)
-        G = (u32)(ctx->num_cus - ctx->reserved_cus) * MSD_BPC;
-    if (R.K.msd_grid > 0 && (u32)R.K.msd_grid < G) G = (u32)R.K.msd_grid;
+    const MsdTextDigit td = sa_msd_text_digit(R, kg);
+    const u32 G = sa_msd_grid(R);
     u32 *maxchild = sa_dev_slot(ctx, SA_SLOT_MAXCHILD);
-    msd_root_kernel<<<1, 1, 0, s>>>(b.msd_pstart[0], b.msd_pcnt[0], N, maxchild, sa_dev_slot(ctx, SA_SLOT_MSD_DIR));
-    TC_LAUNCH_CHECK(ctx);
+    const bool counted = R.census_level1 && R.census_G == G;
+    R.census_level1 = false;
+    if (counted) ctx->census_level1 = 1;
+    else {
+        msd_root_kernel<<<1, 1, 0, s>>>(b.msd_pstart[0], b.msd_pcnt[0], N, maxchild, sa_dev_slot(ctx, SA_SLOT_MSD_DIR));
+        TC_LAUNCH_CHECK(ctx);
+    }
     u64 *kbuf[2] = {b.k0, b.k1};
     u32 *vbuf[2] = {keyonly ? nullptr : b.v0, keyonly ? nullptr : R.sa};
     st.msd_keyonly = keyonly ? 1u : 0u;
@@ -630,26 +723,22 @@
     if (joint) tc_memset_async(ctx, b.msd_joint, 0, (size_t)256 * 256 * 256 * sizeof(u32));
     u32 np = 1;
     for (int l = 0; l < MSD_LEVELS; l++, np *= 256) {
-        MsdLevel ML;
-        ML.pstart = b.msd_pstart[l]; ML.pcnt = b.msd_pcnt[l]; ML.tpre = b.msd_tpre[l];
-        ML.nparents = np; ML.shift = 56 - 8 * l; ML.seg = b.msd_seg[l];
-        ML.cstart = b.msd_pstart[l + 1]; ML.ccnt = b.msd_pcnt[l + 1];
+        MsdLevel ML = sa_msd_level(R, l, np);
         ML.aligned = (joint && l == MSD_LEVELS - 1) ? 1 : 0;
-        ML.ntot = N; ML.cnt_in = b.msd_joint; ML.flags = counters + 1;
-        ML.dbg = ctx->d_scalars + SA_SLOT_MSD_PROF + 16 * l;
-        ML.dirfills = sa_dev_slot(ctx, SA_SLOT_MSD_DIR);
         const u64 *kin = l ? kbuf[(l - 1) & 1] : nullptr;
         const u32 *vin = l ? vbuf[(l - 1) & 1] : nullptr;
-        msd_prep_kernel<<<1, 1024, 0, s>>>(ML.pcnt, np, b.msd_tpre[l]);
-        TC_LAUNCH_CHECK(ctx);
-        if (l == 0) msd_count_kernel<true, false><<<G, MSD_NT, 0, s>>>(ML, nullptr, td, nullptr, jr);
-        else if (ML.aligned) {  }
-        else if (joint && l == MSD_LEVELS - 2 && split) msd_count_hi_kernel<<<G, MSD_NT, 0, s>>>(ML, khi, td, b.msd_joint, jr);
-        else if (joint && l == MSD_LEVELS - 2) msd_count_kernel<false, true><<<G, MSD_NT, 0, s>>>(ML, kin, td, b.msd_joint, jr);
-        else msd_count_kernel<false, false><<<G, MSD_NT, 0, s>>>(ML, kin, td, nullptr, jr);
-        TC_LAUNCH_CHECK(ctx);
-        msd_scan_kernel<<<np, 256, 0, s>>>(ML, G, l == MSD_LEVELS - 1 ? maxchild : nullptr);
-        TC_LAUNCH_CHECK(ctx);
+        if (l > 0 || !counted) {
+            msd_prep_kernel<<<1, 1024, 0, s>>>(ML.pcnt, np, b.msd_tpre[l]);
+            TC_LAUNCH_CHECK(ctx);
+            if (l == 0) msd_count_kernel<true, false><<<G, MSD_NT, 0, s>>>(ML, nullptr, td, nullptr, jr);
+            else if (ML.aligned) {  }
+            else if (joint && l == MSD_LEVELS - 2 && split) msd_count_hi_kernel<<<G, MSD_NT, 0, s>>>(ML, khi, td, b.msd_joint, jr);
+            else if (joint && l == MSD_LEVELS - 2) msd_count_kernel<false, true><<<G, MSD_NT, 0, s>>>(ML, kin, td, b.msd_joint, jr);
+            else msd_count_kernel<false, false><<<G, MSD_NT, 0, s>>>(ML, kin, td, nullptr, jr);
+            TC_LAUNCH_CHECK(ctx);
+            msd_scan_kernel<<<np, 256, 0, s>>>(ML, G, l == MSD_LEVELS - 1 ? maxchild : nullptr);
+            TC_LAUNCH_CHECK(ctx);
+        }
         const bool ev = ctx->profile && ctx->pev_used < 16;
         if (ev) TC_HIP(ctx, hipEventRecord(ctx->pev[2 * ctx->pev_used], s));
         if (split && l <= 1) {
@@ -893,7 +982,11 @@
     sa_round0_depth(in, R.K, pl);
     const bool finish_fits = (int)(cfg.P * cfg.w) - pl.topbits <= 32;
     if (finish_fits && R.n >= (1u << 20) && R.K.sample != 0) {
-        sa_sample(R, pl.topbits);
+        if (R.census_topbits == pl.topbits) R.st().sample_dups = R.census_dups;
+        else {
+            if (R.census_topbits != 0) R.ctx->census_state = SA_CENSUS_RESAMPLED;
+            sa_sample(R, pl.topbits);
+        }
         hopeless = R.st().sample_dups > SAMP_N / 10;
     }
     if (!finish_fits || hopeless) return false;
@@ -912,6 +1005,13 @@
             o = sa_round0_msd(R, pl, false);
             res = sa_round0_collect(R, o, pl.keyround, many_ties);
         }
+    }
+    if (res == R0_ACCEPTED) {
+        tc_ctx::CensusMemo &memo = R.ctx->census_memo;
+        memcpy(memo.lut, cfg.lut, sizeof memo.lut);
+        memo.B = cfg.B; memo.s = cfg.s; memo.w = cfg.w;
+        memo.topbits = pl.topbits;
+        memo.valid = 1;
     }
     if (res == R0_GIVE_WAY) {
         R.ctx->msd_split_used = 0;
@@ -1175,7 +1275,10 @@
     ctx->msd_dir_used = 0;
     ctx->tied_probe_used = 0;
     ctx->tied_probe_found = 0;
-    if (sa_alphabet(R, counts256_out, primary)) return;
+    ctx->census_state = ctx->census_level1 = ctx->census_sample = 0;
+    const tc_ctx::CensusMemo memo = ctx->census_memo;
+    ctx->census_memo.valid = 0;
+    if (!sa_census(R, memo, counts256_out) && sa_alphabet(R, counts256_out, primary)) return;
 
     const u32 P_full = R.cfg.P;
     R.h_start = R.cfg.h0;
diff --git a/text-compression_amd/csrc/tc_sa_plan.hpp b/text-compression_amd/csrc/tc_sa_plan.hpp
--- a/text-compression_amd/csrc/tc_sa_plan.hpp
+++ b/text-compression_amd/csrc/tc_sa_plan.hpp
@@ -13,6 +13,7 @@
     int dense = env_int("TC_SA_DENSE", 0);
     int global_passes = env_int("TC_SA_GLOBAL_PASSES", 0);
     int sample = env_int("TC_SA_SAMPLE", 1);
+    int census = env_int("TC_SA_CENSUS", 1);
     int msd = env_int("TC_SA_MSD", 1);
     int msd_big = env_int("TC_SA_MSD_BIG", 0);
     int msd_max_dups = env_int("TC_SA_MSD_MAX_DUPS", 8);
@@ -89,6 +90,30 @@
     pl.keyonly = !in.want_sa && (tied_est < (double)in.tied_max / 4.0 || K.msd_keyonly == 2) && K.msd_keyonly != 0;
 }
 
+enum { SA_CENSUS_HIT = 1, SA_CENSUS_FOREIGN = 2, SA_CENSUS_SHORT = 3, SA_CENSUS_RESAMPLED = 4 };
+static inline int sa_census_verdict(const uint32_t totals[256], uint32_t foreign, const uint16_t lut[256], uint32_t B,
+                                    uint32_t s, uint64_t n, uint32_t hist256[256]) {
+    if (foreign) return SA_CENSUS_FOREIGN;
+    if (B < 2 || B > 256 || s < 1) return SA_CENSUS_SHORT;
+    uint64_t lead = 1, nd = B;
+    for (uint32_t j = 1; j < s; j++) { lead = nd; nd *= B; }
+    if (nd > 256) return SA_CENSUS_SHORT;
+    uint64_t marg[256] = {0}, sum = 0;
+    for (uint32_t d = 0; d < 256; d++) {
+        if (d < nd) marg[d / lead] += totals[d];
+        else if (totals[d]) return SA_CENSUS_SHORT;
+        sum += totals[d];
+    }
+    if (sum != n + 1 || marg[0] != 1) return SA_CENSUS_SHORT;
+    for (uint32_t v = 0; v < 256; v++) {
+        const uint32_t c = lut[v];
+        if (c >= B) return SA_CENSUS_SHORT;
+        if (c != 0 && marg[c] == 0) return SA_CENSUS_SHORT;
+        hist256[v] = c ? (uint32_t)marg[c] : 0u;
+    }
+    return SA_CENSUS_HIT;
+}
+
 struct ChainPolicy {
     int mode;
     int keymode = 0;
diff --git a/text-compression_amd/csrc/textcomp.hip b/text-compression_amd/csrc/textcomp.hip
--- a/text-compression_amd/csrc/textcomp.hip
+++ b/text-compression_amd/csrc/textcomp.hip
@@ -15,21 +15,26 @@
 #include "tc_comm.hpp"
 #include "textcomp_debug.h"
 
+static inline int tc_api_err(tc_ctx *ctx, int code) {
+    ctx->census_memo.valid = 0;
+    return code;
+}
+
 #define TC_API_BEGIN(ctx)                                  \
     if (!(ctx)) return TC_ERR_ARG;                         \
     try {                                                  \
         if (hipSetDevice((ctx)->device) != hipSuccess) {   \
             (ctx)->err = "hipSetDevice failed";            \
-            return TC_ERR_HIP;                             \
+            return tc_api_err(ctx, TC_ERR_HIP);            \
         }
 #define TC_API_END(ctx)                                    \
         return TC_OK;                                      \
     } catch (const TcFail &f) {                            \
         (void)hipGetLastError();                           \
-        return f.code;                                     \
+        return tc_api_err(ctx, f.code);                    \
     } catch (...) {                                        \
         (ctx)->err = "unexpected exception";               \
-        return TC_ERR_INTERNAL;                            \
+        return tc_api_err(ctx, TC_ERR_INTERNAL);           \
     }
 
 extern "C" {
@@ -57,7 +62,7 @@
         TC_HIP(ctx, hipStreamCreateWithFlags(&ctx->stream, hipStreamNonBlocking));
         TC_HIP(ctx, hipMalloc((void **)&ctx->d_err, 256));
         TC_HIP(ctx, hipMalloc((void **)&ctx->d_scalars, 128 * sizeof(u64)));
-        TC_HIP(ctx, hipHostMalloc((void **)&ctx->h_scalars, 64 * sizeof(u64), hipHostMallocDefault));
+        TC_HIP(ctx, hipHostMalloc((void **)&ctx->h_scalars, (64 + 128) * sizeof(u64), hipHostMallocDefault));
         TC_HIP(ctx, hipHostMalloc((void **)&ctx->h_hdr, 1024, hipHostMallocDefault));
         TC_HIP(ctx, hipMemsetAsync(ctx->d_err, 0, 256, ctx->stream));
         TC_HIP(ctx, hipMemsetAsync(ctx->d_scalars, 0, 128 * sizeof(u64), ctx->stream));
@@ -120,7 +125,7 @@
     if (!ctx) return TC_ERR_ARG;
     if (coding != TC_CODING_PACKED && coding != TC_CODING_HUFFMAN) {
         ctx->err = "unknown container coding";
-        return TC_ERR_ARG;
+        return tc_api_err(ctx, TC_ERR_ARG);
     }
     ctx->coding = coding;
     return TC_OK;
@@ -467,7 +472,7 @@
         if (nruns) *nruns = h.nruns;
         return TC_OK;
     } catch (const TcFail &f) {
-        return f.code;
+        return tc_api_err(ctx, f.code);
     }
 }
 
@@ -482,7 +487,7 @@
         else TC_FAIL(ctx, TC_ERR_MALFORMED, "container header names no known body format");
         return TC_OK;
     } catch (const TcFail &f) {
-        return f.code;
+        return tc_api_err(ctx, f.code);
     }
 }
 
@@ -521,7 +526,7 @@
         if (nblocks) *nblocks = ix.off.size();
         return TC_OK;
     } catch (const TcFail &f) {
-        return f.code;
+        return tc_api_err(ctx, f.code);
     }
 }
 
@@ -793,7 +798,7 @@
     if (!ctx) return TC_ERR_ARG;
     if (cap != 0 && (cap < 16 || cap > 65536 || cap % 16 != 0)) {
         ctx->err = "the short cap is a multiple of 16 in 16 .. 65536, or 0";
-        return TC_ERR_ARG;
+        return tc_api_err(ctx, TC_ERR_ARG);
     }
     ctx->lcp_cap = cap;
     return TC_OK;
@@ -803,7 +808,7 @@
     if (!ctx) return TC_ERR_ARG;
     if (fanout != 4 && fanout != 8 && fanout != 16 && fanout != 64) {
         ctx->err = "the fan-out of the LCP min tree is 4, 8, 16 or 64";
-        return TC_ERR_ARG;
+        return tc_api_err(ctx, TC_ERR_ARG);
     }
     ctx->fm_lcp_fanout = fanout;
     return TC_OK;
@@ -813,14 +818,15 @@
     if (!ctx) return TC_ERR_ARG;
     if (tile != 0 && (tile < 64 || tile > LZ_TILE_MAX || (tile & (tile - 1)) != 0)) {
         ctx->err = "the tile of the LZ77 parse is a power of two in 64 .. 16384, or 0";
-        return TC_ERR_ARG;
+        return tc_api_err(ctx, TC_ERR_ARG);
     }
     ctx->lz_tile = tile;
     return TC_OK;
 }
 
 int tc_dbg_msd_split_used(tc_ctx *ctx, uint32_t *used) {
-    if (!ctx || !used) return TC_ERR_ARG;
+    if (!ctx) return TC_ERR_ARG;
+    if (!used) return tc_api_err(ctx, TC_ERR_ARG);
     *used = ctx->msd_split_used ? 1u : 0u;
     return TC_OK;
 }
@@ -833,14 +839,25 @@
 }
 
 int tc_dbg_tied_probe(tc_ctx *ctx, uint32_t out[2]) {
-    if (!ctx || !out) return TC_ERR_ARG;
+    if (!ctx) return TC_ERR_ARG;
+    if (!out) return tc_api_err(ctx, TC_ERR_ARG);
     out[0] = (uint32_t)ctx->tied_probe_used;
     out[1] = ctx->tied_probe_found;
     return TC_OK;
 }
 
+int tc_dbg_census(tc_ctx *ctx, uint32_t out[3]) {
+    if (!ctx) return TC_ERR_ARG;
+    if (!out) return tc_api_err(ctx, TC_ERR_ARG);
+    out[0] = ctx->census_state;
+    out[1] = ctx->census_level1;
+    out[2] = ctx->census_sample;
+    return TC_OK;
+}
+
 int tc_dbg_ibwt_walk(tc_ctx *ctx, uint32_t out[3]) {
-    if (!ctx || !out) return TC_ERR_ARG;
+    if (!ctx) return TC_ERR_ARG;
+    if (!out) return tc_api_err(ctx, TC_ERR_ARG);
     out[0] = ctx->ibwt_attempts;
     out[1] = ctx->ibwt_overflowed;
     out[2] = ctx->ibwt_extra_taken;
diff --git a/text-compression_amd/host/check/census_verdict.cpp b/text-compression_amd/host/check/census_verdict.cpp
--- /dev/null
+++ b/text-compression_amd/host/check/census_verdict.cpp
@@ -0,0 +1,115 @@
+#include <algorithm>
+#include <cstdio>
+#include <cstring>
+#include <random>
+#include <vector>
+
+static int env_int(const char *, int dflt) { return dflt; }
+#include "tc_sa_plan.hpp"
+
+#define EXPECT(cond)                                                              \
+    do {                                                                          \
+        if (!(cond)) {                                                            \
+            std::fprintf(stderr, "%s:%d: failed: %s (sigma %u, s %u, n %zu)\n", __FILE__, __LINE__, #cond, sigma, s, text.size()); \
+            return 1;                                                             \
+        }                                                                         \
+    } while (0)
+
+static void digit_totals(const std::vector<uint8_t> &text, const uint16_t *lut, uint32_t B, uint32_t s, uint32_t *totals) {
+    memset(totals, 0, 256 * sizeof(uint32_t));
+    const size_t n = text.size();
+    for (size_t i = 0; i <= n; i++) {
+        uint32_t g = 0;
+        for (uint32_t j = 0; j < s; j++) g = g * B + (i + j < n ? (uint32_t)lut[text[i + j]] : 0u);
+        totals[g]++;
+    }
+}
+
+static int one_case(std::mt19937 &rng, uint32_t sigma, uint32_t s, size_t n) {
+    const uint32_t B = sigma + 1;
+    std::vector<int> pool(256);
+    for (int v = 0; v < 256; v++) pool[v] = v;
+    std::shuffle(pool.begin(), pool.end(), rng);
+    uint16_t lut[256] = {0};
+    std::vector<uint8_t> alpha;
+    for (int v = 0, c = 0; v < 256; v++) {
+        bool in = false;
+        for (uint32_t k = 0; k < sigma; k++) in = in || pool[k] == v;
+        if (in) { lut[v] = (uint16_t)++c; alpha.push_back((uint8_t)v); }
+    }
+    std::vector<uint8_t> text(n);
+    for (size_t i = 0; i < n; i++) text[i] = alpha[i < sigma ? i : rng() % sigma];
+    uint32_t want[256] = {0};
+    for (uint8_t c : text) want[c]++;
+    uint32_t totals[256], hist[256];
+    digit_totals(text, lut, B, s, totals);
+
+    memset(hist, 0xff, sizeof hist);
+    EXPECT(sa_census_verdict(totals, 0, lut, B, s, n, hist) == SA_CENSUS_HIT);
+    EXPECT(memcmp(hist, want, sizeof want) == 0);
+    EXPECT(totals[0] == 1);
+    EXPECT(sa_census_verdict(totals, 1, lut, B, s, n, hist) == SA_CENSUS_FOREIGN);
+    EXPECT(sa_census_verdict(totals, 0x00410000u, lut, B, s, n, hist) == SA_CENSUS_FOREIGN);
+    uint32_t d_real = 0;
+    for (uint32_t d = 1; d < 256; d++)
+        if (totals[d]) d_real = d;
+    EXPECT(d_real != 0);
+    totals[d_real]++;
+    EXPECT(sa_census_verdict(totals, 0, lut, B, s, n, hist) == SA_CENSUS_SHORT);
+    totals[d_real] -= 2;
+    EXPECT(sa_census_verdict(totals, 0, lut, B, s, n, hist) == SA_CENSUS_SHORT);
+    totals[d_real]++;
+    totals[0] = 0;
+    EXPECT(sa_census_verdict(totals, 0, lut, B, s, n, hist) == SA_CENSUS_SHORT);
+    totals[0] = 2;
+    EXPECT(sa_census_verdict(totals, 0, lut, B, s, n, hist) == SA_CENSUS_SHORT);
+    totals[d_real]--;
+    EXPECT(sa_census_verdict(totals, 0, lut, B, s, n, hist) == SA_CENSUS_SHORT);
+    totals[d_real]++;
+    totals[0] = 1;
+    EXPECT(sa_census_verdict(totals, 0, lut, B, s, n, hist) == SA_CENSUS_HIT);
+    EXPECT(sa_census_verdict(totals, 0, lut, B, s, n + 1, hist) == SA_CENSUS_SHORT);
+    if (sigma < 15) {
+        uint32_t B2 = B + 1, nd2 = 1;
+        for (uint32_t j = 0; j < s; j++) nd2 *= B2;
+        if (nd2 <= 256) {
+            int extra = 0;
+            while (lut[extra]) extra++;
+            uint16_t lut2[256] = {0};
+            for (int v = 0, c = 0; v < 256; v++)
+                if (lut[v] || v == extra) lut2[v] = (uint16_t)++c;
+            uint32_t totals2[256];
+            digit_totals(text, lut2, B2, s, totals2);
+            EXPECT(sa_census_verdict(totals2, 0, lut2, B2, s, n, hist) == SA_CENSUS_SHORT);
+        }
+    }
+    return 0;
+}
+
+int main() {
+    std::mt19937 rng(20260101u);
+    int cases = 0;
+    for (uint32_t sigma = 1; sigma <= 15; sigma++)
+        for (uint32_t s = 1; s <= 3; s++) {
+            uint32_t nd = 1;
+            for (uint32_t j = 0; j < s; j++) nd *= sigma + 1;
+            if (nd > 256) continue;
+            for (size_t n : {(size_t)sigma, (size_t)sigma + 1, (size_t)64, (size_t)1000, (size_t)20011}) {
+                if (n < sigma) continue;
+                if (one_case(rng, sigma, s, n)) return 1;
+                cases++;
+            }
+        }
+    {
+        uint32_t totals[256] = {0}, hist[256];
+        uint16_t lut[256] = {0};
+        lut[65] = 1;
+        totals[0] = 1;
+        if (sa_census_verdict(totals, 0, lut, 16, 3, 0, hist) != SA_CENSUS_SHORT || sa_census_verdict(totals, 0, lut, 1, 1, 0, hist) != SA_CENSUS_SHORT) {
+            std::fprintf(stderr, "a configuration without a digit table was not refused\n");
+            return 1;
+        }
+    }
+    std::printf("ok: census verdict, %d cases\n", cases);
+    return 0;
+}
```
